# google-research/seed_rl

Measured on NVIDIA H100. Metric: env-frames/sec (learner, device-timed) on synthetic 84x84x4 T=20 unrolls @1/2/4/8 H100, higher is better.
Workload: dtype bf16x3 (fp32-faithful tensor-core contraction; activations stored as bf16 hi+lo pairs), f32 elsewhere

## Files before the change

include/seedrl_b200.h:

```cpp
#ifndef SEEDRL_B200_H_
#define SEEDRL_B200_H_

#include <stddef.h>
#include <stdint.h>

#ifdef __cplusplus
extern "C" {
#endif

#define SEEDRL_OK 0
#define SEEDRL_ERR_INVALID_ARGUMENT 3
#define SEEDRL_ERR_OUT_OF_RANGE 11
#define SEEDRL_ERR_INTERNAL 13
#define SEEDRL_ERR_CANCELLED 1
#define SEEDRL_ERR_UNAVAILABLE 14

typedef void* seedrl_stream_t;

const char* seedrl_last_error(void);
int seedrl_abi_version(void);
uint64_t seedrl_kernel_launch_count(void);

int seedrl_vtrace_from_importance_weights(
    int T, int B,
    const float* target_action_log_probs, const float* behaviour_action_log_probs,
    const float* discounts, const float* rewards, const float* values,
    const float* bootstrap_value,
    float clip_rho_threshold, float clip_pg_rho_threshold, float lambda_,
    float* vs, float* pg_advantages, seedrl_stream_t stream);

int seedrl_categorical_log_prob(int N, int A, const float* logits,
                                const int64_t* actions, float* log_prob,
                                seedrl_stream_t stream);
int seedrl_categorical_entropy(int N, int A, const float* logits, float* entropy,
                               seedrl_stream_t stream);
int seedrl_categorical_sample(int N, int A, const float* logits,
                              const float* gumbel_noise, uint64_t seed,
                              uint64_t offset, int64_t* actions,
                              seedrl_stream_t stream);
int seedrl_categorical_sample_counter(int N, int A, const float* logits, const float* gumbel_noise,
                                      uint64_t seed, uint64_t* counter_dev, int64_t* actions,
                                      seedrl_stream_t stream);

typedef struct seedrl_loss_config {
  float discounting;
  float lambda_;
  float baseline_cost;
  float kl_cost;
  float max_abs_reward;
  float clip_rho_threshold;
  float clip_pg_rho_threshold;
  float target_entropy;
  int32_t has_target_entropy;
  float entropy_cost_adjustment_speed;
// ... 171 lines not shown
                             const int64_t* replay_action, const float* reward, const uint8_t* done,
                             const float* importance_weights, float gamma, int n_steps, float eta,
                             float value_rescaling_eps, float* loss, float* priorities, float* dq,
                             void* scratch, seedrl_stream_t stream);
size_t seedrl_r2d2_retrace_loss_scratch_bytes(int T, int B);
int seedrl_r2d2_retrace_loss_fwd_bwd(int T, int B, int A, const float* q_train, const float* q_target,
                                     const int64_t* replay_action, const float* reward,
                                     const uint8_t* done, const float* importance_weights, float gamma,
                                     float lambda_, float eta, float value_rescaling_eps, float* loss,
                                     float* priorities, float* dq, void* scratch,
                                     seedrl_stream_t stream);
int seedrl_r2d2_epsilon_greedy(int N, int A, const int32_t* env_ids, const float* envs_epsilon,
                               uint64_t seed, uint64_t* counter_dev, int32_t* actions,
                               seedrl_stream_t stream);
int seedrl_replay_sample(int limit, const float* priorities, float priority_exp,
                         float importance_sampling_exp, int num_samples, const float* uniforms,
                         int64_t* indices, float* weights, float* probs_out, seedrl_stream_t stream);
size_t seedrl_clip_scratch_bytes(void);
int seedrl_clip_by_global_norm(size_t n, float* grads, float clip_norm, float* norm_out,
                               void* scratch, seedrl_stream_t stream);

int seedrl_debug_conv3x3(int cin, int cout, int in_mode, int N, int H, int W,
                         const void* in, const float* w, const float* bias,
                         const float* mask, const float* res, float* out,
                         seedrl_stream_t stream);
int seedrl_debug_conv3x3_flip(int cin, int cout, const float* w, float* wt,
                              seedrl_stream_t stream);
size_t seedrl_debug_wgrad_partial_bytes(void);
int seedrl_debug_conv_pixels(int N, int H, int W, int which, int start, int count, int* out);
int seedrl_debug_set_loss_stream(int enabled);
int seedrl_debug_set_wgrad_chunk(int kc);
int seedrl_debug_set_conv_tile(int mt);
int seedrl_debug_set_gemm_gather(int on);
int seedrl_debug_set_first_layer_dense(int on);
int seedrl_debug_conv0pool(int N, int H, int W, const uint8_t* frames, const float* w, const float* bias,
                           void* praw, void* prelu, uint8_t* idx, int* err, seedrl_stream_t stream);
int seedrl_debug_conv0pool_c(int N, int H, int W, int C, const uint8_t* frames, const float* w, const float* bias,
                             void* praw, void* prelu, uint8_t* idx, int* err, seedrl_stream_t stream);
int seedrl_debug_first_wgrad_pooled_c(int N, int H, int W, int C, const uint8_t* frames, const void* g_planes,
                                      const uint8_t* idx, float* dw, float* db, float* partial,
                                      size_t partial_bytes, seedrl_stream_t stream);
int seedrl_debug_conv3x3_wgrad(int cin, int cout, int in_mode, int N, int H, int W,
                               const void* x, const float* dy, float* dw, float* db,
                               float* partial, size_t partial_bytes,
                               seedrl_stream_t stream);
int seedrl_debug_conv3x3_tc(int cin, int cout, int in_mode, int split, int N, int H, int W,
                            const void* in, const float* w, const float* bias,
                            const float* mask, const float* res, float* out, int flip,
                            int variant, void* wq_scratch, int* error_flag,
                            seedrl_stream_t stream);
int seedrl_debug_conv3x3_wgrad_tc(int cin, int cout, int in_mode, int split, int N, int H, int W,
                                  const void* x, const float* dy, float* dw, float* db,
                                  float* partial, size_t partial_bytes, int* error_flag,
                                  seedrl_stream_t stream);
int seedrl_debug_maxpool(int backward, int N, int H, int W, int C, const float* x_or_dy,
                         float* y_or_dx, uint8_t* idx, seedrl_stream_t stream);
int seedrl_debug_gemm_tc(int ta, int tb, int split, int M, int N, int K, const float* A, int lda,
                         const float* B, int ldb, float* C, int ldc, const float* bias,
                         const float* mask, int ldm, int relu, int accumulate, int a_relu,
                         float* ws, size_t ws_bytes, int* error_flag, seedrl_stream_t stream);
int seedrl_debug_colsum(int M, int N, const float* X, int ld, float* out, float* ws, size_t ws_bytes,
                        seedrl_stream_t stream);
int seedrl_debug_sgemm(int ta, int tb, int M, int N, int K, const float* A, int lda,
                       const float* B, int ldb, float* C, int ldc, const float* bias,
                       const float* mask, int ldm, int relu, int accumulate, int a_relu,
                       seedrl_stream_t stream);
// ... 36 lines not shown
```

seed_rl_b200/_lib.py:

```python
import ctypes
import os

_HERE = os.path.dirname(os.path.abspath(__file__))
LIB_PATH = os.path.join(_HERE, 'libseedrl_b200.so')

c_void_p, c_int, c_float, c_size_t = ctypes.c_void_p, ctypes.c_int, ctypes.c_float, ctypes.c_size_t
c_i64, c_u64 = ctypes.c_int64, ctypes.c_uint64
P = c_void_p


class SeedrlError(RuntimeError):

  def __init__(self, code, msg):
    super().__init__('libseedrl_b200 error %d: %s' % (code, msg))
    self.code = code


class LossConfig(ctypes.Structure):
  _fields_ = [('discounting', c_float), ('lambda_', c_float), ('baseline_cost', c_float),
              ('kl_cost', c_float), ('max_abs_reward', c_float),
              ('clip_rho_threshold', c_float), ('clip_pg_rho_threshold', c_float),
              ('target_entropy', c_float), ('has_target_entropy', ctypes.c_int32),
              ('entropy_cost_adjustment_speed', c_float)]

# ... 5 lines not shown

ROW_GATHER, ROW_SCATTER, ROW_APPEND = 0, 1, 2


def rows_multi(jobs, env_ids_i32, index=None, id_limit=None):
  n = int(env_ids_i32.numel())
  arr = (RowJob * len(jobs))()
  for k, (table, rows, mode) in enumerate(jobs):
    rb = (table[0, 0] if mode == ROW_APPEND else table[0]).numel() * table.element_size()
    if rows.numel() * rows.element_size() != n * rb or rows.dtype != table.dtype or not rows.is_contiguous():
      raise ValueError('rows_multi: rows do not match the table (job %d)' % k)
    arr[k] = RowJob(table.data_ptr(), rows.data_ptr(), rb, mode, table.shape[1] if mode == ROW_APPEND else 0)
  if id_limit is None:
    check(lib().seedrl_rows_multi(arr, len(jobs), ptr(env_ids_i32), n, ptr(index), stream_ptr()))
  else:
    check(lib().seedrl_rows_multi_limit(arr, len(jobs), ptr(env_ids_i32), n, ptr(index), int(id_limit),
                                        stream_ptr()))


class NetConfig(ctypes.Structure):
  _fields_ = [('net', ctypes.c_int32), ('num_actions', ctypes.c_int32),
              ('obs_h', ctypes.c_int32), ('obs_w', ctypes.c_int32), ('obs_c', ctypes.c_int32)]


NET_DEEP, NET_SHALLOW = 0, 1
LOSS_TERMS = 16
LT = dict(total=0, policy=1, V=2, entropy=3, kl=4, entropy_adj=5, v_mean=6, v_l2_error=7,
          mean_entropy=8, entropy_cost=9, mean_kl=10, max_action_abs=11, popart_mean=12, popart_std=13)

SIGNATURES = {
    'seedrl_last_error': (ctypes.c_char_p, []),
    'seedrl_abi_version': (c_int, []),
    'seedrl_kernel_launch_count': (c_u64, []),
    'seedrl_vtrace_from_importance_weights':
        (c_int, [c_int, c_int, P, P, P, P, P, P, c_float, c_float, c_float, P, P, P]),
    'seedrl_categorical_log_prob': (c_int, [c_int, c_int, P, P, P, P]),
    'seedrl_categorical_entropy': (c_int, [c_int, c_int, P, P, P]),
    'seedrl_categorical_sample': (c_int, [c_int, c_int, P, P, c_u64, c_u64, P, P]),
    'seedrl_categorical_sample_counter': (c_int, [c_int, c_int, P, P, c_u64, P, P, P]),
    'seedrl_vtrace_loss_scratch_bytes': (c_size_t, [c_int, c_int, c_int]),
    'seedrl_vtrace_loss_fwd_bwd':
        (c_int, [c_int, c_int, c_int, P, P, P, P, P, P, ctypes.POINTER(LossConfig), P,
                 P, P, P, P, P, P, P, P]),
    'seedrl_vtrace_popart_loss_fwd':
        (c_int, [c_int, c_int, c_int, P, P, P, P, P, P, ctypes.POINTER(LossConfig), P, P, P,
                 P, P, P, P, P, P, P, P, P, P]),
    'seedrl_vtrace_popart_update':
        (c_int, [c_int, c_int, c_int, c_float, c_float, P, P, P, P, P, P, P, P, P, P]),
    'seedrl_adam_apply':
        (c_int, [c_size_t, P, P, P, P, c_float, c_float, c_float, c_float, c_float, c_i64,
                 c_float, c_float, P]),
    'seedrl_net_create': (c_int, [ctypes.POINTER(NetConfig), ctypes.POINTER(P)]),
    'seedrl_net_destroy': (None, [P]),
    'seedrl_net_num_param_tensors': (c_int, [P]),
    'seedrl_net_num_params': (c_size_t, [P]),
    'seedrl_net_arena_floats': (c_size_t, [P]),
    'seedrl_net_set_conv_mode': (c_int, [P, c_int]),
    'seedrl_net_set_lstm_mode': (c_int, [P, c_int]),
    'seedrl_net_param_info':
        (c_int, [P, c_int, ctypes.c_char_p, c_size_t, ctypes.POINTER(c_i64),
                 ctypes.POINTER(c_size_t)]),
    'seedrl_net_workspace_bytes': (c_size_t, [P, c_int, c_int]),
    'seedrl_net_forward':
        (c_int, [P, P, c_int, c_int, P, P, P, P, P, P, P, P, P, P, P, c_size_t, P]),
    'seedrl_net_backward':
        (c_int, [P, P, c_int, c_int, P, P, P, P, P, P, P, P, c_size_t, P]),
# ... 51 lines not shown
    'seedrl_clip_by_global_norm': (c_int, [c_size_t, P, c_float, P, P, P]),
    'seedrl_profile_num_categories': (c_int, []),
    'seedrl_profile_category_name': (ctypes.c_char_p, [c_int]),
    'seedrl_profile_begin': (c_int, [P]),
    'seedrl_profile_end': (c_int, [ctypes.POINTER(ctypes.c_double), ctypes.POINTER(c_u64)]),
    'seedrl_debug_planes_bytes': (c_size_t, [c_int, c_int, c_int, c_int]),
    'seedrl_debug_to_planes': (c_int, [c_int, c_int, c_int, c_int, c_int, P, P, P]),
    'seedrl_debug_from_planes': (c_int, [c_int, c_int, c_int, c_int, P, P, P]),
    'seedrl_debug_convp': (c_int, [c_int, c_int, c_int, c_int, c_int, P, P, P, P, P, c_int, P, P, P, P, P, P]),
    'seedrl_debug_wgradp': (c_int, [c_int, c_int, c_int, c_int, c_int, P, P, P, P, P, c_size_t, P, P]),
    'seedrl_debug_poolp': (c_int, [c_int, c_int, c_int, c_int, c_int, P, P, P, P, P, P]),
    'seedrl_debug_conv3x3': (c_int, [c_int, c_int, c_int, c_int, c_int, c_int, P, P, P, P, P, P, P]),
    'seedrl_debug_conv3x3_flip': (c_int, [c_int, c_int, P, P, P]),
    'seedrl_debug_conv3x3_tc':
        (c_int, [c_int, c_int, c_int, c_int, c_int, c_int, c_int, P, P, P, P, P, P, c_int, c_int, P, P, P]),
    'seedrl_debug_wgrad_partial_bytes': (c_size_t, []),
    'seedrl_debug_conv_pixels': (c_int, [c_int, c_int, c_int, c_int, c_int, c_int, P]),
    'seedrl_debug_set_loss_stream': (c_int, [c_int]),
    'seedrl_debug_set_wgrad_chunk': (c_int, [c_int]),
    'seedrl_debug_set_conv_tile': (c_int, [c_int]),
    'seedrl_debug_set_first_layer_dense': (c_int, [c_int]),
    'seedrl_debug_conv0pool': (c_int, [c_int, c_int, c_int, P, P, P, P, P, P, P, P]),
    'seedrl_debug_conv0pool_c': (c_int, [c_int, c_int, c_int, c_int, P, P, P, P, P, P, P, P]),
    'seedrl_debug_first_wgrad_pooled_c': (c_int, [c_int, c_int, c_int, c_int, P, P, P, P, P, P, c_size_t, P]),
    'seedrl_debug_conv3x3_wgrad_tc':
        (c_int, [c_int, c_int, c_int, c_int, c_int, c_int, c_int, P, P, P, P, P, c_size_t, P, P]),
    'seedrl_debug_conv3x3_wgrad':
        (c_int, [c_int, c_int, c_int, c_int, c_int, c_int, P, P, P, P, P, c_size_t, P]),
    'seedrl_debug_maxpool': (c_int, [c_int, c_int, c_int, c_int, c_int, P, P, P, P]),
    'seedrl_debug_gemm_tc':
        (c_int, [c_int, c_int, c_int, c_int, c_int, c_int, P, c_int, P, c_int, P, c_int, P, P, c_int, c_int, c_int,
                 c_int, P, c_size_t, P, P]),
    'seedrl_debug_set_gemm_gather': (c_int, [c_int]),
    'seedrl_debug_colsum': (c_int, [c_int, c_int, P, c_int, P, P, c_size_t, P]),
    'seedrl_debug_sgemm':
        (c_int, [c_int, c_int, c_int, c_int, c_int, P, c_int, P, c_int, P, c_int, P, P, c_int,
                 c_int, c_int, c_int, P]),
    'seedrl_debug_strided_conv':
        (c_int, [c_int, c_int, c_int, c_int, c_int, c_int, c_int, c_int, c_int, c_int, c_int, P, P, P, P, P, P,
                 c_int, P, P, c_size_t, P, c_size_t, P, ctypes.POINTER(c_int), P]),
    'seedrl_debug_lstm_workspace_bytes': (c_size_t, [c_int, c_int, c_int, c_int]),
    'seedrl_debug_lstm_forward':
        (c_int, [c_int, c_int, c_int, c_int, P, P, P, P, P, P, P, P, P, c_size_t, P, P]),
    'seedrl_debug_lstm_backward':
        (c_int, [c_int, c_int, c_int, c_int, P, P, P, P, P, P, P, P, c_size_t, P, P]),
    'seedrl_debug_r2d2_net_views':
        (c_int, [P, c_int, c_int, c_int, ctypes.POINTER(c_size_t), ctypes.POINTER(c_size_t)]),
    'seedrl_debug_net_views':
        (c_int, [P, c_int, c_int, c_int, ctypes.POINTER(c_size_t), ctypes.POINTER(c_size_t),
                 ctypes.POINTER(c_int)]),
}

_lib = None


def lib():
  global _lib
  if _lib is None:
    if not os.path.exists(LIB_PATH):
      raise ImportError(
          'seed_rl_b200: %s is missing -- build it with `python -c "import '
          '__graft_entry__ as g; g.build()"` (seed_rl_b200/csrc/build.sh). There is no '
          'CPU or PyTorch fallback.' % LIB_PATH)
    l = ctypes.CDLL(LIB_PATH)
    for name, (res, args) in SIGNATURES.items():
      fn = getattr(l, name)
      fn.restype = res
      fn.argtypes = args
    _lib = l
  return _lib


def check(rc):
  if rc != 0:
    raise SeedrlError(rc, (lib().seedrl_last_error() or b'').decode('utf-8', 'replace'))


def launch_count():
  return int(lib().seedrl_kernel_launch_count())


def ptr(t):
  return None if t is None else ctypes.c_void_p(t.data_ptr())


def stream_ptr():
  import torch
  return ctypes.c_void_p(torch.cuda.current_stream().cuda_stream)


def require_cuda(t, dtype, name):
  import torch
  if not isinstance(t, torch.Tensor):
    t = torch.as_tensor(t)
  if not torch.cuda.is_available():
    raise RuntimeError('seed_rl_b200 needs a CUDA device (H100); there is no CPU path '
                       '(argument %r).' % name)
  if t.device.type != 'cuda':
    t = t.cuda()
  if t.dtype != dtype:
    t = t.to(dtype)
  return t.contiguous()
```

seed_rl_b200/csrc/capi.cu:

```cuda
#include <vector>

#include "common.cuh"

namespace seedrl {
thread_local std::string g_last_error;
std::atomic<uint64_t> g_launch_count{0};
bool g_prof_on = false;
int g_conv_cat = PC_CONV_FWD;

struct ProfRec { int cat; cudaEvent_t e; };
static std::vector<ProfRec> g_prof;
static cudaEvent_t g_prof_start;

void prof_mark_(int cat, cudaStream_t st) {
  ProfRec r;
  r.cat = cat;
  cudaEventCreate(&r.e);
  cudaEventRecord(r.e, st);
  g_prof.push_back(r);
}
}

static const char* kProfNames[seedrl::PC_COUNT] = {
    "conv3x3_fwd", "conv3x3_dgrad", "conv3x3_wgrad", "maxpool", "sgemm", "lstm_pointwise",
    "vtrace_loss", "adam", "vtrace", "misc"};

extern "C" const char* seedrl_last_error(void) { return seedrl::g_last_error.c_str(); }
extern "C" int seedrl_abi_version(void) { return 1; }
extern "C" uint64_t seedrl_kernel_launch_count(void) {
  return seedrl::g_launch_count.load(std::memory_order_relaxed);
}

extern "C" int seedrl_profile_num_categories(void) { return seedrl::PC_COUNT; }
extern "C" const char* seedrl_profile_category_name(int i) {
  return (i >= 0 && i < seedrl::PC_COUNT) ? kProfNames[i] : "";
}
extern "C" int seedrl_profile_begin(seedrl_stream_t stream) {
  seedrl::g_prof.clear();
  cudaEventCreate(&seedrl::g_prof_start);
  cudaEventRecord(seedrl::g_prof_start, (cudaStream_t)stream);
  seedrl::g_prof_on = true;
  return SEEDRL_OK;
}
extern "C" int seedrl_profile_end(double* ms_per_category, uint64_t* launches_per_category) {
  seedrl::g_prof_on = false;
  if (!ms_per_category || !launches_per_category)
    return seedrl::set_error(SEEDRL_ERR_INVALID_ARGUMENT, "seedrl_profile_end: null pointer");
  if (cudaDeviceSynchronize() != cudaSuccess)
    return seedrl::set_error(SEEDRL_ERR_INTERNAL, "seedrl_profile_end: device sync failed");
  for (int i = 0; i < seedrl::PC_COUNT; ++i) {
    ms_per_category[i] = 0;
    launches_per_category[i] = 0;
  }
  cudaEvent_t prev = seedrl::g_prof_start;
  for (auto& r : seedrl::g_prof) {
    float ms = 0.f;
    if (cudaEventElapsedTime(&ms, prev, r.e) == cudaSuccess) {
      ms_per_category[r.cat] += ms;
      launches_per_category[r.cat] += 1;
    }
    cudaEventDestroy(prev);
    prev = r.e;
  }
// ... 5 lines not shown
```

seed_rl_b200/csrc/common.cuh:

```cuda
#pragma once
#include <cuda.h>
#include <cuda_runtime.h>
#include <stdint.h>
#include <stdio.h>

#include <atomic>
#include <string>

#include "../../include/seedrl_b200.h"

namespace seedrl {

extern thread_local std::string g_last_error;
extern std::atomic<uint64_t> g_launch_count;

inline int set_error(int code, const std::string& msg) {
  g_last_error = msg;
  return code;
}

#define SEEDRL_TRY(expr)                \
  do {                                  \
    const int rc__ = (expr);            \
    if (rc__ != SEEDRL_OK) return rc__; \
  } while (0)

#define SEEDRL_CHECK_ARG(cond, msg)                                         \
  do {                                                                      \
    if (!(cond))                                                            \
      return ::seedrl::set_error(SEEDRL_ERR_INVALID_ARGUMENT,               \
                                 std::string(__func__) + ": " + (msg));     \
  } while (0)

#define SEEDRL_CHECK_LAUNCH()                                               \
  do {                                                                      \
    cudaError_t e__ = cudaGetLastError();                                   \
    if (e__ != cudaSuccess)                                                 \
      return ::seedrl::set_error(                                           \
          SEEDRL_ERR_INTERNAL, std::string(__func__) + ": CUDA launch: " +  \
                                   cudaGetErrorString(e__));                \
  } while (0)

#define SEEDRL_CUDA(...)                                                    \
  do {                                                                      \
    cudaError_t e__ = (__VA_ARGS__);                                        \
    if (e__ != cudaSuccess)                                                 \
      return ::seedrl::set_error(                                           \
          SEEDRL_ERR_INTERNAL,                                              \
          std::string(__func__) + ": " #__VA_ARGS__ ": " + cudaGetErrorString(e__)); \
  } while (0)

enum ProfCat { PC_CONV_FWD = 0, PC_CONV_DGRAD, PC_CONV_WGRAD, PC_POOL, PC_GEMM, PC_LSTM_PW,
               PC_LOSS, PC_ADAM, PC_VTRACE, PC_MISC, PC_COUNT };
extern bool g_prof_on;
extern int g_conv_cat;
void prof_mark_(int cat, cudaStream_t st);

inline void count_launch(int cat = PC_MISC, cudaStream_t st = 0) {
  g_launch_count.fetch_add(1, std::memory_order_relaxed);
  if (g_prof_on) prof_mark_(cat, st);
}

constexpr int kNumSMs = 132;

template <auto K>
cudaError_t allow_smem(int bytes) {
  static const cudaError_t e = cudaFuncSetAttribute(K, cudaFuncAttributeMaxDynamicSharedMemorySize, bytes);
  return e;
}

typedef CUresult (*EncodeTiledFn)(CUtensorMap*, CUtensorMapDataType, cuuint32_t, void*, const cuuint64_t*,
                                  const cuuint64_t*, const cuuint32_t*, const cuuint32_t*, CUtensorMapInterleave,
                                  CUtensorMapSwizzle, CUtensorMapL2promotion, CUtensorMapFloatOOBfill);
inline EncodeTiledFn encode_tiled_fn() {
  static const EncodeTiledFn fn = [] {
    void* q = nullptr;
    cudaDriverEntryPointQueryResult qr;
    const bool found = cudaGetDriverEntryPoint("cuTensorMapEncodeTiled", &q, cudaEnableDefault, &qr) == cudaSuccess &&
                       qr == cudaDriverEntryPointSuccess;
    (void)cudaGetLastError();
    return found ? reinterpret_cast<EncodeTiledFn>(q) : nullptr;
  }();
  return fn;
}

__host__ __device__ inline int ceil_div(int a, int b) { return (a + b - 1) / b; }
__host__ __device__ inline size_t ceil_div_sz(size_t a, size_t b) { return (a + b - 1) / b; }

__device__ __forceinline__ float warp_sum(float v) {
#pragma unroll
  for (int o = 16; o > 0; o >>= 1) v += __shfl_xor_sync(0xffffffffu, v, o);
  return v;
}
__device__ __forceinline__ float warp_max(float v) {
#pragma unroll
// ... 21 lines not shown
```

seed_rl_b200/csrc/conv_first.cu:

```cuda
#include <cuda.h>

#include <cstring>

#include "kernels.h"
#include "tc_common.cuh"

namespace seedrl {

constexpr int kFwThreads = 256;
constexpr int kFwCo = 16;
constexpr int kFwLanes = kFwThreads / kFwCo;

static inline int first_layer_cp(int c) { return c <= 4 ? 4 : (c <= 8 ? 8 : 16); }
static inline int fw_rows_per_band(int cp) { return cp == 16 ? 4 : 6; }
static inline size_t fw_pixels_8b(int cp, int rb, int W) { return ((size_t)(2 * rb + 3) * (W + 2) * (cp / 4) + 1) & ~(size_t)1; }
static inline size_t fw_smem(int cp, int rb, int W) {
  const int wo = (W + 1) / 2;
  return fw_pixels_8b(cp, rb, W) * 8 + (size_t)rb * wo * kFwCo * 5;
}

struct FirstWgradArgs {
  int N, H, W, C, Ho, Wo, pt, pl;
  int Lpp, PWp, RHp;
  int rb;
  const uint8_t* frames;
  const uint4* g;
  const uint8_t* idx;
  float* partial;
};

__device__ __forceinline__ uint32_t load_u8x4(const uint8_t* px, int c0, int C) {
  uint32_t v = 0u;
#pragma unroll
  for (int j = 0; j < 4; ++j)
    if (c0 + j < C) v |= (uint32_t)__ldg(px + c0 + j) << (8 * j);
  return v;
}

template <int CP, bool kU32>
__global__ void __launch_bounds__(kFwThreads, kU32 ? 3 : 2) first_wgrad_pooled_kernel(const FirstWgradArgs a) {
  constexpr int G = CP / 4;
  constexpr int NL = kFwLanes / G;
  extern __shared__ __align__(128) uint8_t smem_raw[];
  const int tid = threadIdx.x;
  const int co = tid & (kFwCo - 1), grp = (tid >> 4) & (G - 1), ql = (tid >> 4) / G;
  const int SW = a.W + 2;
  const int RB = a.rb;
  const int SR = 2 * RB + 3;
  uint2* s_x = reinterpret_cast<uint2*>(smem_raw);
  float* s_g = reinterpret_cast<float*>(s_x + ((SR * SW * G + 1) & ~1));
  uint8_t* s_t = reinterpret_cast<uint8_t*>(s_g + RB * a.Wo * kFwCo);
  float acc[36];
#pragma unroll
  for (int i = 0; i < 36; ++i) acc[i] = 0.f;
  float accb = 0.f;
  const int bands = (a.Ho + RB - 1) / RB;
  const int units = a.N * bands;
  for (int u = blockIdx.x; u < units; u += gridDim.x) {
    const int n = u / bands, band = u - n * bands;
    const int r0 = band * RB, r1 = min(a.Ho, r0 + RB);
    const int nq = (r1 - r0) * a.Wo;
    const int f0 = 2 * r0 - a.pt - 1;
    for (int i = tid; i < SR * SW * G; i += kFwThreads) {
      const int px = i / G, gi = i - px * G;
      const int lr = px / SW, bc = px - lr * SW, fr = f0 + lr;
      uint32_t w32 = 0u;
      if (fr >= 0 && fr < a.H && bc >= 1 && bc <= a.W) {
        const size_t pix = ((size_t)n * a.H + fr) * a.W + bc - 1;
        if (kU32) w32 = __ldg(reinterpret_cast<const uint32_t*>(a.frames) + pix);
        else w32 = load_u8x4(a.frames + pix * a.C, 4 * gi, a.C);
      }
      const uint32_t f0_ = __float_as_uint(__uint_as_float(__byte_perm(w32, 0x4B000000u, 0x7540)) - 8388608.0f);
      const uint32_t f1_ = __float_as_uint(__uint_as_float(__byte_perm(w32, 0x4B000000u, 0x7541)) - 8388608.0f);
      const uint32_t f2_ = __float_as_uint(__uint_as_float(__byte_perm(w32, 0x4B000000u, 0x7542)) - 8388608.0f);
      const uint32_t f3_ = __float_as_uint(__uint_as_float(__byte_perm(w32, 0x4B000000u, 0x7543)) - 8388608.0f);
      s_x[i] = make_uint2(__byte_perm(f0_, f1_, 0x7632), __byte_perm(f2_, f3_, 0x7632));
    }
    for (int i = tid; i < nq * 2; i += kFwThreads) {
      const int gq = i & 1, qq = i >> 1;
      const int qr = qq / a.Wo, qw = qq - qr * a.Wo;
      const size_t sp = (size_t)(n * a.RHp + r0 + qr + 1) * a.PWp + qw + 1;
      const uint4 hh = __ldg(a.g + (size_t)gq * a.Lpp + sp), ll = __ldg(a.g + (size_t)(2 + gq) * a.Lpp + sp);
      float4* dst = reinterpret_cast<float4*>(s_g + (size_t)qq * kFwCo + gq * 8);
      dst[0] = make_float4(__uint_as_float(hh.x << 16) + __uint_as_float(ll.x << 16),
                           __uint_as_float(hh.x & 0xFFFF0000u) + __uint_as_float(ll.x & 0xFFFF0000u),
                           __uint_as_float(hh.y << 16) + __uint_as_float(ll.y << 16),
                           __uint_as_float(hh.y & 0xFFFF0000u) + __uint_as_float(ll.y & 0xFFFF0000u));
      dst[1] = make_float4(__uint_as_float(hh.z << 16) + __uint_as_float(ll.z << 16),
// ... 31 lines not shown
      while (qw >= a.Wo) { qw -= a.Wo; ++qh; }
    }
    __syncthreads();
  }
  float* s_red = reinterpret_cast<float*>(smem_raw);
  const int slot = ql * G + grp;
#pragma unroll
  for (int i = 0; i < 36; ++i) s_red[(slot * 37 + i) * kFwCo + co] = acc[i];
  s_red[(slot * 37 + 36) * kFwCo + co] = accb;
  __syncthreads();
  const int nw = 9 * a.C;
  float* dst = a.partial + (size_t)blockIdx.x * ((nw + 1) * kFwCo);
  for (int e = tid; e < (nw + 1) * kFwCo; e += kFwThreads) {
    const int i = e / kFwCo, c = e - i * kFwCo;
    const int tap = i / a.C, ci = i - tap * a.C;
    const int gi = i < nw ? ci >> 2 : 0, k = i < nw ? tap * 4 + (ci & 3) : 36;
    float s = 0.f;
#pragma unroll
    for (int l = 0; l < NL; ++l) s += s_red[((l * G + gi) * 37 + k) * kFwCo + c];
    if (i < nw) dst[i * kFwCo + c] = s * (1.0f / 255.0f);
    else dst[nw * kFwCo + c] = s;
  }
}

bool first_wgrad_pooled_supported(int cin, int cout, int H, int W) {
  if (cin < 1 || cin > 16 || cout != 16 || H < 3 || W < 3) return false;
  const int cp = first_layer_cp(cin);
  return fw_smem(cp, fw_rows_per_band(cp), W) <= 70 * 1024;
}

template <int CP, bool kU32>
static int launch_first_wgrad(const FirstWgradArgs& a, int grid, size_t smem, cudaStream_t st) {
  SEEDRL_CUDA(allow_smem<first_wgrad_pooled_kernel<CP, kU32>>(72 * 1024));
  first_wgrad_pooled_kernel<CP, kU32><<<grid, kFwThreads, smem, st>>>(a);
  return SEEDRL_OK;
}

int first_wgrad_pooled(int N, int H, int W, int C, const uint8_t* frames, const void* g_planes, const uint8_t* idx,
                       float* dw, float* db, WgradBatch* batch, cudaStream_t st) {
  if (!first_wgrad_pooled_supported(C, 16, H, W))
    return set_error(SEEDRL_ERR_INVALID_ARGUMENT, "first_wgrad_pooled: unsupported frame shape");
  int Ho, Wo, pt, pl;
  same_pad3s2(H, &Ho, &pt);
  same_pad3s2(W, &Wo, &pl);
  const int cp = first_layer_cp(C);
  FirstWgradArgs a;
  a.N = N; a.H = H; a.W = W; a.C = C; a.Ho = Ho; a.Wo = Wo; a.pt = pt; a.pl = pl;
  a.Lpp = (int)planes_positions(N, Ho, Wo); a.PWp = Wo + 2; a.RHp = Ho + 1;
  a.frames = frames; a.g = reinterpret_cast<const uint4*>(g_planes); a.idx = idx;
  a.rb = fw_rows_per_band(cp) < Ho ? fw_rows_per_band(cp) : Ho;
  size_t smem = fw_smem(cp, a.rb, W);
  const size_t red = (size_t)kFwLanes * 37 * kFwCo * 4;
  if (red > smem) smem = red;
  smem = (smem + 127) / 128 * 128;
  const int NW = 9 * C * kFwCo + kFwCo;
  const int units = N * ((Ho + a.rb - 1) / a.rb);
  int grid = (C == 4 ? 3 : 2) * kNumSMs;
  if (grid > units) grid = units;
  if (!batch || batch->n >= kMaxReduceJobs || batch->used + (size_t)grid * NW > batch->cap_floats)
    return set_error(SEEDRL_ERR_INVALID_ARGUMENT, "first_wgrad_pooled: partial buffer too small");
  a.partial = batch->buf + batch->used;
  batch->used += (size_t)grid * NW;
  const int rc = C == 4    ? launch_first_wgrad<4, true>(a, grid, smem, st)
                 : cp == 4 ? launch_first_wgrad<4, false>(a, grid, smem, st)
                 : cp == 8 ? launch_first_wgrad<8, false>(a, grid, smem, st)
                           : launch_first_wgrad<16, false>(a, grid, smem, st);
  if (rc != SEEDRL_OK) return rc;
  count_launch(PC_CONV_WGRAD, st);
  SEEDRL_CHECK_LAUNCH();
  batch->jobs[batch->n++] = ReduceJob{a.partial, dw, db, grid, 9 * C * kFwCo, kFwCo};
  return SEEDRL_OK;
}

constexpr int kCpThreadsF = 256;
constexpr int kCpRows = 3;
constexpr int kCpMaxBlocks = 6;
constexpr int kCpOutStride = 20;

struct Conv0PoolArgs {
  int N, H, W, Ho, Wo, pt, pl;
  int Lpp, PWp, RHp;
  int C;
  unsigned int sw_mul; int sw_sh;
  const uint8_t* frames;
  const float* w;
  const float* bias;
  uint4* praw; uint4* prelu;
  uint8_t* idx;
  int* err;
};

__device__ __forceinline__ uint2 u8x4_to_bf16x4(uint32_t w32) {
  const uint32_t f0 = __float_as_uint(__uint_as_float(__byte_perm(w32, 0x4B000000u, 0x7540)) - 8388608.0f);
  const uint32_t f1 = __float_as_uint(__uint_as_float(__byte_perm(w32, 0x4B000000u, 0x7541)) - 8388608.0f);
  const uint32_t f2 = __float_as_uint(__uint_as_float(__byte_perm(w32, 0x4B000000u, 0x7542)) - 8388608.0f);
  const uint32_t f3 = __float_as_uint(__uint_as_float(__byte_perm(w32, 0x4B000000u, 0x7543)) - 8388608.0f);
  return make_uint2(__byte_perm(f0, f1, 0x7632), __byte_perm(f2, f3, 0x7632));
}

template <int CP, bool kTma>
__global__ void __launch_bounds__(kCpThreadsF, 2) conv0pool_kernel(const __grid_constant__ CUtensorMap tm_frames,
// ... 9 lines not shown
  uint4* s_p = reinterpret_cast<uint4*>(smem_raw);
  float* s_out = reinterpret_cast<float*>(smem_raw + (size_t)kPlanes * npair * 16);
  uint8_t* s_bq = reinterpret_cast<uint8_t*>(s_out + (size_t)kCpMaxBlocks * 128 * kCpOutStride);
  s_bq = reinterpret_cast<uint8_t*>(((uintptr_t)s_bq + 127) & ~(uintptr_t)127);
  float* s_bias = reinterpret_cast<float*>(s_bq + KT * 32 * 2);
  uint64_t* s_full = reinterpret_cast<uint64_t*>(s_bias + 16);
  constexpr int kRawRows = 2 * kCpRows + 3;
  uint32_t* s_raw = reinterpret_cast<uint32_t*>(((uintptr_t)(s_full + 4) + 127) & ~(uintptr_t)127);
  const uint32_t raw_bytes = (uint32_t)(kRawRows * W) * 4u;
  const uint32_t raw_stride = (raw_bytes + 127u) & ~127u;

  for (int i = tid; i < KT * 32; i += kCpThreadsF) {
    const int k = i / 32, nn = i - k * 32;
    const int kh = k / KH, kw = (k - kh * KH) / CP, ci = k - kh * KH - kw * CP;
    float v = 0.f;
    if (kw < 3 && ci < a.C) {
      const float wv = __ldg(a.w + ((kh * 3 + kw) * a.C + ci) * 16 + (nn & 15));
      v = nn < 16 ? wv : bf16_resid(wv);
    }
    const uint32_t off = (uint32_t)(k >> 3) * 512u + (uint32_t)(nn >> 3) * 128u + (uint32_t)(nn & 7) * 16u +
                         (uint32_t)(k & 7) * 2u;
    *reinterpret_cast<__nv_bfloat16*>(s_bq + off) = __float2bfloat16_rn(v);
  }
  if (tid < 16) s_bias[tid] = __ldg(a.bias + tid);
  for (int i = tid; i < kPlanes * npair; i += kCpThreadsF) s_p[i] = make_uint4(0u, 0u, 0u, 0u);
  if (kTma && tid == 0) {
    mbar_init(s_full, 1);
    mbar_init(s_full + 1, 1);
    asm volatile("fence.mbarrier_init.release.cluster;" ::: "memory");
    asm volatile("prefetch.tensormap [%0];" ::"l"(reinterpret_cast<uint64_t>(&tm_frames)) : "memory");
  }
  asm volatile("fence.proxy.async.shared::cta;" ::: "memory");
  __syncthreads();
  const uint32_t a_base = smem_u32(s_p), b_base = smem_u32(s_bq);

  const int bands = (a.Ho + kCpRows - 1) / kCpRows;
  const int units = a.N * bands;
  bool timed_out = false;
  auto unit_geom = [&](int u, int* n, int* r0, int* r1, int* cr0, int* cr1) {
    *n = u / bands;
    const int band = u - *n * bands;
    *r0 = band * kCpRows; *r1 = min(a.Ho, *r0 + kCpRows);
    *cr0 = max(0, 2 * *r0 - a.pt); *cr1 = min(H - 1, 2 * (*r1 - 1) - a.pt + 2);
  };
  auto issue_tile = [&](int u, int st) {
    int n, r0, r1, cr0, cr1;
    unit_geom(u, &n, &r0, &r1, &cr0, &cr1);
    const uint32_t dst = smem_u32(s_raw) + (uint32_t)st * raw_stride, bar = smem_u32(s_full + st);
    asm volatile("mbarrier.arrive.expect_tx.shared::cta.b64 _, [%0], %1;" ::"r"(bar), "r"(raw_bytes) : "memory");
    asm volatile(
        "cp.async.bulk.tensor.3d.shared::cluster.global.tile.mbarrier::complete_tx::bytes [%0], [%1, {%2, %3, %4}], [%5];" ::
            "r"(dst), "l"(reinterpret_cast<uint64_t>(&tm_frames)), "r"(0), "r"(cr0 - 1), "r"(n), "r"(bar)
        : "memory");
  };
  if (kTma && tid == 0 && (int)blockIdx.x < units) issue_tile(blockIdx.x, 0);
  int it = 0;
  for (int u = blockIdx.x; u < units; u += gridDim.x, ++it) {
    int n, r0, r1, cr0, cr1;
    unit_geom(u, &n, &r0, &r1, &cr0, &cr1);
    const int band = u - n * bands;
    const int CR = cr1 - cr0 + 1, npos = CR * SW, nblk = (npos + 127) >> 7;
    const int st = it & 1;
    if constexpr (kTma) {
      if (tid == 0 && u + (int)gridDim.x < units) issue_tile(u + gridDim.x, st ^ 1);
      if (!mbar_wait_bounded(s_full + st, (uint32_t)((it >> 1) & 1))) timed_out = true;
      const uint32_t* raw = s_raw + (size_t)st * (raw_stride / 4);
// ... 123 lines not shown
        const size_t sp = (size_t)(n * a.RHp + r0 + rr + 1) * a.PWp + (side ? a.Wo + 1 : 0);
        a.praw[(size_t)pl_ * a.Lpp + sp] = z;
        a.prelu[(size_t)pl_ * a.Lpp + sp] = z;
      }
      if (band == 0) {
        for (int i = tid; i < a.PWp * 4; i += kCpThreadsF) {
          const int pl_ = i & 3, cc = i >> 2;
          const size_t sp = (size_t)(n * a.RHp) * a.PWp + cc;
          a.praw[(size_t)pl_ * a.Lpp + sp] = z;
          a.prelu[(size_t)pl_ * a.Lpp + sp] = z;
        }
      }
      if (u == units - 1) {
        const int t0 = a.N * a.RHp * a.PWp;
        for (int i = tid; i < (a.Lpp - t0) * 4; i += kCpThreadsF) {
          const int pl_ = i & 3, cc = i >> 2;
          a.praw[(size_t)pl_ * a.Lpp + t0 + cc] = z;
          a.prelu[(size_t)pl_ * a.Lpp + t0 + cc] = z;
        }
      }
    }
    __syncthreads();
  }
  if (timed_out && a.err) atomicExch(a.err, 1);
}

bool conv0pool_supported(int cin, int cout, int H, int W) {
  if (cout != 16 || H < 3 || W < 3 || 7 * (W + 2) > 6 * 128) return false;
  if (cin == 4) return W % 4 == 0 && W <= 256;
  return cin >= 1 && cin <= 16;
}

template <int CP, bool TMA>
static int launch_conv0pool(Conv0PoolArgs a, const uint8_t* frames, cudaStream_t st) {
  constexpr int KT = 3 * (CP == 16 ? 48 : 4 * CP);
  const int N = a.N, H = a.H, W = a.W;
  const size_t raw_stride = TMA ? (((size_t)(2 * kCpRows + 3) * W * 4) + 127) / 128 * 128 : 0;
  const size_t smem = (size_t)(CP == 16 ? 2 : 1) * (kCpMaxBlocks * 128 + 2 * (W + 2) + 8) * 16 +
                      (size_t)kCpMaxBlocks * 128 * kCpOutStride * 4 + 128 + KT * 32 * 2 + 16 * 4 + 64 + 128 +
                      2 * raw_stride;
  SEEDRL_CUDA(allow_smem<conv0pool_kernel<CP, TMA>>(112 * 1024));
  if (smem > 112 * 1024) return set_error(SEEDRL_ERR_INVALID_ARGUMENT, "conv0pool: image too wide");
  CUtensorMap tm;
  memset(&tm, 0, sizeof(tm));
  if (TMA) {
    const EncodeTiledFn enc = encode_tiled_fn();
    if (!enc) return set_error(SEEDRL_ERR_INTERNAL, "cuTensorMapEncodeTiled is not available");
    const cuuint64_t gdim[3] = {(cuuint64_t)W, (cuuint64_t)H, (cuuint64_t)N};
    const cuuint64_t gstr[2] = {(cuuint64_t)W * 4, (cuuint64_t)H * W * 4};
    const cuuint32_t box[3] = {(cuuint32_t)W, (cuuint32_t)(2 * kCpRows + 3), 1};
    const cuuint32_t estr[3] = {1, 1, 1};
    if (enc(&tm, CU_TENSOR_MAP_DATA_TYPE_UINT32, 3, const_cast<uint8_t*>(frames), gdim, gstr, box, estr,
            CU_TENSOR_MAP_INTERLEAVE_NONE, CU_TENSOR_MAP_SWIZZLE_NONE, CU_TENSOR_MAP_L2_PROMOTION_L2_128B,
            CU_TENSOR_MAP_FLOAT_OOB_FILL_NONE) != CUDA_SUCCESS)
      return set_error(SEEDRL_ERR_INTERNAL, "conv0pool: cuTensorMapEncodeTiled failed");
  }
  const int units = N * ((a.Ho + kCpRows - 1) / kCpRows);
  const int grid = units < 2 * kNumSMs ? units : 2 * kNumSMs;
  conv0pool_kernel<CP, TMA><<<grid, kCpThreadsF, smem, st>>>(tm, a);
  count_launch(PC_CONV_FWD, st);
  SEEDRL_CHECK_LAUNCH();
  return SEEDRL_OK;
}

int conv0pool_forward(int N, int H, int W, int C, const uint8_t* frames, const float* w, const float* bias,
                      void* praw, void* prelu, uint8_t* idx, int* err, cudaStream_t st) {
  if (!conv0pool_supported(C, 16, H, W))
    return set_error(SEEDRL_ERR_INVALID_ARGUMENT, "conv0pool: unsupported frame shape");
  Conv0PoolArgs a;
  a.N = N; a.H = H; a.W = W; a.C = C;
  same_pad3s2(H, &a.Ho, &a.pt);
  same_pad3s2(W, &a.Wo, &a.pl);
  a.Lpp = (int)planes_positions(N, a.Ho, a.Wo); a.PWp = a.Wo + 2; a.RHp = a.Ho + 1;
  fast_div_setup((unsigned int)(W + 2), &a.sw_mul, &a.sw_sh);
  a.frames = frames; a.w = w; a.bias = bias;
  a.praw = reinterpret_cast<uint4*>(praw); a.prelu = reinterpret_cast<uint4*>(prelu); a.idx = idx; a.err = err;
  if (C == 4) return launch_conv0pool<4, true>(a, frames, st);
  const int cp = first_layer_cp(C);
  return cp == 4 ? launch_conv0pool<4, false>(a, frames, st)
                 : (cp == 8 ? launch_conv0pool<8, false>(a, frames, st) : launch_conv0pool<16, false>(a, frames, st));
}

}
```

seed_rl_b200/csrc/conv_planes.cu:

```cuda
#include <cuda.h>
#include <cuda_bf16.h>

#include <cstdio>

#include "kernels.h"
#include "tc_common.cuh"

namespace seedrl {

long long planes_positions(int N, int H, int W) {
  const long long Q = (long long)N * (H + 1) * (W + 2);
  return ((Q + 2 * (W + 2) + 2 + 256 + 127) / 128) * 128;
}
size_t planes_bytes(int N, int H, int W, int C) {
  return (size_t)planes_positions(N, H, W) * 16 * 2 * (C / 8);
}

constexpr int kPlanesChunk = 128;

static int make_plane_map(CUtensorMap* tm, const void* base, long long Lp, int planes, int shift,
                          int CH, int box_chunks, int box_planes) {
  EncodeTiledFn enc = encode_tiled_fn();
  if (!enc) return set_error(SEEDRL_ERR_INTERNAL, "cuTensorMapEncodeTiled is not available");
  if (box_chunks < 1 || box_chunks > 256 || box_planes < 1 || box_planes > planes)
// ... 65 lines not shown
    }
  }
}

template <int CIN, int COUT, int NSUB>
__global__ void __launch_bounds__(kCpThreads, 1)
convp_kernel(const __grid_constant__ CUtensorMap tm_in, const ConvpArgs a) {
  constexpr int G = CIN / 8, GO = COUT / 8, NS = CIN / 16;
  constexpr int MT = NSUB * kCpM;
  constexpr int NBLK = 2 * NSUB;
  extern __shared__ __align__(128) uint8_t smem_raw[];
  const int PW = a.g.PW, nb = a.nb;
  const uint32_t P = (uint32_t)(a.nch * a.chunk) * 16u;
  const uint32_t stage_bytes = 2u * G * P;
  uint8_t* s_stage = smem_raw;
  uint4* s_b = reinterpret_cast<uint4*>(smem_raw + (size_t)nb * stage_bytes);
  float* s_bias = reinterpret_cast<float*>(s_b + 2 * 9 * CIN * COUT / 8);
  uint64_t* s_full = reinterpret_cast<uint64_t*>(s_bias + COUT);
  uint64_t* s_empty = s_full + kCpMaxStages;
  const int tid = threadIdx.x, warp = tid >> 5, lane = tid & 31;

  for (int i = tid; i < 2 * 9 * CIN * COUT / 8; i += kCpThreads) s_b[i] = __ldg(a.wq + i);
  if (tid < COUT) s_bias[tid] = a.bias ? __ldg(a.bias + tid) : 0.f;
  if (tid == 0) {
    for (int i = 0; i < nb; ++i) {
      mbar_init(s_full + i, 1);
      mbar_init(s_empty + i, 4 * kCpWarpgroups);
    }
    asm volatile("fence.mbarrier_init.release.cluster;" ::: "memory");
    asm volatile("prefetch.tensormap [%0];" ::"l"(reinterpret_cast<uint64_t>(&tm_in)) : "memory");
  }
  asm volatile("fence.proxy.async.shared::cta;" ::: "memory");
  __syncthreads();

  const int my_tiles = ((int)blockIdx.x < a.ntiles) ? (a.ntiles - 1 - (int)blockIdx.x) / (int)gridDim.x + 1 : 0;
  bool timed_out = false;

  if (warp == 4 * kCpWarpgroups) {
    if (elect_one()) {
      for (int it = 0; it < my_tiles; ++it) {
        const int s = it % nb;
        if (it >= nb && !mbar_wait_bounded(s_empty + s, (uint32_t)(((it / nb) - 1) & 1))) { timed_out = true; break; }
        const int tile = (int)blockIdx.x + it * (int)gridDim.x;
        mbar_expect_tx(s_full + s, stage_bytes);
        tma_load_3d(s_stage + (size_t)s * stage_bytes, &tm_in, 0, tile * MT / a.chunk, 0, s_full + s);
      }
    }
    __syncwarp();
  } else {
    const int cw = warp >> 2;
    const size_t plane_u = (size_t)a.Lp;
    if (blockIdx.x == 0) {
      const uint4 z = make_uint4(0u, 0u, 0u, 0u);
      for (int i = tid; i < (PW + 1) * 2 * GO; i += 128 * kCpWarpgroups) {
        const int pl = i / (PW + 1), s = i - pl * (PW + 1);
        if (a.out_raw) a.out_raw[(size_t)pl * plane_u + s] = z;
        if (a.out_relu) a.out_relu[(size_t)pl * plane_u + s] = z;
      }
    }
    const int q = lane & 3;
    const int row = 16 * (warp & 3) + (lane >> 2) + 8 * (q & 1);
    const uint32_t b_base = smem_u32(s_b);
    const uint64_t db0 = gmma_desc(b_base, (uint32_t)(2 * GO) * 128u, 128u);
    for (int it = 0; it < my_tiles; ++it) {
      const int s = it % nb;
      const int tile = (int)blockIdx.x + it * (int)gridDim.x;
// ... 98 lines not shown
      }
    }
  }
  if (timed_out && a.err) atomicExch(a.err, 1);
}

template <int CIN, int COUT, int NSUB>
static int launch_convp(const PlaneConv& c, cudaStream_t st) {
  const ConvGeom g = make_geom(c.N, c.H, c.W);
  constexpr int MT = NSUB * kCpM;
  const long long Lp = planes_positions(c.N, c.H, c.W);
  if (Lp + MT + 4 * g.PW >= (1LL << 31))
    return set_error(SEEDRL_ERR_INVALID_ARGUMENT, "convp: batch too large for 32-bit positions");
  const int L = MT + 2 * g.PW + 2;
  const int CH = kPlanesChunk;
  const int nch = (L + CH - 1) / CH;
  const size_t stage = (size_t)2 * (CIN / 8) * nch * CH * 16;
  const size_t fixed = (size_t)2 * 9 * CIN * COUT * 2 + COUT * 4 + 2 * kCpMaxStages * 8;
  int nb = kCpMaxStages;
  while (nb > 1 && nb * stage + fixed > 227 * 1024) --nb;
  if (nb < 2) return kPlanesTryNext;
  const size_t smem = nb * stage + fixed;
  CUtensorMap tm;
  SEEDRL_TRY(make_plane_map(&tm, c.in, Lp, 2 * (CIN / 8), 0, CH, nch, 2 * (CIN / 8)));
  SEEDRL_CUDA(allow_smem<convp_kernel<CIN, COUT, NSUB>>(227 * 1024));
  ConvpArgs a;
  a.g = g; a.Lp = (int)Lp; a.nch = nch; a.chunk = CH; a.nb = nb;
  a.ntiles = (int)((Lp - g.PW - 1 + MT - 1) / MT);
  a.wq = reinterpret_cast<const uint4*>(c.wq); a.bias = c.bias;
  a.mask = reinterpret_cast<const uint4*>(c.mask); a.res = reinterpret_cast<const uint4*>(c.res);
  a.out_raw = reinterpret_cast<uint4*>(c.out_raw); a.out_relu = reinterpret_cast<uint4*>(c.out_relu);
  a.out_nhwc = c.out_nhwc; a.err = c.err;
  const int grid = a.ntiles < kNumSMs ? a.ntiles : kNumSMs;
  convp_kernel<CIN, COUT, NSUB><<<grid, kCpThreads, smem, st>>>(tm, a);
  count_launch(g_conv_cat, st);
  SEEDRL_CHECK_LAUNCH();
  return SEEDRL_OK;
}

bool convp_supported(int cin, int cout) {
  return (cin == 16 || cin == 32) && (cout == 16 || cout == 32);
}

int convp_forward(int cin, int cout, const PlaneConv& c, cudaStream_t st) {
  const long long Lp = planes_positions(c.N, c.H, c.W);
  const bool small = Lp / 512 < 2 * kNumSMs;
#define SEEDRL_CP_CASE(CI, CO_)                                                   \
  if (cin == CI && cout == CO_) {                                                 \
    int rc = kPlanesTryNext;                                                      \
    if (!small) rc = launch_convp<CI, CO_, 4>(c, st);                             \
    if (rc == kPlanesTryNext) rc = launch_convp<CI, CO_, 2>(c, st);               \
    if (rc == kPlanesTryNext) rc = launch_convp<CI, CO_, 1>(c, st);               \
    if (rc == kPlanesTryNext) return set_error(SEEDRL_ERR_INVALID_ARGUMENT, "convp: image too wide"); \
    return rc;                                                                    \
  }
  SEEDRL_CP_CASE(16, 16)
  SEEDRL_CP_CASE(16, 32)
  SEEDRL_CP_CASE(32, 16)
  SEEDRL_CP_CASE(32, 32)
#undef SEEDRL_CP_CASE
  return set_error(SEEDRL_ERR_INVALID_ARGUMENT, "convp: unsupported (cin,cout)");
}

struct WgradpArgs {
  int PW, T, nchunks, nb;
  int chunk;
  float* partial;
  int* err;
};

constexpr int kWpMaxStages = 6;
constexpr int kWpHaloRow = 8;
__host__ __device__ constexpr int wgradp_mtiles(int CP) { return 3 * CP + 1 <= 64 ? 1 : 2; }
__host__ __device__ constexpr int wgradp_khsplit(int CP) { return CP == 16 ? 3 : 1; }
__host__ __device__ constexpr int wgradp_threads(int CP) { return 128 * wgradp_mtiles(CP) * wgradp_khsplit(CP) + 32; }

struct WgradMaps { CUtensorMap x, x_halo, dy, dy_halo; };

template <int CP, int COUT, int KC>
__global__ void __launch_bounds__(wgradp_threads(CP), 1)
wgradp_kernel(const __grid_constant__ WgradMaps tm, const WgradpArgs a) {
  constexpr int G = CP / 8, GO = COUT / 8;
  constexpr int MT = wgradp_mtiles(CP), KSPL = wgradp_khsplit(CP), NCW = MT * KSPL;
  constexpr int NKH = 3 / KSPL;
  constexpr int NW = 9 * CP * COUT + COUT;
  constexpr uint32_t Px = (KC + kWpHaloRow) * 16;
  extern __shared__ __align__(128) uint8_t smem_raw[];
  const int nb = a.nb, PW = a.PW;
  const uint32_t Pd = (uint32_t)(KC + a.T) * 16u;
  const uint32_t x_bytes = 2u * G * Px;
  const uint32_t stage_bytes = x_bytes + 2u * GO * Pd;
  uint64_t* s_full = reinterpret_cast<uint64_t*>(smem_raw);
  uint64_t* s_empty = s_full + kWpMaxStages;
  uint8_t* s_stage = smem_raw + 128;
  const int tid = threadIdx.x, warp = tid >> 5, lane = tid & 31;

  if (tid == 0) {
    for (int i = 0; i < kWpMaxStages; ++i) { mbar_init(s_full + i, 1); mbar_init(s_empty + i, 4 * NCW); }
    asm volatile("fence.mbarrier_init.release.cluster;" ::: "memory");
  }
  __syncthreads();

  const int my_chunks = ((int)blockIdx.x < a.nchunks) ? (a.nchunks - 1 - (int)blockIdx.x) / (int)gridDim.x + 1 : 0;
  bool timed_out = false;

  if (warp == 4 * NCW) {
    if (elect_one()) {
      for (int it = 0; it < my_chunks; ++it) {
        const int s = it % nb;
        if (it >= nb && !mbar_wait_bounded(s_empty + s, (uint32_t)(((it / nb) - 1) & 1))) { timed_out = true; break; }
        const int j0 = ((int)blockIdx.x + it * (int)gridDim.x) * KC;
        uint8_t* xs = s_stage + (size_t)s * stage_bytes;
        uint8_t* ds = xs + x_bytes;
        mbar_expect_tx(s_full + s, stage_bytes);
        for (int p = 0; p < 2 * G; ++p) {
          tma_load_3d(xs + p * Px, &tm.x, 0, j0 / a.chunk, p, s_full + s);
          tma_load_3d(xs + p * Px + KC * 16, &tm.x_halo, 0, (j0 + KC) / kWpHaloRow, p, s_full + s);
        }
        for (int p = 0; p < 2 * GO; ++p) {
          tma_load_3d(ds + p * Pd, &tm.dy, 0, j0 / a.chunk, p, s_full + s);
          tma_load_3d(ds + p * Pd + KC * 16, &tm.dy_halo, 0, (j0 + KC) / kWpHaloRow, p, s_full + s);
        }
      }
    }
    __syncwarp();
  } else {
    const int cw = warp >> 2, mt = cw % MT, kh0 = (cw / MT) * NKH;
    const int mg0 = 8 * mt + 2 * (warp & 3);
    const int mg = mg0 + ((lane >> 3) & 1);
    const uint32_t a_off = (mg < 3 * G ? (uint32_t)(mg % G) * Px + (uint32_t)(mg / G) * 16u : 0u) +
                           (uint32_t)((lane >> 4) * 8 + (lane & 7)) * 16u;
    const bool data0 = mg0 < 3 * G, data1 = mg0 + 1 < 3 * G;
    const uint32_t one = (lane >> 2) == 0 ? 0x3F803F80u : 0u;
    const uint32_t c0 = mg0 == 3 * G ? one : 0u, c1 = mg0 + 1 == 3 * G ? one : 0u;
// ... 55 lines not shown
  }
  if (timed_out && a.err) atomicExch(a.err, 1);
}

template <int CP, int COUT, int KC>
static int launch_wgradp(int N, int H, int W, const void* x, const void* dy, float* dw, float* db, int* err,
                         WgradBatch* batch, cudaStream_t st) {
  const ConvGeom g = make_geom(N, H, W);
  const long long Lp = planes_positions(N, H, W);
  constexpr int G = CP / 8, GO = COUT / 8;
  const int CH = kPlanesChunk < KC ? kPlanesChunk : KC;
  if (KC % CH) return kPlanesTryNext;
  const int T = (2 * g.PW + kWpHaloRow - 1) / kWpHaloRow * kWpHaloRow;
  const size_t stage = (size_t)2 * G * (KC + kWpHaloRow) * 16 + (size_t)2 * GO * (KC + T) * 16;
  int nb = kWpMaxStages;
  while (nb > 1 && 128 + nb * stage > 227 * 1024) --nb;
  if (nb < 2) return kPlanesTryNext;
  const size_t smem = 128 + nb * stage;
  WgradMaps tm;
  SEEDRL_TRY(make_plane_map(&tm.x, x, Lp, 2 * G, g.PW, CH, KC / CH, 1));
  SEEDRL_TRY(make_plane_map(&tm.x_halo, x, Lp, 2 * G, g.PW, kWpHaloRow, 1, 1));
  SEEDRL_TRY(make_plane_map(&tm.dy, dy, Lp, 2 * GO, 1, CH, KC / CH, 1));
  SEEDRL_TRY(make_plane_map(&tm.dy_halo, dy, Lp, 2 * GO, 1, kWpHaloRow, T / kWpHaloRow, 1));
  SEEDRL_CUDA(allow_smem<wgradp_kernel<CP, COUT, KC>>(227 * 1024));
  constexpr int NW = 9 * CP * COUT + COUT;
  WgradpArgs a;
  a.PW = g.PW; a.T = T; a.nb = nb; a.err = err; a.chunk = CH;
  a.nchunks = (int)((g.Q + g.PW + KC - 1) / KC);
  const int grid = a.nchunks < kNumSMs ? a.nchunks : kNumSMs;
  if (!batch || batch->n >= kMaxReduceJobs || batch->used + (size_t)grid * NW > batch->cap_floats)
    return set_error(SEEDRL_ERR_INVALID_ARGUMENT, "wgradp: partial buffer too small");
  a.partial = batch->buf + batch->used;
  batch->used += (size_t)grid * NW;
  wgradp_kernel<CP, COUT, KC><<<grid, wgradp_threads(CP), smem, st>>>(tm, a);
  count_launch(PC_CONV_WGRAD, st);
  SEEDRL_CHECK_LAUNCH();
  batch->jobs[batch->n++] = ReduceJob{a.partial, dw, db, grid, 9 * CP * COUT, COUT};
  return SEEDRL_OK;
}

int wgradp(int cin, int cout, int N, int H, int W, const void* x, const void* dy, float* dw, float* db,
           int* err, WgradBatch* batch, cudaStream_t st) {
#define SEEDRL_WP_CASE(CI, CO_, KC0)                                                                        \
  if (cin == CI && cout == CO_) {                                                                           \
    int rc = kPlanesTryNext;                                                                                \
    if constexpr (KC0 >= 256) rc = launch_wgradp<CI, CO_, 256>(N, H, W, x, dy, dw, db, err, batch, st);     \
    if (rc == kPlanesTryNext) rc = launch_wgradp<CI, CO_, 128>(N, H, W, x, dy, dw, db, err, batch, st);     \
    if (rc == kPlanesTryNext) rc = launch_wgradp<CI, CO_, 64>(N, H, W, x, dy, dw, db, err, batch, st);      \
    if (rc == kPlanesTryNext) return set_error(SEEDRL_ERR_INVALID_ARGUMENT, "wgradp: does not fit");        \
    return rc;                                                                                              \
  }
  SEEDRL_WP_CASE(16, 16, 256)
  SEEDRL_WP_CASE(16, 32, 128)
  SEEDRL_WP_CASE(32, 32, 128)
#undef SEEDRL_WP_CASE
  return set_error(SEEDRL_ERR_INVALID_ARGUMENT, "wgradp: unsupported (cin,cout)");
}

__global__ void to_planes_kernel(ConvGeom g, int Lp, int G, int relu, const float* __restrict__ x,
                                 uint4* __restrict__ out) {
  const long long i = (long long)blockIdx.x * blockDim.x + threadIdx.x;
  if (i >= (long long)Lp * G) return;
  const int s = (int)(i / G), go = (int)(i - (long long)s * G);
  const int pix = in_pixel(g, s);
  float4 a = make_float4(0.f, 0.f, 0.f, 0.f), b = a;
  if (pix >= 0) {
    const float4* src = reinterpret_cast<const float4*>(x + (size_t)pix * (G * 8) + go * 8);
    a = __ldg(src); b = __ldg(src + 1);
    if (relu) {
      a.x = fmaxf(a.x, 0.f); a.y = fmaxf(a.y, 0.f); a.z = fmaxf(a.z, 0.f); a.w = fmaxf(a.w, 0.f);
      b.x = fmaxf(b.x, 0.f); b.y = fmaxf(b.y, 0.f); b.z = fmaxf(b.z, 0.f); b.w = fmaxf(b.w, 0.f);
    }
  }
  out[(size_t)go * Lp + s] = pack8_bf16(a, b);
  out[(size_t)(G + go) * Lp + s] = pack8_bf16(bf16_resid4(a), bf16_resid4(b));
}

__global__ void from_planes_kernel(ConvGeom g, int Lp, int G, const uint4* __restrict__ in, float* __restrict__ y) {
  const long long i = (long long)blockIdx.x * blockDim.x + threadIdx.x;
  if (i >= (long long)Lp * G) return;
  const int s = (int)(i / G), go = (int)(i - (long long)s * G);
  const int pix = in_pixel(g, s);
  if (pix < 0) return;
  const uint4 h = __ldg(in + (size_t)go * Lp + s), l = __ldg(in + (size_t)(G + go) * Lp + s);
  float4* dst = reinterpret_cast<float4*>(y + (size_t)pix * (G * 8) + go * 8);
  dst[0] = make_float4(bf16lo(h.x) + bf16lo(l.x), bf16hi(h.x) + bf16hi(l.x), bf16lo(h.y) + bf16lo(l.y),
                       bf16hi(h.y) + bf16hi(l.y));
  dst[1] = make_float4(bf16lo(h.z) + bf16lo(l.z), bf16hi(h.z) + bf16hi(l.z), bf16lo(h.w) + bf16lo(l.w),
                       bf16hi(h.w) + bf16hi(l.w));
}

int to_planes(int N, int H, int W, int C, int relu, const float* x, void* out, cudaStream_t st) {
  const ConvGeom g = make_geom(N, H, W);
  const long long Lp = planes_positions(N, H, W);
  const long long n = Lp * (C / 8);
  to_planes_kernel<<<(unsigned)((n + 255) / 256), 256, 0, st>>>(g, (int)Lp, C / 8, relu, x,
                                                                reinterpret_cast<uint4*>(out));
  count_launch(PC_MISC, st);
  SEEDRL_CHECK_LAUNCH();
  return SEEDRL_OK;
}
int from_planes(int N, int H, int W, int C, const void* in, float* y, cudaStream_t st) {
  const ConvGeom g = make_geom(N, H, W);
  const long long Lp = planes_positions(N, H, W);
  const long long n = Lp * (C / 8);
  from_planes_kernel<<<(unsigned)((n + 255) / 256), 256, 0, st>>>(g, (int)Lp, C / 8,
                                                                  reinterpret_cast<const uint4*>(in), y);
  count_launch(PC_MISC, st);
  SEEDRL_CHECK_LAUNCH();
  return SEEDRL_OK;
}

__global__ void poolp_fwd_kernel(ConvGeom go_, int Lp, int G, int H, int W, int pt, int pl,
                                 const float* __restrict__ x, uint4* __restrict__ out_raw,
                                 uint4* __restrict__ out_relu, uint8_t* __restrict__ idx) {
  const long long i = (long long)blockIdx.x * blockDim.x + threadIdx.x;
  if (i >= (long long)Lp * G) return;
  const int s = (int)(i / G), gq = (int)(i - (long long)s * G);
  const int pix = in_pixel(go_, s);
  float best[8];
  unsigned char arg[8];
#pragma unroll
  for (int e = 0; e < 8; ++e) { best[e] = 0.f; arg[e] = 0; }
  if (pix >= 0) {
    const int Wo = go_.W, Ho = go_.H, C = G * 8;
    const int n = pix / (Ho * Wo), r = pix - n * (Ho * Wo), ho = r / Wo, wo = r - ho * Wo;
#pragma unroll
    for (int e = 0; e < 8; ++e) best[e] = -INFINITY;
#pragma unroll
    for (int kh = 0; kh < 3; ++kh) {
      const int h = ho * 2 - pt + kh;
      if (h < 0 || h >= H) continue;
#pragma unroll
      for (int kw = 0; kw < 3; ++kw) {
        const int w = wo * 2 - pl + kw;
        if (w < 0 || w >= W) continue;
        const float4* src = reinterpret_cast<const float4*>(x + ((size_t)(n * H + h) * W + w) * C + gq * 8);
        const float4 a = __ldg(src), b = __ldg(src + 1);
        const float v[8] = {a.x, a.y, a.z, a.w, b.x, b.y, b.z, b.w};
        const unsigned char t = (unsigned char)(kh * 3 + kw);
#pragma unroll
        for (int e = 0; e < 8; ++e)
          if (v[e] > best[e]) { best[e] = v[e]; arg[e] = t; }
      }
    }
    uint2 packed;
    packed.x = arg[0] | (arg[1] << 8) | (arg[2] << 16) | ((uint32_t)arg[3] << 24);
    packed.y = arg[4] | (arg[5] << 8) | (arg[6] << 16) | ((uint32_t)arg[7] << 24);
    *reinterpret_cast<uint2*>(idx + (size_t)pix * C + gq * 8) = packed;
  }
  const float4 a = make_float4(best[0], best[1], best[2], best[3]), b = make_float4(best[4], best[5], best[6], best[7]);
  out_raw[(size_t)gq * Lp + s] = pack8_bf16(a, b);
  out_raw[(size_t)(G + gq) * Lp + s] = pack8_bf16(bf16_resid4(a), bf16_resid4(b));
  const float4 ra = make_float4(fmaxf(a.x, 0.f), fmaxf(a.y, 0.f), fmaxf(a.z, 0.f), fmaxf(a.w, 0.f));
  const float4 rb = make_float4(fmaxf(b.x, 0.f), fmaxf(b.y, 0.f), fmaxf(b.z, 0.f), fmaxf(b.w, 0.f));
  out_relu[(size_t)gq * Lp + s] = pack8_bf16(ra, rb);
  out_relu[(size_t)(G + gq) * Lp + s] = pack8_bf16(bf16_resid4(ra), bf16_resid4(rb));
}

template <bool OUT_PLANES>
__global__ void poolp_bwd_kernel(ConvGeom gf, int Lpf, ConvGeom gp, int Lpp, int G, int pt, int pl,
                                 const uint4* __restrict__ dy, const uint8_t* __restrict__ idx,
                                 uint4* __restrict__ dx_planes, float* __restrict__ dx_nhwc) {
  const long long i = (long long)blockIdx.x * blockDim.x + threadIdx.x;
  const int H = gf.H, W = gf.W, Ho = gp.H, Wo = gp.W, C = G * 8;
  int gq, s = 0, pix;
  if (OUT_PLANES) {
    if (i >= (long long)Lpf * G) return;
    s = (int)(i / G); gq = (int)(i - (long long)s * G);
    pix = in_pixel(gf, s);
  } else {
    if (i >= (long long)gf.N * H * W * G) return;
    pix = (int)(i / G); gq = (int)(i - (long long)pix * G);
  }
  float acc[8];
#pragma unroll
  for (int e = 0; e < 8; ++e) acc[e] = 0.f;
  if (pix >= 0) {
    const int n = pix / (H * W), r = pix - n * (H * W), h = r / W, w = r - h * W;
    const int hp = h + pt, wp = w + pl;
#pragma unroll
    for (int dh = 0; dh < 2; ++dh) {
      const int ho = (hp >> 1) - dh;
      const int kh = hp - 2 * ho;
      if (ho < 0 || ho >= Ho || kh > 2) continue;
#pragma unroll
      for (int dw = 0; dw < 2; ++dw) {
        const int wo = (wp >> 1) - dw;
        const int kw = wp - 2 * wo;
        if (wo < 0 || wo >= Wo || kw > 2) continue;
        const unsigned tap = (unsigned)(kh * 3 + kw);
        const size_t o = ((size_t)(n * Ho + ho) * Wo + wo) * C + gq * 8;
        const uint2 t = __ldg(reinterpret_cast<const uint2*>(idx + o));
        const int sp = (n * gp.RH + ho + 1) * gp.PW + wo + 1;
        const uint4 hh = __ldg(dy + (size_t)gq * Lpp + sp), ll = __ldg(dy + (size_t)(G + gq) * Lpp + sp);
        const float gv[8] = {bf16lo(hh.x) + bf16lo(ll.x), bf16hi(hh.x) + bf16hi(ll.x), bf16lo(hh.y) + bf16lo(ll.y),
                             bf16hi(hh.y) + bf16hi(ll.y), bf16lo(hh.z) + bf16lo(ll.z), bf16hi(hh.z) + bf16hi(ll.z),
                             bf16lo(hh.w) + bf16lo(ll.w), bf16hi(hh.w) + bf16hi(ll.w)};
#pragma unroll
        for (int e = 0; e < 8; ++e) {
          const unsigned te = ((e < 4 ? t.x : t.y) >> (8 * (e & 3))) & 0xFFu;
          if (te == tap) acc[e] += gv[e];
        }
      }
    }
  }
  const float4 a = make_float4(acc[0], acc[1], acc[2], acc[3]), b = make_float4(acc[4], acc[5], acc[6], acc[7]);
  if (OUT_PLANES) {
    dx_planes[(size_t)gq * Lpf + s] = pack8_bf16(a, b);
    dx_planes[(size_t)(G + gq) * Lpf + s] = pack8_bf16(bf16_resid4(a), bf16_resid4(b));
  } else {
    float4* dst = reinterpret_cast<float4*>(dx_nhwc + (size_t)pix * C + gq * 8);
    dst[0] = a; dst[1] = b;
  }
}

int poolp_forward(int N, int H, int W, int C, const float* x, void* out_raw, void* out_relu, uint8_t* idx,
                  cudaStream_t st) {
  int Ho, Wo, pt, pl;
  same_pad3s2(H, &Ho, &pt);
  same_pad3s2(W, &Wo, &pl);
  const ConvGeom g = make_geom(N, Ho, Wo);
  const long long Lp = planes_positions(N, Ho, Wo);
  const long long n = Lp * (C / 8);
  poolp_fwd_kernel<<<(unsigned)((n + 255) / 256), 256, 0, st>>>(g, (int)Lp, C / 8, H, W, pt, pl, x,
                                                                reinterpret_cast<uint4*>(out_raw),
                                                                reinterpret_cast<uint4*>(out_relu), idx);
  count_launch(PC_POOL, st);
  SEEDRL_CHECK_LAUNCH();
  return SEEDRL_OK;
}

int poolp_backward(int N, int H, int W, int C, const void* dy, const uint8_t* idx, void* dx_planes,
                   float* dx_nhwc, cudaStream_t st) {
  int Ho, Wo, pt, pl;
  same_pad3s2(H, &Ho, &pt);
  same_pad3s2(W, &Wo, &pl);
  const ConvGeom gf = make_geom(N, H, W), gp = make_geom(N, Ho, Wo);
  const long long Lpf = planes_positions(N, H, W), Lpp = planes_positions(N, Ho, Wo);
  if (dx_planes) {
    const long long n = Lpf * (C / 8);
    poolp_bwd_kernel<true><<<(unsigned)((n + 255) / 256), 256, 0, st>>>(
        gf, (int)Lpf, gp, (int)Lpp, C / 8, pt, pl, reinterpret_cast<const uint4*>(dy), idx,
        reinterpret_cast<uint4*>(dx_planes), nullptr);
  } else {
    const long long n = (long long)N * H * W * (C / 8);
    poolp_bwd_kernel<false><<<(unsigned)((n + 255) / 256), 256, 0, st>>>(
        gf, (int)Lpf, gp, (int)Lpp, C / 8, pt, pl, reinterpret_cast<const uint4*>(dy), idx, nullptr, dx_nhwc);
  }
  count_launch(PC_POOL, st);
  SEEDRL_CHECK_LAUNCH();
  return SEEDRL_OK;
}

}
```

seed_rl_b200/csrc/conv_tc_kernels.cu:

```cuda
#include <cuda_bf16.h>

#include "kernels.h"
#include "tc_common.cuh"

namespace seedrl {

__global__ void pack_w_tc_kernel(int CIN, int COUT, int cin_src, int flip, int split, const float* __restrict__ w,
                                 __nv_bfloat16* __restrict__ wq) {
  const int i = blockIdx.x * blockDim.x + threadIdx.x;
  if (i >= 9 * CIN * COUT) return;
  const int e = i & 7;
  const int r = (i >> 3) & 7;
  int rest = i >> 6;
  const int cog = rest % (COUT / 8); rest /= (COUT / 8);
  const int kc = rest & 1; rest >>= 1;
  const int NS = CIN / 16;
  const int slab = rest % NS;
  const int tap = rest / NS;
  const int ci = slab * 16 + kc * 8 + e, co = cog * 8 + r;
  const float v = ci >= cin_src ? 0.f
                  : (flip ? w[((size_t)(8 - tap) * COUT + co) * CIN + ci] : w[((size_t)tap * cin_src + ci) * COUT + co]);
  const __nv_bfloat16 hi = __float2bfloat16_rn(v);
  if (split == 2) {
    const int GOc = COUT / 8;
    const size_t j = ((((size_t)(tap * NS + slab) * 2 + kc) * (2 * GOc) + cog) * 8 + r) * 8 + e;
    wq[j] = hi;
    wq[j + (size_t)GOc * 64] = __float2bfloat16_rn(v - __bfloat162float(hi));
    return;
  }
  wq[i] = hi;
  if (split) wq[9 * CIN * COUT + i] = __float2bfloat16_rn(v - __bfloat162float(hi));
}

__global__ void pack_w_tc_batch_kernel(const __grid_constant__ PackTable t, int split) {
  const PackJob j = t.jobs[blockIdx.y];
  const int CIN = j.ck, COUT = j.cout;
  const int i = blockIdx.x * blockDim.x + threadIdx.x;
  if (i >= 9 * CIN * COUT) return;
  const int e = i & 7;
  const int r = (i >> 3) & 7;
  int rest = i >> 6;
  const int cog = rest % (COUT / 8); rest /= (COUT / 8);
  const int kc = rest & 1; rest >>= 1;
  const int NS = CIN / 16;
  const int slab = rest % NS;
  const int tap = rest / NS;
  const int ci = slab * 16 + kc * 8 + e, co = cog * 8 + r;
  const float v = ci >= j.cin_src ? 0.f
                  : (j.flip ? j.w[((size_t)(8 - tap) * COUT + co) * CIN + ci]
                            : j.w[((size_t)tap * j.cin_src + ci) * COUT + co]);
  __nv_bfloat16* wq = reinterpret_cast<__nv_bfloat16*>(j.wq);
  const __nv_bfloat16 hi = __float2bfloat16_rn(v);
  if (split == 2 && !j.legacy) {
    const int GOc = COUT / 8;
    const size_t q = ((((size_t)(tap * NS + slab) * 2 + kc) * (2 * GOc) + cog) * 8 + r) * 8 + e;
    wq[q] = hi;
    wq[q + (size_t)GOc * 64] = __float2bfloat16_rn(v - __bfloat162float(hi));
    return;
  }
  wq[i] = hi;
  if (split) wq[9 * CIN * COUT + i] = __float2bfloat16_rn(v - __bfloat162float(hi));
}

int conv3x3_tc_pack_weights_batch(const PackTable& t, int split, cudaStream_t st) {
  if (t.n == 0) return SEEDRL_OK;
  pack_w_tc_batch_kernel<<<dim3(ceil_div(9 * 32 * 32, 256), t.n), 256, 0, st>>>(t, split);
  count_launch(PC_MISC, st);
  SEEDRL_CHECK_LAUNCH();
  return SEEDRL_OK;
}

constexpr int kTcThreads = 256;
constexpr int kTcM = 128;
#ifndef SEEDRL_TC_ITEMS_U8
#define SEEDRL_TC_ITEMS_U8 4
#endif
#ifndef SEEDRL_TC_ITEMS_G2
#define SEEDRL_TC_ITEMS_G2 4
#endif
#ifndef SEEDRL_TC_MIN_BLOCKS
#define SEEDRL_TC_MIN_BLOCKS 4
#endif
constexpr int kTcMinBlocks = SEEDRL_TC_MIN_BLOCKS;

template <int CIN, int COUT, int IN_MODE, bool SPLIT, int MT>
__global__ void __launch_bounds__(kTcThreads, CIN >= 32 ? kTcMinBlocks - 1 : kTcMinBlocks)
conv3x3_tc_kernel(ConvGeom g, const void* __restrict__ in_, const uint4* __restrict__ wq,
                  const float* __restrict__ bias, const float* __restrict__ mask,
                  const float* __restrict__ res, float* __restrict__ out) {
  constexpr int CK = CIN < 16 ? 16 : CIN;
  constexpr int G = CIN < 8 ? 1 : CIN / 8;
  constexpr int NS = CK / 16;
  constexpr bool ASPLIT = SPLIT && IN_MODE != IN_U8;
  constexpr int SA = ASPLIT ? 2 : 1, SB = SPLIT ? 2 : 1;
  constexpr int NBLK = MT / 64;
  constexpr int IT = IN_MODE == IN_U8 ? SEEDRL_TC_ITEMS_U8 : (G == 2 ? SEEDRL_TC_ITEMS_G2 : 4);
  extern __shared__ __align__(128) uint8_t smem_raw[];
  const int PW = g.PW;
  const int L = MT + 2 * PW + 2;
  const int LPl = L | 1;
// ... 422 lines not shown
  if (grid > nchunks) grid = (int)nchunks;
  const bool defer = batch && batch->n < kMaxReduceJobs &&
                     batch->used + (size_t)grid * NW <= batch->cap_floats;
  if (defer) {
    partial = batch->buf + batch->used;
    batch->used += (size_t)grid * NW;
  } else if ((size_t)grid * NW * sizeof(float) > partial_bytes) {
    return set_error(SEEDRL_ERR_INVALID_ARGUMENT, "wgrad_tc: partial buffer too small");
  }
  conv3x3_wgrad_tc_kernel<CIN, COUT, IN_MODE, SPLIT, KC><<<grid, kWgThreads, smem, st>>>(g, x, dy, partial, nb, err);
  count_launch(PC_CONV_WGRAD, st);
  SEEDRL_CHECK_LAUNCH();
  if (defer) {
    batch->jobs[batch->n++] = ReduceJob{partial, dw, db, grid, 9 * CIN * COUT, COUT};
    return SEEDRL_OK;
  }
  return wgrad_reduce(grid, 9 * CIN * COUT, COUT, partial, dw, db, st);
}

template <int CIN, int COUT, int IN_MODE, int KC>
static int try_wgrad_tc(int split, int N, int H, int W, const void* x, const float* dy, float* dw, float* db,
                        float* partial, size_t partial_bytes, int* err, WgradBatch* batch, cudaStream_t st) {
  if constexpr (KC > wg_max_chunk(CIN < 8 ? 8 : CIN)) {
    return kWgTryNext;
  } else {
    return split ? launch_wgrad_tc<CIN, COUT, IN_MODE, true, KC>(N, H, W, x, dy, dw, db, partial, partial_bytes,
                                                                 err, batch, st)
                 : launch_wgrad_tc<CIN, COUT, IN_MODE, false, KC>(N, H, W, x, dy, dw, db, partial, partial_bytes,
                                                                  err, batch, st);
  }
}

__global__ void wgrad_reduce_batch_kernel(const __grid_constant__ ReduceTable t) {
  const ReduceJob j = t.jobs[blockIdx.y];
  const int i = blockIdx.x * blockDim.x + threadIdx.x;
  if (i >= j.nw + j.nb) return;
  float s = 0.f;
  const size_t stride = (size_t)(j.nw + j.nb);
  const float* src = j.partial + i;
  int k = 0;
  for (; k + 8 <= j.nparts; k += 8) {
    float v[8];
#pragma unroll
    for (int q = 0; q < 8; ++q) v[q] = __ldcs(src + (size_t)(k + q) * stride);
#pragma unroll
    for (int q = 0; q < 8; ++q) s += v[q];
  }
  for (; k < j.nparts; ++k) s += __ldcs(src + (size_t)k * stride);
  if (i < j.nw) j.dw[i] = s; else j.db[i - j.nw] = s;
}

int wgrad_reduce_batch(WgradBatch* b, cudaStream_t st) {
  if (!b || b->n == 0) return SEEDRL_OK;
  ReduceTable t;
  int maxn = 0;
  for (int i = 0; i < b->n; ++i) {
    t.jobs[i] = b->jobs[i];
    if (b->jobs[i].nw + b->jobs[i].nb > maxn) maxn = b->jobs[i].nw + b->jobs[i].nb;
  }
  wgrad_reduce_batch_kernel<<<dim3(ceil_div(maxn, 256), b->n), 256, 0, st>>>(t);
  count_launch(PC_CONV_WGRAD, st);
  SEEDRL_CHECK_LAUNCH();
  b->n = 0;
  b->used = 0;
  return SEEDRL_OK;
}

int conv3x3_wgrad_tc(int cin, int cout, int in_mode, int split, int N, int H, int W, const void* x,
                     const float* dy, float* dw, float* db, float* partial, size_t partial_bytes,
                     int* err, WgradBatch* batch, cudaStream_t st) {
#define SEEDRL_WGTC_ARGS N, H, W, x, dy, dw, db, partial, partial_bytes, err, batch, st
#define SEEDRL_WGTC_CASE(CI, CO_, MODE)                                                          \
  if (cin == CI && cout == CO_ && in_mode == MODE) {                                             \
    int rc = kWgTryNext;                                                                         \
    if (g_wgrad_kc >= 512) rc = try_wgrad_tc<CI, CO_, MODE, 512>(split, SEEDRL_WGTC_ARGS);         \
    if (rc == kWgTryNext && g_wgrad_kc >= 256)                                                   \
      rc = try_wgrad_tc<CI, CO_, MODE, 256>(split, SEEDRL_WGTC_ARGS);                            \
    if (rc == kWgTryNext) rc = try_wgrad_tc<CI, CO_, MODE, 128>(split, SEEDRL_WGTC_ARGS);          \
    if (rc == kWgTryNext) return set_error(SEEDRL_ERR_INVALID_ARGUMENT, "wgrad_tc: image too wide"); \
    return rc;                                                                                   \
  }
  SEEDRL_WGTC_CASE(4, 16, IN_U8)
  SEEDRL_WGTC_CASE(16, 16, IN_RELU)
  SEEDRL_WGTC_CASE(16, 32, IN_F32)
  SEEDRL_WGTC_CASE(32, 32, IN_F32)
  SEEDRL_WGTC_CASE(32, 32, IN_RELU)
#undef SEEDRL_WGTC_CASE
#undef SEEDRL_WGTC_ARGS
  return set_error(SEEDRL_ERR_INVALID_ARGUMENT, "wgrad_tc: unsupported (cin,cout,mode)");
}

bool conv3x3_wgrad_tc_supported(int cin, int cout, int in_mode) {
  return (cin == 4 && cout == 16 && in_mode == IN_U8) || (cin == 16 && cout == 16 && in_mode == IN_RELU) ||
         (cin == 16 && cout == 32 && in_mode == IN_F32) ||
// ... 49 lines not shown
```

seed_rl_b200/csrc/gemm_kernels.cu:

```cuda
#include "kernels.h"

namespace seedrl {

template <bool TA, bool TB>
__global__ void __launch_bounds__(256)
sgemm_kernel(int M, int N, int K, const float* __restrict__ A, int lda,
             const float* __restrict__ B, int ldb, float* __restrict__ C, int ldc, GemmEpi e) {
  constexpr int BM = 64, BN = 64, BK = 16;
  __shared__ float As[BK][BM + 4];
  __shared__ float Bs[BK][BN + 4];
  const int tid = threadIdx.x;
  const int m0 = blockIdx.y * BM, n0 = blockIdx.x * BN;
  const int tx = tid & 15, ty = tid >> 4;
  float acc[4][4];
#pragma unroll
  for (int i = 0; i < 4; ++i)
#pragma unroll
    for (int j = 0; j < 4; ++j) acc[i][j] = 0.f;

  for (int k0 = 0; k0 < K; k0 += BK) {
#pragma unroll
    for (int r = 0; r < 4; ++r) {
      const int idx = tid + r * 256;
      int m, k;
// ... 24 lines not shown
      const float av[4] = {a.x, a.y, a.z, a.w};
      const float bv[4] = {b.x, b.y, b.z, b.w};
#pragma unroll
      for (int i = 0; i < 4; ++i)
#pragma unroll
        for (int j = 0; j < 4; ++j) acc[i][j] = fmaf(av[i], bv[j], acc[i][j]);
    }
    __syncthreads();
  }
#pragma unroll
  for (int i = 0; i < 4; ++i) {
    const int gm = m0 + ty * 4 + i;
    if (gm >= M) continue;
#pragma unroll
    for (int j = 0; j < 4; ++j) {
      const int gn = n0 + tx * 4 + j;
      if (gn >= N) continue;
      float v = acc[i][j];
      if (e.bias) v += e.bias[gn];
      if (e.relu) v = fmaxf(v, 0.f);
      if (e.mask) v = e.mask[(size_t)gm * e.ldm + gn] > 0.f ? v : 0.f;
      float* c = C + (size_t)gm * ldc + gn;
      *c = e.accumulate ? *c + v : v;
    }
  }
}

__global__ void colsum_kernel(int M, int N, const float* __restrict__ X, int ld, const float* __restrict__ w,
                              int ldw, float* __restrict__ out);

__global__ void __launch_bounds__(256) rowdot_kernel(int M, int K, const float* __restrict__ A, int lda,
                                                      const float* __restrict__ b, const float* __restrict__ bias,
                                                      float* __restrict__ C) {
  const int row = blockIdx.x * (blockDim.x >> 5) + (threadIdx.x >> 5), lane = threadIdx.x & 31;
  if (row >= M) return;
  const float* a = A + (size_t)row * lda;
  float s = 0.f;
  for (int k = lane; k < K; k += 32) s = fmaf(a[k], __ldg(b + k), s);
  s = warp_sum(s);
  if (lane == 0) C[row] = s + (bias ? __ldg(bias) : 0.f);
}

int sgemm(bool ta, bool tb, int M, int N, int K, const float* A, int lda, const float* B, int ldb,
          float* C, int ldc, const GemmEpi& e, cudaStream_t st) {
  if (M <= 0 || N <= 0) return SEEDRL_OK;
  if (!ta && !tb && N == 1 && ldb == 1 && ldc == 1 && !e.mask && !e.relu && !e.accumulate && !e.a_relu) {
    rowdot_kernel<<<ceil_div(M, 8), 256, 0, st>>>(M, K, A, lda, B, e.bias, C);
    count_launch(PC_GEMM, st);
    SEEDRL_CHECK_LAUNCH();
    return SEEDRL_OK;
  }
  if (ta && N == 1 && ldc == 1 && !e.bias && !e.mask && !e.relu && !e.accumulate && !e.a_relu) {
    colsum_kernel<<<ceil_div(M, 32), 1024, 0, st>>>(K, M, A, lda, B, ldb, C);
    count_launch(PC_GEMM, st);
    SEEDRL_CHECK_LAUNCH();
    return SEEDRL_OK;
  }
  constexpr int kRowsPerLaunch = 65535 * 64;
  for (int r0 = 0; r0 < M; r0 += kRowsPerLaunch) {
    const int m = M - r0 < kRowsPerLaunch ? M - r0 : kRowsPerLaunch;
    const float* Ar = ta ? A + r0 : A + (size_t)r0 * lda;
    float* Cr = C + (size_t)r0 * ldc;
    GemmEpi er = e;
    if (e.mask) er.mask = e.mask + (size_t)r0 * e.ldm;
    dim3 grid(ceil_div(N, 64), ceil_div(m, 64));
    if (!ta && !tb) sgemm_kernel<false, false><<<grid, 256, 0, st>>>(m, N, K, Ar, lda, B, ldb, Cr, ldc, er);
    else if (ta && !tb) sgemm_kernel<true, false><<<grid, 256, 0, st>>>(m, N, K, Ar, lda, B, ldb, Cr, ldc, er);
    else if (!ta && tb) sgemm_kernel<false, true><<<grid, 256, 0, st>>>(m, N, K, Ar, lda, B, ldb, Cr, ldc, er);
    else sgemm_kernel<true, true><<<grid, 256, 0, st>>>(m, N, K, Ar, lda, B, ldb, Cr, ldc, er);
    count_launch(PC_GEMM, st);
    SEEDRL_CHECK_LAUNCH();
  }
  return SEEDRL_OK;
}

__global__ void __launch_bounds__(1024)
colsum_kernel(int M, int N, const float* __restrict__ X, int ld, const float* __restrict__ w, int ldw,
              float* __restrict__ out) {
  __shared__ float red[32][33];
  const int lane = threadIdx.x & 31, wid = threadIdx.x >> 5;
  const int n = blockIdx.x * 32 + lane;
  float s0 = 0.f, s1 = 0.f, s2 = 0.f, s3 = 0.f;
  if (n < N) {
    int m = wid;
    for (; m + 96 < M; m += 128) {
      const float x0 = X[(size_t)m * ld + n], x1 = X[(size_t)(m + 32) * ld + n];
      const float x2 = X[(size_t)(m + 64) * ld + n], x3 = X[(size_t)(m + 96) * ld + n];
      if (w) {
        s0 = fmaf(x0, w[(size_t)m * ldw], s0); s1 = fmaf(x1, w[(size_t)(m + 32) * ldw], s1);
        s2 = fmaf(x2, w[(size_t)(m + 64) * ldw], s2); s3 = fmaf(x3, w[(size_t)(m + 96) * ldw], s3);
      } else {
        s0 += x0; s1 += x1; s2 += x2; s3 += x3;
      }
    }
    for (; m < M; m += 32) s0 += X[(size_t)m * ld + n] * (w ? w[(size_t)m * ldw] : 1.f);
  }
  red[wid][lane] = (s0 + s1) + (s2 + s3);
  __syncthreads();
  if (wid == 0 && n < N) {
    float t = 0.f;
#pragma unroll
    for (int k = 0; k < 32; ++k) t += red[k][lane];
    out[n] = t;
  }
}

__global__ void __launch_bounds__(512)
colsum_slab_kernel(int M, int N, int rps, const float* __restrict__ X, float* __restrict__ part) {
  __shared__ float4 red[512];
  const int t = threadIdx.x;
  const size_t r0 = (size_t)blockIdx.x * rps;
  const size_t r1 = r0 + rps < (size_t)M ? r0 + rps : (size_t)M;
  const float4* x4 = reinterpret_cast<const float4*>(X);
  const size_t e4 = r1 * N / 4;
  size_t j = r0 * N / 4 + t;
  float4 a0 = make_float4(0.f, 0.f, 0.f, 0.f), a1 = a0, a2 = a0, a3 = a0;
  for (; j + 3 * 512 < e4; j += 4 * 512) {
    const float4 v0 = __ldcs(x4 + j), v1 = __ldcs(x4 + j + 512), v2 = __ldcs(x4 + j + 1024), v3 = __ldcs(x4 + j + 1536);
    a0.x += v0.x; a0.y += v0.y; a0.z += v0.z; a0.w += v0.w;
    a1.x += v1.x; a1.y += v1.y; a1.z += v1.z; a1.w += v1.w;
    a2.x += v2.x; a2.y += v2.y; a2.z += v2.z; a2.w += v2.w;
    a3.x += v3.x; a3.y += v3.y; a3.z += v3.z; a3.w += v3.w;
  }
  for (; j < e4; j += 512) {
    const float4 v0 = __ldcs(x4 + j);
    a0.x += v0.x; a0.y += v0.y; a0.z += v0.z; a0.w += v0.w;
  }
  red[t] = make_float4((a0.x + a1.x) + (a2.x + a3.x), (a0.y + a1.y) + (a2.y + a3.y),
                       (a0.z + a1.z) + (a2.z + a3.z), (a0.w + a1.w) + (a2.w + a3.w));
  __syncthreads();
  const int G = N >> 2;
  if (t < G) {
    float4 s = red[t];
    for (int k = t + G; k < 512; k += G) {
      const float4 v = red[k];
      s.x += v.x; s.y += v.y; s.z += v.z; s.w += v.w;
    }
    reinterpret_cast<float4*>(part + (size_t)blockIdx.x * N)[t] = s;
  }
}

int colsum(int M, int N, const float* X, int ld, float* out, cudaStream_t st, float* ws, size_t ws_bytes) {
  const bool pow2 = N >= 4 && N <= 2048 && (N & (N - 1)) == 0;
  if (ws && pow2 && ld == N && (size_t)M * N >= ((size_t)1 << 20) && (reinterpret_cast<uintptr_t>(X) & 15) == 0) {
    const int sweep = 2048 / N;
    int rps = ceil_div(ceil_div(M, 4 * kNumSMs), sweep) * sweep;
    if (rps < 8 * sweep) rps = 8 * sweep;
    const int S = ceil_div(M, rps);
    if ((size_t)S * N * sizeof(float) <= ws_bytes && S > 1) {
      colsum_slab_kernel<<<S, 512, 0, st>>>(M, N, rps, X, ws);
      count_launch(PC_GEMM, st);
      SEEDRL_CHECK_LAUNCH();
      colsum_kernel<<<ceil_div(N, 32), 1024, 0, st>>>(S, N, ws, N, nullptr, 0, out);
      count_launch(PC_GEMM, st);
      SEEDRL_CHECK_LAUNCH();
      return SEEDRL_OK;
    }
  }
  colsum_kernel<<<ceil_div(N, 32), 1024, 0, st>>>(M, N, X, ld, nullptr, 0, out);
  count_launch(PC_GEMM, st);
  SEEDRL_CHECK_LAUNCH();
  return SEEDRL_OK;
}

__global__ void fill_kernel(size_t n, float* p, float v) {
  const size_t i = (size_t)blockIdx.x * blockDim.x + threadIdx.x;
  if (i < n) p[i] = v;
}
int fill(size_t n, float* p, float v, cudaStream_t st) {
  if (n == 0) return SEEDRL_OK;
  fill_kernel<<<(unsigned)ceil_div_sz(n, 256), 256, 0, st>>>(n, p, v);
  count_launch(PC_MISC, st);
  SEEDRL_CHECK_LAUNCH();
  return SEEDRL_OK;
}

__global__ void copy_col_kernel(int n, const float* __restrict__ src, int ld, int col,
                                float* __restrict__ dst) {
  const int i = blockIdx.x * blockDim.x + threadIdx.x;
  if (i < n) dst[i] = src[(size_t)i * ld + col];
}

}
```

seed_rl_b200/csrc/gemm_tc_kernels.cu:

```cuda
#include "kernels.h"
#include "tc_common.cuh"

namespace seedrl {

constexpr int kGtThreads = 256;
constexpr int kGtBM = 128;
constexpr int kGtMaxBN = 128;
constexpr int kGtBK = 32;

struct GemmTcParams {
  int M, N, K;
  const float* A; int lda;
  const float* B; int ldb;
  float* C; int ldc;
  float* ws;
  int BN;
  int kblocks_per_split;
  int vecA, vecB;
  GemmEpi e;
  int* error_flag;
  ConvGather cg;
};

struct RawUnit { float4 a, b; };
// ... 62 lines not shown
    case 48: Wgmma<48>::mma<TA, TB>(acc, a, b, 1u); break;
    case 64: Wgmma<64>::mma<TA, TB>(acc, a, b, 1u); break;
    case 80: Wgmma<80>::mma<TA, TB>(acc, a, b, 1u); break;
    case 96: Wgmma<96>::mma<TA, TB>(acc, a, b, 1u); break;
    case 112: Wgmma<112>::mma<TA, TB>(acc, a, b, 1u); break;
    default: Wgmma<128>::mma<TA, TB>(acc, a, b, 1u); break;
  }
}

template <bool TA, bool TB, bool SPLIT, bool GATHER>
__global__ void __launch_bounds__(kGtThreads)
gemm_tc_kernel(const GemmTcParams p) {
  constexpr int S = SPLIT ? 2 : 1;
  constexpr int KG = kGtBK / 8;
  extern __shared__ __align__(128) uint8_t smem_raw[];
  const int BN = p.BN;
  constexpr uint32_t a_ps = TA ? (kGtBK + 1) : (kGtBM + 1);
  constexpr uint32_t a_units = TA ? (kGtBM / 8) * a_ps : (kGtBK / 8) * a_ps;
  const uint32_t b_ps = TB ? (uint32_t)BN + 1 : (uint32_t)kGtBK + 1;
  const uint32_t b_units = TB ? (kGtBK / 8) * b_ps : (uint32_t)(BN / 8) * b_ps;
  const int b_items = BN * kGtBK / 8;
  const uint32_t stage_units = S * (a_units + b_units);
  uint4* s_buf = reinterpret_cast<uint4*>(smem_raw);
  const int tid = threadIdx.x, wg = tid >> 7;
  const int m0 = blockIdx.y * kGtBM, n0 = blockIdx.x * BN;
  const int kb0 = blockIdx.z * p.kblocks_per_split;
  const int nkb_total = (p.K + kGtBK - 1) / kGtBK;
  const int nkb = min(p.kblocks_per_split, nkb_total - kb0);
  const uint32_t a_wg = TA ? (uint32_t)wg * 8u * a_ps * 16u : (uint32_t)wg * 64u * 16u;
  float acc[kGtMaxBN / 2];
#pragma unroll
  for (int i = 0; i < kGtMaxBN / 2; ++i) acc[i] = 0.f;
  wgmma_fence_acc<kGtMaxBN / 2>(acc);

  for (int kb = 0; kb < nkb; ++kb) {
    const int st = kb & 1;
    const int k0 = (kb0 + kb) * kGtBK;
    uint4* sA = s_buf + (size_t)st * stage_units;
    uint4* sB = sA + (size_t)S * a_units;
    constexpr int AI = (kGtBM * kGtBK / 8) / kGtThreads;
    constexpr int BI = (kGtMaxBN * kGtBK / 8) / kGtThreads;
    RawUnit ra[AI], rb[BI];
#pragma unroll
    for (int r = 0; r < AI; ++r) {
      const int u = tid + r * kGtThreads;
      if (GATHER) {
        if (!TA) ra[r] = load_gather(p.cg, m0 + u / KG, k0 + (u % KG) * 8, p.M, p.K);
        else     ra[r] = load_gather(p.cg, k0 + (u >> 4), m0 + (u & 15) * 8, p.K, p.M);
      } else {
        if (!TA) ra[r] = load_raw(p.A, p.lda, m0 + u / KG, k0 + (u % KG) * 8, p.M, p.K, p.vecA != 0);
        else     ra[r] = load_raw(p.A, p.lda, k0 + (u >> 4), m0 + (u & 15) * 8, p.K, p.M, p.vecA != 0);
      }
    }
    const int bng = BN >> 3;
#pragma unroll
    for (int r = 0; r < BI; ++r) {
      const int u = tid + r * kGtThreads;
      if (u < b_items) {
        if (TB) rb[r] = load_raw(p.B, p.ldb, n0 + u / KG, k0 + (u % KG) * 8, p.N, p.K, p.vecB != 0);
        else    rb[r] = load_raw(p.B, p.ldb, k0 + u / bng, n0 + (u % bng) * 8, p.K, p.N, p.vecB != 0);
      }
    }
    if (kb >= 2) wgmma_wait<1>();
    __syncthreads();
#pragma unroll
    for (int r = 0; r < AI; ++r) {
// ... 40 lines not shown
    for (int j = 0; j < kGtMaxBN / 8; ++j) {
      if (8 * j < BN) {
#pragma unroll
        for (int h = 0; h < 2; ++h)
          *reinterpret_cast<float2*>(tile + (size_t)(r0 + 8 * h) * ld + 8 * j + c0) =
              make_float2(acc[4 * j + 2 * h], acc[4 * j + 2 * h + 1]);
      }
    }
    __syncthreads();
    const bool partial = p.ws != nullptr;
    for (int i = tid; i < kGtBM * BN; i += kGtThreads) {
      const int r = i / BN, c = i - r * BN;
      const int gm = m0 + r, gn = n0 + c;
      if (gm < p.M && gn < p.N) {
        float x = tile[(size_t)r * ld + c];
        if (partial) {
          p.ws[((size_t)blockIdx.z * p.M + gm) * p.N + gn] = x;
        } else {
          if (p.e.bias) x += __ldg(p.e.bias + gn);
          if (p.e.relu) x = fmaxf(x, 0.f);
          if (p.e.mask) x = __ldg(p.e.mask + (size_t)gm * p.e.ldm + gn) > 0.f ? x : 0.f;
          float* cp = p.C + (size_t)gm * p.ldc + gn;
          *cp = p.e.accumulate ? *cp + x : x;
        }
      }
    }
  }
}

template <bool VEC>
__global__ void gemm_tc_reduce_kernel(int M, int N, int splits, const float* __restrict__ ws,
                                      float* __restrict__ C, int ldc, GemmEpi e) {
  constexpr int W = VEC ? 4 : 1;
  const int i = (blockIdx.x * blockDim.x + threadIdx.x) * W;
  if (i >= M * N) return;
  const int m = i / N, n = i - m * N;
  float x[W];
#pragma unroll
  for (int j = 0; j < W; ++j) x[j] = 0.f;
  const size_t plane = (size_t)M * N;
#pragma unroll 4
  for (int z = 0; z < splits; ++z) {
    if (VEC) {
      const float4 v = __ldcs(reinterpret_cast<const float4*>(ws + (size_t)z * plane + i));
      x[0] += v.x; x[W > 1 ? 1 : 0] += v.y; x[W > 2 ? 2 : 0] += v.z; x[W > 3 ? 3 : 0] += v.w;
    } else {
      x[0] += __ldcs(ws + (size_t)z * plane + i);
    }
  }
#pragma unroll
  for (int j = 0; j < W; ++j) {
    float v = x[j];
    if (e.bias) v += __ldg(e.bias + n + j);
    if (e.relu) v = fmaxf(v, 0.f);
    if (e.mask) v = __ldg(e.mask + (size_t)m * e.ldm + n + j) > 0.f ? v : 0.f;
    float* c = C + (size_t)m * ldc + n + j;
    *c = e.accumulate ? *c + v : v;
  }
}

__global__ void __launch_bounds__(256)
gemm_tc_reduce_wide_kernel(int M, int N, int splits, const float* __restrict__ ws, float* __restrict__ C, int ldc,
                           GemmEpi e) {
  __shared__ float4 part[8][32];
  const int o = threadIdx.x & 31, zl = threadIdx.x >> 5;
  const int i = (blockIdx.x * 32 + o) * 4;
  const bool in = i < M * N;
  const size_t plane = (size_t)M * N;
  float4 a = make_float4(0.f, 0.f, 0.f, 0.f), b = a;
  if (in) {
    int z = zl;
    for (; z + 8 < splits; z += 16) {
      const float4 v = __ldcs(reinterpret_cast<const float4*>(ws + (size_t)z * plane + i));
      const float4 w = __ldcs(reinterpret_cast<const float4*>(ws + (size_t)(z + 8) * plane + i));
      a.x += v.x; a.y += v.y; a.z += v.z; a.w += v.w;
      b.x += w.x; b.y += w.y; b.z += w.z; b.w += w.w;
    }
    if (z < splits) {
      const float4 v = __ldcs(reinterpret_cast<const float4*>(ws + (size_t)z * plane + i));
      a.x += v.x; a.y += v.y; a.z += v.z; a.w += v.w;
    }
  }
  part[zl][o] = make_float4(a.x + b.x, a.y + b.y, a.z + b.z, a.w + b.w);
  __syncthreads();
  if (zl != 0 || !in) return;
  float x[4] = {0.f, 0.f, 0.f, 0.f};
#pragma unroll
  for (int k = 0; k < 8; ++k) {
    const float4 v = part[k][o];
    x[0] += v.x; x[1] += v.y; x[2] += v.z; x[3] += v.w;
  }
  const int m = i / N, n = i - m * N;
#pragma unroll
  for (int j = 0; j < 4; ++j) {
    float v = x[j];
    if (e.bias) v += __ldg(e.bias + n + j);
    if (e.relu) v = fmaxf(v, 0.f);
// ... 34 lines not shown
  if (cg) p.cg = *cg; else p.cg = ConvGather{};
  p.M = M; p.N = N; p.K = K; p.A = A; p.lda = lda; p.B = B; p.ldb = ldb; p.C = C; p.ldc = ldc;
  p.e = e; p.error_flag = err;
  const int n16 = ((N + 15) / 16) * 16;
  int bn = kGtMaxBN;
  if (bn > n16) bn = n16;
  const int nkb_all = ceil_div(K, kGtBK);
  const int kb256 = 256 / kGtBK;
  while (bn > 64 && ceil_div(M, kGtBM) * ceil_div(N, bn) * (nkb_all >= kb256 ? nkb_all / (kb256 / 2) : 1) < kNumSMs)
    bn >>= 1;
  p.BN = ((bn + 15) / 16) * 16;
  auto al16 = [](const void* q) { return (reinterpret_cast<uintptr_t>(q) & 15) == 0; };
  p.vecA = al16(A) && (lda & 3) == 0;
  p.vecB = al16(B) && (ldb & 3) == 0;
  const int tiles = ceil_div(M, kGtBM) * ceil_div(N, p.BN);
  const int nkb = ceil_div(K, kGtBK);
  int splits = 1;
  while (tiles * splits < kNumSMs && nkb / (splits * 2) >= 128 / kGtBK &&
         (size_t)(splits * 2) * M * N * sizeof(float) <= ws_bytes && ws)
    splits *= 2;
  p.kblocks_per_split = ceil_div(nkb, splits);
  splits = ceil_div(nkb, p.kblocks_per_split);
  p.ws = splits > 1 ? ws : nullptr;
  const int S = split ? 2 : 1;
  const size_t a_un = ta ? (size_t)(kGtBM / 8) * (kGtBK + 1) : (size_t)(kGtBK / 8) * (kGtBM + 1);
  const size_t b_un = tb ? (size_t)(kGtBK / 8) * (p.BN + 1) : (size_t)(p.BN / 8) * (kGtBK + 1);
  size_t smem = (size_t)2 * S * (a_un + b_un) * 16;
  const size_t epi = (size_t)kGtBM * (p.BN + 4) * 4;
  if (smem < epi) smem = epi;
  dim3 grid(ceil_div(N, p.BN), ceil_div(M, kGtBM), splits);
#define SEEDRL_GT_LAUNCH2(TA_, TB_, SP_, G_)                                                    \
  do {                                                                                          \
    SEEDRL_CUDA(allow_smem<gemm_tc_kernel<TA_, TB_, SP_, G_>>(200 * 1024));                     \
    gemm_tc_kernel<TA_, TB_, SP_, G_><<<grid, kGtThreads, smem, st>>>(p);                       \
  } while (0)
#define SEEDRL_GT_LAUNCH(TA_, TB_, SP_)                                                         \
  do {                                                                                          \
    if (cg && !(TB_)) SEEDRL_GT_LAUNCH2(TA_, false, SP_, true);                                 \
    else SEEDRL_GT_LAUNCH2(TA_, TB_, SP_, false);                                               \
  } while (0)
  if (split) {
    if (!ta && !tb) SEEDRL_GT_LAUNCH(false, false, true);
    else if (ta && !tb) SEEDRL_GT_LAUNCH(true, false, true);
    else if (!ta && tb) SEEDRL_GT_LAUNCH(false, true, true);
    else SEEDRL_GT_LAUNCH(true, true, true);
  } else {
    if (!ta && !tb) SEEDRL_GT_LAUNCH(false, false, false);
    else if (ta && !tb) SEEDRL_GT_LAUNCH(true, false, false);
    else if (!ta && tb) SEEDRL_GT_LAUNCH(false, true, false);
    else SEEDRL_GT_LAUNCH(true, true, false);
  }
#undef SEEDRL_GT_LAUNCH
#undef SEEDRL_GT_LAUNCH2
  count_launch(PC_GEMM, st);
  SEEDRL_CHECK_LAUNCH();
  if (splits > 1) {
    if ((N & 3) == 0 && splits >= 16)
      gemm_tc_reduce_wide_kernel<<<ceil_div(M * N / 4, 32), 256, 0, st>>>(M, N, splits, ws, C, ldc, e);
    else if ((N & 3) == 0)
      gemm_tc_reduce_kernel<true><<<ceil_div(M * N / 4, 256), 256, 0, st>>>(M, N, splits, ws, C, ldc, e);
    else
      gemm_tc_reduce_kernel<false><<<ceil_div(M * N, 256), 256, 0, st>>>(M, N, splits, ws, C, ldc, e);
    count_launch(PC_GEMM, st);
    SEEDRL_CHECK_LAUNCH();
  }
  return SEEDRL_OK;
}

}
```

seed_rl_b200/csrc/kernels.h:

```cpp
#pragma once
#include "common.cuh"

namespace seedrl {

enum { IN_F32 = 0, IN_RELU = 1, IN_U8 = 2 };

struct ConvGeom {
  int N, H, W;
  int PW;
  int RH;
  long long Q;
  unsigned int pw_mul, rh_mul;
  int pw_sh, rh_sh;
};

__host__ __device__ inline void fast_div_setup(unsigned int d, unsigned int* mul, int* sh) {
  int l = 1;
  while ((1u << l) < d) ++l;
  *mul = (unsigned int)(((1ULL << (31 + l)) + d - 1) / d);
  *sh = l - 1;
}
__host__ __device__ __forceinline__ unsigned int fast_div(unsigned int n, unsigned int mul, int sh) {
#ifdef __CUDA_ARCH__
  return __umulhi(n, mul) >> sh;
// ... 34 lines not shown
struct ReduceJob { const float* partial; float* dw; float* db; int nparts, nw, nb; };
struct ReduceTable { ReduceJob jobs[kMaxReduceJobs]; };
struct WgradBatch { float* buf; size_t cap_floats, used; int n; ReduceJob jobs[kMaxReduceJobs]; };

bool conv3x3_tc_supported(int cin, int cout, int in_mode);
int conv3x3_tc_pack_weights(int cin, int cout, int flip, int split, const float* w, void* wq,
                            cudaStream_t st);
bool conv3x3_wgrad_tc_supported(int cin, int cout, int in_mode);
void conv3x3_wgrad_tc_set_chunk(int kc);
int conv3x3_wgrad_tc(int cin, int cout, int in_mode, int split, int N, int H, int W, const void* x,
                     const float* dy, float* dw, float* db, float* partial, size_t partial_bytes,
                     int* err, WgradBatch* batch, cudaStream_t st);
int wgrad_reduce_batch(WgradBatch* b, cudaStream_t st);
int conv3x3_tc_pack_weights_batch(const PackTable& t, int split, cudaStream_t st);
void conv3x3_tc_set_tile(int mt);
int conv3x3_tc_forward(int cin, int cout, int in_mode, int split, int N, int H, int W, const void* in,
                       const void* wq, const float* bias, const float* mask, const float* res,
                       float* out, int* err, cudaStream_t st);

constexpr int kPlanesTryNext = -12347;
long long planes_positions(int N, int H, int W);
size_t planes_bytes(int N, int H, int W, int C);
struct PlaneConv {
  int N, H, W;
  const void* in;
  const void* wq;
  const float* bias;
  const void* mask;
  const void* res;
  void* out_raw;
  void* out_relu;
  float* out_nhwc;
  int* err;
};
bool convp_supported(int cin, int cout);
int convp_forward(int cin, int cout, const PlaneConv& c, cudaStream_t st);
int wgradp(int cin, int cout, int N, int H, int W, const void* x, const void* dy, float* dw, float* db,
           int* err, WgradBatch* batch, cudaStream_t st);
int to_planes(int N, int H, int W, int C, int relu, const float* x, void* out, cudaStream_t st);
int from_planes(int N, int H, int W, int C, const void* in, float* y, cudaStream_t st);
int poolp_forward(int N, int H, int W, int C, const float* x, void* out_raw, void* out_relu, uint8_t* idx,
                  cudaStream_t st);
int poolp_backward(int N, int H, int W, int C, const void* dy, const uint8_t* idx, void* dx_planes,
                   float* dx_nhwc, cudaStream_t st);

bool first_wgrad_pooled_supported(int cin, int cout, int H, int W);
int first_wgrad_pooled(int N, int H, int W, int C, const uint8_t* frames, const void* g_planes, const uint8_t* idx,
                       float* dw, float* db, WgradBatch* batch, cudaStream_t st);
bool conv0pool_supported(int cin, int cout, int H, int W);
int conv0pool_forward(int N, int H, int W, int C, const uint8_t* frames, const float* w, const float* bias,
                      void* praw, void* prelu, uint8_t* idx, int* err, cudaStream_t st);

int conv3x3_forward(int cin, int cout, int in_mode, int N, int H, int W, const void* in,
                    const float* w, const float* bias, const float* mask, const float* res,
                    float* out, cudaStream_t st);
int conv3x3_u8_forward(int C, int N, int H, int W, const uint8_t* frames, const float* w, const float* bias,
                       float* out, cudaStream_t st);
int conv3x3_u8_wgrad(int C, int N, int H, int W, const uint8_t* frames, const float* dy, float* dw, float* db,
                     float* partial, size_t partial_bytes, cudaStream_t st);
int conv3x3_flip_weights(int cin, int cout, const float* w, float* wt, cudaStream_t st);
size_t conv3x3_wgrad_partial_bytes();
int wgrad_reduce(int nparts, int nw, int nb, const float* partial, float* dw, float* db,
                 cudaStream_t st);
int conv3x3_wgrad(int cin, int cout, int in_mode, int N, int H, int W, const void* x,
                  const float* dy, float* dw, float* db, float* partial, size_t partial_bytes,
                  cudaStream_t st);
inline void same_pad3s2(int in, int* out, int* before) {
  *out = (in + 1) / 2;
  const int total = (*out - 1) * 2 + 3 - in;
  *before = total > 0 ? total / 2 : 0;
}
int maxpool3s2_forward(int N, int H, int W, int C, const float* x, float* y, uint8_t* idx,
                       cudaStream_t st);
int maxpool3s2_backward(int N, int H, int W, int C, const float* dy, const uint8_t* idx, float* dx,
                        cudaStream_t st);

int convgen_forward(int N, int H, int W, int cin, int cout, int k, int stride, int in_u8,
                    const void* in, const float* w, const float* bias, int relu, float* out,
                    cudaStream_t st);
int convgen_dgrad(int N, int H, int W, int cin, int cout, int k, int stride, const float* dy,
                  const float* w, const float* mask, float* dx, cudaStream_t st);
int convgen_wgrad(int N, int H, int W, int cin, int cout, int k, int stride, int in_u8,
                  const void* x, const float* dy, float* dw, float* db, float* partial,
                  size_t partial_bytes, cudaStream_t st);
// ... 49 lines not shown
```

seed_rl_b200/csrc/lstm.cu:

```cuda
#include "schedule.h"

namespace seedrl {

int lstm_recurrence_forward(int mode, int H, int T1, int B, const float* U, const uint8_t* done, float* z,
                            const float* h0, const float* c0, float* hs, float* cs, float* hp, unsigned int* counter,
                            int* err, cudaStream_t st) {
  if (mode == 2) return lstm_forward_tiled(H, T1, B, U, done, z, h0, c0, hs, cs, hp, counter, err, st);
  if (mode == 3) return lstm_forward_tc(H, T1, B, U, done, z, h0, c0, hs, cs, hp, counter, err, st);
  return set_error(SEEDRL_ERR_INVALID_ARGUMENT, "lstm mode must be 2 (tiled) or 3 (tc3)");
}

int lstm_recurrence_backward(int mode, int H, int T1, int B, const float* U, const uint8_t* done, const float* gates,
                             const float* cs, const float* c0, const float* dhs, float* dz, unsigned int* counter,
                             int* err, cudaStream_t st) {
  if (mode == 2) return lstm_backward_tiled(H, T1, B, U, done, gates, cs, c0, dhs, dz, counter, err, st);
  if (mode == 3) return lstm_backward_tc(H, T1, B, U, done, gates, cs, c0, dhs, dz, counter, err, st);
  return set_error(SEEDRL_ERR_INVALID_ARGUMENT, "lstm mode must be 2 (tiled) or 3 (tc3)");
}

Core core_create(ParamTable& t, const std::string& dense, int H, int flat, int A, bool clip_reward, bool flat_relu) {
  Core k;
  k.H = H; k.flat = flat; k.A = A; k.core_in = H + 1 + A;
  k.clip_reward = clip_reward; k.flat_relu = flat_relu;
  k.dense_w = t.add(dense + "/kernel", {flat, H});
  k.dense_b = t.add(dense + "/bias", {H});
  k.w = t.add("core/kernel", {k.core_in, 4 * H});
  k.u = t.add("core/recurrent_kernel", {H, 4 * H});
  k.b = t.add("core/bias", {4 * H});
  return k;
}

CorePlan core_plan(const Core& k, Bump& b, int T1, int B) {
  CorePlan p;
  p.T1 = T1; p.B = B; p.N = T1 * B;
  const size_t N = (size_t)p.N, H = (size_t)k.H;
  p.xc = b.take(N * k.core_in * 4);
  p.z = b.take(N * 4 * H * 4);
  p.hp = b.take(N * H * 4);
  p.cs = b.take(N * H * 4);
  p.hs = b.take(N * H * 4);
  p.c0buf = b.take((size_t)B * H * 4);
  p.dhs = b.take(N * H * 4);
  p.dz = b.take(N * 4 * H * 4);
  p.dd = b.take(N * H * 4);
  p.counter = b.take(256);
  return p;
}

__global__ void core_input_tail_kernel(int Nrows, int D, int A, bool clip, const float* __restrict__ reward,
                                       const int64_t* __restrict__ prev_action, float* __restrict__ core_in) {
  const int i = blockIdx.x * blockDim.x + threadIdx.x;
  const int Wd = 1 + A;
  if (i >= Nrows * Wd) return;
  const int n = i / Wd, j = i - n * Wd;
  float v;
  if (j == 0) v = clip ? fminf(fmaxf(reward[n], -1.f), 1.f) : reward[n];
  else v = prev_action[n] == (int64_t)(j - 1) ? 1.f : 0.f;
  core_in[(size_t)n * (D + Wd) + D + j] = v;
}

int core_forward(const Core& k, const ParamTable& t, const CorePlan& p, const GemmExec& ex, void* ws, const float* prm,
                 const float* flat, const float* reward, const int64_t* prev_actions, const uint8_t* done,
                 const float* h0, const float* c0) {
  cudaStream_t st = ex.st;
  const int N = p.N, H = k.H, CI = k.core_in;
  float* xc = W<float>(ws, p.xc);
  float* z = W<float>(ws, p.z);
  float* c0buf = W<float>(ws, p.c0buf);
  GemmEpi e = epi_none();
  e.bias = prm + t.offset(k.dense_b); e.relu = 1; e.a_relu = k.flat_relu;
  SEEDRL_TRY(ex.gemm(false, false, N, H, k.flat, flat, k.flat, prm + t.offset(k.dense_w), H, xc, CI, e));
  core_input_tail_kernel<<<ceil_div(N * (1 + k.A), 256), 256, 0, st>>>(N, H, k.A, k.clip_reward, reward,
                                                                       prev_actions, xc);
  count_launch(PC_MISC, st);
  SEEDRL_CHECK_LAUNCH();
  e = epi_none();
  e.bias = prm + t.offset(k.b);
  SEEDRL_TRY(ex.gemm(false, false, N, 4 * H, CI, xc, CI, prm + t.offset(k.w), 4 * H, z, 4 * H, e));
  SEEDRL_CUDA(cudaMemcpyAsync(c0buf, c0, (size_t)p.B * H * 4, cudaMemcpyDeviceToDevice, st));
  return lstm_recurrence_forward(k.lstm_mode, H, p.T1, p.B, prm + t.offset(k.u), done, z, h0, c0buf,
                                 W<float>(ws, p.hs), W<float>(ws, p.cs), W<float>(ws, p.hp),
                                 W<unsigned int>(ws, p.counter), ex.err, st);
}

int core_final_state(const Core& k, const CorePlan& p, cudaStream_t st, void* ws, float* h_out, float* c_out) {
  const size_t last = (size_t)(p.T1 - 1) * p.B * k.H, bytes = (size_t)p.B * k.H * 4;
  if (h_out)
    SEEDRL_CUDA(cudaMemcpyAsync(h_out, W<float>(ws, p.hs) + last, bytes, cudaMemcpyDeviceToDevice, st));
  if (c_out)
    SEEDRL_CUDA(cudaMemcpyAsync(c_out, W<float>(ws, p.cs) + last, bytes, cudaMemcpyDeviceToDevice, st));
  return SEEDRL_OK;
}

int core_backward(const Core& k, const ParamTable& t, const CorePlan& p, const GemmExec& ex, void* ws,
                  const float* prm, float* grd, const uint8_t* done, const float* flat, float* dflat,
                  cudaEvent_t head_ready) {
  const int N = p.N, H = k.H, CI = k.core_in;
  const float* xc = W<float>(ws, p.xc);
  float* dz = W<float>(ws, p.dz);
  float* dd = W<float>(ws, p.dd);
  const GemmEpi e = epi_none();
  SEEDRL_TRY(lstm_recurrence_backward(k.lstm_mode, H, p.T1, p.B, prm + t.offset(k.u), done, W<float>(ws, p.z),
                                      W<float>(ws, p.cs), W<float>(ws, p.c0buf), W<float>(ws, p.dhs), dz,
                                      W<unsigned int>(ws, p.counter), ex.err, ex.st));
  SEEDRL_TRY(ex.gemm(true, false, H, 4 * H, N, W<float>(ws, p.hp), H, dz, 4 * H, grd + t.offset(k.u), 4 * H, e));
  SEEDRL_TRY(ex.gemm(true, false, CI, 4 * H, N, xc, CI, dz, 4 * H, grd + t.offset(k.w), 4 * H, e));
  SEEDRL_TRY(ex.colsum(N, 4 * H, dz, 4 * H, grd + t.offset(k.b)));
// ... 48 lines not shown
```

seed_rl_b200/csrc/net.cu:

```cuda
#include "schedule.h"

namespace seedrl {

constexpr int kHidden = 256;

struct ConvLayer {
  int cin, cout;
  int w, b;
};
struct Stack {
  int hin, win, cin, c, hout, wout;
  ConvLayer conv, r00, r01, r10, r11;
};

}

struct seedrl_net {
  seedrl_net_config cfg;
  seedrl::ParamTable params;
  size_t logical_params;
  int p_base_w, p_base_b, p_pol_w, p_pol_b;
  seedrl::Core core;
  std::vector<seedrl::Stack> stacks;
  seedrl::StridedConv sh[2];
// ... 185 lines not shown
  wp[i] = ci < 3 ? w[(tap * 3 + ci) * cout + co] : 0.f;
}
__global__ void unpad_dw0_kernel(int cout, const float* __restrict__ dwp, float* __restrict__ dw) {
  const int i = blockIdx.x * blockDim.x + threadIdx.x;
  if (i >= 9 * 3 * cout) return;
  const int co = i % cout, ci = (i / cout) % 3, tap = i / (3 * cout);
  dw[i] = dwp[(tap * 4 + ci) * cout + co];
}

static int pack_all_weights(Call& c, int flip) {
  const seedrl_net* n = c.n;
  c.packed.n = 0;
  if (n->conv_mode < 1 || n->cfg.net != SEEDRL_NET_DEEP) return SEEDRL_OK;
  char* base = W<char>(c.ws, c.pl.wq_all);
  for (size_t s = 0; s < n->stacks.size(); ++s) {
    const Stack& k = n->stacks[s];
    const ConvLayer* ls[5] = {&k.conv, &k.r00, &k.r01, &k.r10, &k.r11};
    for (int i = 0; i < 5; ++i) {
      const ConvLayer& l = *ls[i];
      const bool first = s == 0 && i == 0;
      if (first && (flip || c.first != kFirstStaged)) continue;
      const int cin = flip ? l.cout : l.cin, cout = flip ? l.cin : l.cout;
      if (c.packed.n >= kMaxPackJobs) return SEEDRL_OK;
      PackJob j;
      j.w = c.P(l.w);
      j.wq = base + (size_t)c.packed.n * kPackSlotBytes;
      j.ck = cin < 16 ? 16 : cin; j.cout = cout; j.cin_src = cin; j.flip = flip;
      j.legacy = first;
      c.packed.jobs[c.packed.n++] = j;
    }
  }
  return conv3x3_tc_pack_weights_batch(c.packed, n->conv_mode == 3 ? 2 : (n->conv_mode >= 2 ? 1 : 0), c.ex.st);
}
static int packed_weights(const Call& c, int cin, int cout, const float* w, int flip, int split, const void** wq) {
  for (int i = 0; i < c.packed.n; ++i)
    if (c.packed.jobs[i].w == w && c.packed.jobs[i].flip == flip) {
      *wq = c.packed.jobs[i].wq;
      return SEEDRL_OK;
    }
  void* scratch = W<void>(c.ws, c.pl.wq);
  SEEDRL_TRY(conv3x3_tc_pack_weights(cin, cout, flip, split, w, scratch, c.ex.st));
  *wq = scratch;
  return SEEDRL_OK;
}

static int run_conv(const Call& c, const ConvLayer& l, int H, int Wd, int in_mode, const Act& in, const Act* res,
                    const Act& out, int flip = 0, const Act* mask = nullptr) {
  cudaStream_t st = c.ex.st;
  const int N = c.pl.N, cin = flip ? l.cout : l.cin, cout = flip ? l.cin : l.cout;
  const float* w = c.P(l.w);
  const float* bias = flip ? nullptr : c.P(l.b);
  const void* x = c.at(in_mode == IN_RELU ? in.relu : in.raw);
  const float* m = mask ? c.at<float>(mask->relu) : nullptr;
  const float* r = res ? c.at<float>(res->raw) : nullptr;
  const void* wq;
  if (in.planes) {
    SEEDRL_TRY(packed_weights(c, cin, cout, w, flip, 2, &wq));
    PlaneConv pc;
    pc.N = N; pc.H = H; pc.W = Wd; pc.in = x; pc.wq = wq; pc.bias = bias; pc.mask = m; pc.res = r;
    pc.out_raw = out.planes ? c.at(out.raw) : nullptr; pc.out_relu = out.planes ? c.at(out.relu) : nullptr;
    pc.out_nhwc = out.planes ? nullptr : c.at<float>(out.raw); pc.err = c.ex.err;
    return convp_forward(cin, cout, pc, st);
  }
  if (c.n->conv_mode >= 1 && conv3x3_tc_supported(cin, cout, in_mode)) {
    const int split = c.n->conv_mode >= 2;
    SEEDRL_TRY(packed_weights(c, cin, cout, w, flip, split, &wq));
    return conv3x3_tc_forward(cin, cout, in_mode, split, N, H, Wd, x, wq, bias, m, r, c.at<float>(out.raw),
                              c.ex.err, st);
  }
  if (flip) {
    float* wt = W<float>(c.ws, c.pl.wt);
    SEEDRL_TRY(conv3x3_flip_weights(cout, cin, w, wt, st));
    w = wt;
  }
  return conv3x3_forward(cin, cout, in_mode, N, H, Wd, x, w, bias, m, r, c.at<float>(out.raw), st);
}

static int conv_bwd(Call& c, const ConvLayer& l, int H, int Wd, int x_mode, const Act& x, const Act& dy,
                    const Act* dres, const Act& dx) {
  const seedrl_net* n = c.n; const Plan& pl = c.pl; cudaStream_t st = c.ex.st;
  const void* xin = c.at(x_mode == IN_RELU ? x.relu : x.raw);
  if (x.planes) {
    SEEDRL_TRY(wgradp(l.cin, l.cout, pl.N, H, Wd, xin, c.at(dy.raw), c.G(l.w), c.G(l.b), c.ex.err, &c.wb, st));
  } else if (n->conv_mode >= 1 && conv3x3_wgrad_tc_supported(l.cin, l.cout, x_mode)) {
    SEEDRL_TRY(conv3x3_wgrad_tc(l.cin, l.cout, x_mode, n->conv_mode >= 2, pl.N, H, Wd, xin, c.at<float>(dy.raw),
                                c.G(l.w), c.G(l.b), W<float>(c.ws, pl.partial), conv3x3_wgrad_partial_bytes(),
                                c.ex.err, &c.wb, st));
  } else {
    SEEDRL_TRY(conv3x3_wgrad(l.cin, l.cout, x_mode, pl.N, H, Wd, xin, c.at<float>(dy.raw), c.G(l.w), c.G(l.b),
                             W<float>(c.ws, pl.partial), conv3x3_wgrad_partial_bytes(), st));
  }
  g_conv_cat = PC_CONV_DGRAD;
  const int rc = run_conv(c, l, H, Wd, IN_F32, dy, dres, dx, 1, x_mode == IN_RELU ? &x : nullptr);
  g_conv_cat = PC_CONV_FWD;
// ... 18 lines not shown
  const Act& g = c.pl.g[0];
  if (!g.planes) return SEEDRL_OK;
  const Stack& k = c.n->stacks.back();
  return to_planes(c.pl.N, k.hout, k.wout, k.c, 0, W<float>(c.ws, c.pl.gA), c.at(g.raw), c.ex.st);
}

static int pad_first_layer(Call& c, const uint8_t** obs) {
  const seedrl_net* n = c.n;
  if (n->cfg.net != SEEDRL_NET_DEEP || n->cfg.obs_c != 3) return SEEDRL_OK;
  const Plan& pl = c.pl;
  cudaStream_t st = c.ex.st;
  const size_t npix = (size_t)pl.N * n->cfg.obs_h * n->cfg.obs_w;
  pad_frames3_kernel<<<(unsigned)((npix + 255) / 256), 256, 0, st>>>(npix, *obs, W<uchar4>(c.ws, pl.obs4));
  count_launch(PC_MISC, st);
  const int wi = n->stacks[0].conv.w;
  pad_w0_kernel<<<ceil_div(9 * 4 * 16, 128), 128, 0, st>>>(16, c.prm + n->params.offset(wi), W<float>(c.ws, pl.w0pad));
  count_launch(PC_MISC, st);
  if (cudaGetLastError() != cudaSuccess) return set_error(SEEDRL_ERR_INTERNAL, "3-channel padding launch failed");
  *obs = W<uint8_t>(c.ws, pl.obs4);
  c.w0_index = wi; c.w0_pad = W<float>(c.ws, pl.w0pad); c.dw0_pad = W<float>(c.ws, pl.dw0pad);
  return SEEDRL_OK;
}

static int first_forward(const Call& c, const uint8_t* obs) {
  const seedrl_net* n = c.n; cudaStream_t st = c.ex.st;
  const Stack& k = n->stacks[0];
  const StackBufs& b = c.pl.st[0];
  const int N = c.pl.N, split = n->conv_mode >= 2;
  const float *w = c.P(k.conv.w), *bias = c.P(k.conv.b);
  float* a0 = c.at<float>(b.a0.raw);
  const void* wq;
  if (c.first == kFirstFused)
    return conv0pool_forward(N, k.hin, k.win, first_c(n), obs, w, bias, c.at(b.p.raw), c.at(b.p.relu),
                             c.at<uint8_t>(b.idx), c.ex.err, st);
  if (c.first == kFirstStaged) {
    SEEDRL_TRY(packed_weights(c, k.cin, k.c, w, 0, split, &wq));
    SEEDRL_TRY(conv3x3_tc_forward(k.cin, k.c, IN_U8, split, N, k.hin, k.win, obs, wq, bias, nullptr, nullptr, a0,
                                  c.ex.err, st));
  } else {
    SEEDRL_TRY(conv3x3_u8_forward(first_c(n), N, k.hin, k.win, obs, w, bias, a0, st));
  }
  return pool_forward(c, k, b);
}

static int first_backward(Call& c, const uint8_t* obs) {
  const seedrl_net* n = c.n; const Plan& pl = c.pl; cudaStream_t st = c.ex.st;
  const Stack& k = n->stacks[0];
  const int N = pl.N;
  float *dw = c.G(k.conv.w), *db = c.G(k.conv.b);
  if (c.first == kFirstFused)
    return first_wgrad_pooled(N, k.hin, k.win, first_c(n), obs, c.at(pl.g[0].raw), c.at<uint8_t>(pl.st[0].idx), dw,
                              db, &c.wb, st);
  SEEDRL_TRY(pool_backward(c, k, pl.st[0].idx, pl.g[0], f32_act(pl.gFull)));
  const float* gF = W<float>(c.ws, pl.gFull);
  float* partial = W<float>(c.ws, pl.partial);
  const size_t pbytes = conv3x3_wgrad_partial_bytes();
  if (c.first == kFirstStaged)
    return conv3x3_wgrad_tc(k.cin, k.c, IN_U8, n->conv_mode >= 2, N, k.hin, k.win, obs, gF, dw, db, partial, pbytes,
                            c.ex.err, &c.wb, st);
  return conv3x3_u8_wgrad(first_c(n), N, k.hin, k.win, obs, gF, dw, db, partial, pbytes, st);
}

}

using namespace seedrl;

extern "C" int seedrl_net_create(const seedrl_net_config* cfg, seedrl_net** out) {
// ... 475 lines not shown
```

seed_rl_b200/csrc/optim_kernels.cu:

```cuda
#include "common.cuh"

namespace seedrl {

__global__ void __launch_bounds__(256)
adam_kernel(size_t n, float* __restrict__ p, const float* __restrict__ g, float* __restrict__ m,
            float* __restrict__ v, float lr_t, float b1, float b2, float eps, float gscale,
            long long clamp_index, float clamp_lo, float clamp_hi) {
  const size_t n4 = n >> 2;
  const size_t stride = (size_t)gridDim.x * blockDim.x;
  const size_t tid = (size_t)blockIdx.x * blockDim.x + threadIdx.x;
  const float ob1 = 1.0f - b1, ob2 = 1.0f - b2;
  float4* p4 = reinterpret_cast<float4*>(p);
  const float4* g4 = reinterpret_cast<const float4*>(g);
  float4* m4 = reinterpret_cast<float4*>(m);
  float4* v4 = reinterpret_cast<float4*>(v);
  for (size_t i = tid; i < n4; i += stride) {
    float4 pp = p4[i], gg = g4[i], mm = m4[i], vv = v4[i];
#define SEEDRL_ADAM1(c)                                   \
    {                                                     \
      const float gs = gg.c * gscale;                     \
      mm.c += (gs - mm.c) * ob1;                          \
      vv.c += (gs * gs - vv.c) * ob2;                     \
      pp.c -= (mm.c * lr_t) / (sqrtf(vv.c) + eps);        \
    }
    SEEDRL_ADAM1(x) SEEDRL_ADAM1(y) SEEDRL_ADAM1(z) SEEDRL_ADAM1(w)
#undef SEEDRL_ADAM1
    p4[i] = pp; m4[i] = mm; v4[i] = vv;
  }
  for (size_t i = (n4 << 2) + tid; i < n; i += stride) {
    const float gs = g[i] * gscale;
    const float mm = m[i] + (gs - m[i]) * ob1;
    const float vv = v[i] + (gs * gs - v[i]) * ob2;
    m[i] = mm; v[i] = vv;
    p[i] -= (mm * lr_t) / (sqrtf(vv) + eps);
  }
  (void)clamp_index; (void)clamp_lo; (void)clamp_hi;
}

__global__ void clamp_one_kernel(float* p, long long idx, float lo, float hi) {
  p[idx] = fminf(fmaxf(p[idx], lo), hi);
}

}

using namespace seedrl;

extern "C" int seedrl_adam_apply(size_t n, float* params, const float* grads, float* m, float* v,
                                 float lr_t, float beta1, float beta2, float eps,
                                 float grad_scale, int64_t clamp_index, float clamp_lo,
                                 float clamp_hi, seedrl_stream_t stream) {
  if (n == 0) return SEEDRL_OK;
  SEEDRL_CHECK_ARG(params && grads && m && v, "null pointer");
  SEEDRL_CHECK_ARG(((uintptr_t)params % 16 == 0) && ((uintptr_t)grads % 16 == 0) &&
                       ((uintptr_t)m % 16 == 0) && ((uintptr_t)v % 16 == 0),
                   "arena pointers must be 16-byte aligned");
  SEEDRL_CHECK_ARG(clamp_index < (int64_t)n, "clamp_index out of range");
  const size_t n4 = n >> 2;
  int blocks = (int)ceil_div_sz(n4 > 0 ? n4 : 1, 256);
  const int max_blocks = kNumSMs * 8;
  if (blocks > max_blocks) blocks = max_blocks;
  adam_kernel<<<blocks, 256, 0, (cudaStream_t)stream>>>(n, params, grads, m, v, lr_t, beta1,
                                                         beta2, eps, grad_scale,
                                                         (long long)clamp_index, clamp_lo,
                                                         clamp_hi);
  count_launch(PC_ADAM, (cudaStream_t)stream);
  SEEDRL_CHECK_LAUNCH();
  if (clamp_index >= 0) {
    clamp_one_kernel<<<1, 1, 0, (cudaStream_t)stream>>>(params, (long long)clamp_index, clamp_lo,
                                                         clamp_hi);
    count_launch(PC_ADAM, (cudaStream_t)stream);
    SEEDRL_CHECK_LAUNCH();
  }
  return SEEDRL_OK;
}
```

seed_rl_b200/csrc/vtrace_kernels.cu:

```cuda
#include <cuda.h>
#include <math.h>

#include <algorithm>
#include <type_traits>

#include "common.cuh"

namespace seedrl {

template <int CH>
__global__ void __launch_bounds__(128)
vtrace_kernel(int T, int B, const float* __restrict__ tlp, const float* __restrict__ blp,
              const float* __restrict__ disc, const float* __restrict__ rew,
              const float* __restrict__ val, const float* __restrict__ boot,
              float clip_rho, float clip_pg, float lambda_, int has_clip_rho,
              int has_clip_pg, float* __restrict__ vs, float* __restrict__ pg) {
  const int b = blockIdx.x * blockDim.x + threadIdx.x;
  if (b >= B) return;
  float acc = 0.f;
  const float bootv = boot[b];
  float vs_next = bootv, v_next = bootv;
  int t_hi = T;
  while (t_hi > 0) {
    const int t_lo = t_hi - CH > 0 ? t_hi - CH : 0;
// ... 576 lines not shown
  }
  __syncthreads();
  tile_copy<false>(s_logits, p.dlogits + (size_t)b0 * A, T, B, A, BB, nb, tid);
  {
    float* dst = p.dlogits + ((size_t)T * B + b0) * A;
    for (int e = tid; e < nb * A; e += kLossThreads) dst[e] = 0.f;
  }
  for (int i = tid; i < (T + 1) * BB; i += kLossThreads) {
    const int t = i / BB, c = i - t * BB;
    if (c < nb) {
      if (POPART && t < T) {
        p.pop_td[(size_t)t * B + b0 + c] = s_blp[i];
      } else {
        p.dbaseline[(size_t)t * B + b0 + c] = t < T ? -p.cfg.baseline_cost * s_blp[i] * invN : 0.f;
      }
    }
  }

  double r;
  double* part = p.partials + (size_t)blockIdx.x * kLossPartials;
  r = block_reduce_sum_d(sum_tp);  if (tid == 0) part[0] = r;
  r = block_reduce_sum_d(sum_ve2); if (tid == 0) part[1] = r;
  r = block_reduce_sum_d(sum_h);   if (tid == 0) part[2] = r;
  r = block_reduce_sum_d(sum_kl);  if (tid == 0) part[3] = r;
  r = block_reduce_sum_d(sum_v);   if (tid == 0) part[4] = r;
  r = block_reduce_max(max_a, s_red);   if (tid == 0) part[5] = r;
  if (POPART) {
    r = block_reduce_sum_d(sum_vs);  if (tid == 0) part[6] = r;
    r = block_reduce_sum_d(sum_vs2); if (tid == 0) part[7] = r;
  }
  loss_finalize<POPART>(p, s_red, ec);
}

__global__ void __launch_bounds__(kLossThreads) vtrace_loss_kernel(const LossParams p) { loss_small_body<false>(p); }
__global__ void __launch_bounds__(kLossThreads) vtrace_popart_loss_kernel(const LossParams p) {
  loss_small_body<true>(p);
}


constexpr int kStreamThreadsMax = 1024;
constexpr size_t kStreamSmemMax = 227 * 1024 - 2048;
constexpr int kStreamRounds = 4;

__device__ __forceinline__ uint32_t sm_u32(const void* p) {
  return (uint32_t)__cvta_generic_to_shared(p);
}
__device__ __forceinline__ void mbar_wait_or_trap(uint64_t* bar, uint32_t parity) {
  uint32_t done = 0;
  int spins = 0;
  while (!done) {
    asm volatile(
        "{\n\t.reg .pred p;\n\t"
        "mbarrier.try_wait.parity.shared::cta.b64 p, [%1], %2;\n\t"
        "selp.u32 %0, 1, 0, p;\n\t}\n"
        : "=r"(done)
        : "r"(sm_u32(bar)), "r"(parity)
        : "memory");
    if (!done && ++spins > (1 << 24)) __trap();
  }
}

struct SmallRegs {
  float rew[kStreamRounds], val[kStreamRounds];
  int act[kStreamRounds];
  uint8_t done[kStreamRounds];
};

template <int AS, bool POPART>
// ... 232 lines not shown
                   : "memory");
      asm volatile("cp.async.bulk.commit_group;" ::: "memory");
    }
    {
      float* dz = p.dlogits + ((size_t)T * B + (size_t)tile * BB) * A;
      for (int e = tid; e < BB * A; e += nthreads) dz[e] = 0.f;
      if (tid < BB) p.dbaseline[(size_t)T * B + (size_t)tile * BB + tid] = 0.f;
    }
    if (has_next) store_small(sm);
    __syncthreads();
  }
  if (tid == 0) asm volatile("cp.async.bulk.wait_group.read 0;" ::: "memory");

  double r;
  double* part = p.partials + (size_t)blockIdx.x * kLossPartials;
  r = block_reduce_sum_d(sum_tp);  if (tid == 0) part[0] = r;
  r = block_reduce_sum_d(sum_ve2); if (tid == 0) part[1] = r;
  r = block_reduce_sum_d(sum_h);   if (tid == 0) part[2] = r;
  r = block_reduce_sum_d(sum_kl);  if (tid == 0) part[3] = r;
  r = block_reduce_sum_d(sum_v);   if (tid == 0) part[4] = r;
  r = block_reduce_max(max_a, s_red);   if (tid == 0) part[5] = r;
  if (POPART) {
    r = block_reduce_sum_d(sum_vs);  if (tid == 0) part[6] = r;
    r = block_reduce_sum_d(sum_vs2); if (tid == 0) part[7] = r;
  }
  loss_finalize<POPART>(p, s_red, ec);
}

template <int AS>
__global__ void __launch_bounds__(kStreamThreadsMax)
vtrace_loss_stream_kernel(const LossParams p, const int ntiles, const int tile_stride_f,
                          const __grid_constant__ CUtensorMap tm_bl, const __grid_constant__ CUtensorMap tm_ll,
                          const __grid_constant__ CUtensorMap tm_dl) {
  loss_stream_body<AS, false>(p, ntiles, tile_stride_f, tm_bl, tm_ll, tm_dl);
}
template <int AS>
__global__ void __launch_bounds__(kStreamThreadsMax)
vtrace_popart_loss_stream_kernel(const LossParams p, const int ntiles, const int tile_stride_f,
                                 const __grid_constant__ CUtensorMap tm_bl, const __grid_constant__ CUtensorMap tm_ll,
                                 const __grid_constant__ CUtensorMap tm_dl) {
  loss_stream_body<AS, true>(p, ntiles, tile_stride_f, tm_bl, tm_ll, tm_dl);
}

constexpr int kPopThreads = 512;
constexpr int kPopPartials = 4;

struct PopArtUpdateParams {
  int T, B;
  float baseline_cost, beta;
  double count;
  const float* lb;
  const float* td;
  const float* sums;
  float* mom;
  float* comp;
  float* dbaseline;
  float* dcomp;
  float* loss_terms;
  double* partials;
  unsigned int* ticket;
};

__global__ void __launch_bounds__(kPopThreads)
vtrace_popart_update_kernel(const PopArtUpdateParams p) {
  __shared__ bool s_last;
  const int tid = threadIdx.x;
  const float mu1 = p.mom[0], mu2 = p.mom[1], sigma = p.comp[0], mu = p.comp[1];
  const float bm1 = (float)((double)p.sums[0] / p.count), bm2 = (float)((double)p.sums[1] / p.count);
  const float mu1n = __fadd_rn(mu1, __fmul_rn(p.beta, __fsub_rn(bm1, mu1)));
  const float mu2n = __fadd_rn(mu2, __fmul_rn(p.beta, __fsub_rn(bm2, mu2)));
  const float s = popart_std(mu1, mu2), sn = popart_std(mu1n, mu2n);
  const float sigma_n = __fmul_rn(__fdiv_rn(s, sn), sigma);
  const float mu_n = __fdiv_rn(__fadd_rn(__fsub_rn(mu1, mu1n), __fmul_rn(s, mu)), sn);

  const size_t n = (size_t)p.T * p.B;
  const float invN = 1.0f / ((float)p.T * (float)p.B);
  double se2 = 0.0, sev = 0.0, se = 0.0;
  for (size_t i = (size_t)blockIdx.x * kPopThreads + tid; i < n; i += (size_t)gridDim.x * kPopThreads) {
    const float V = __ldg(p.lb + i);
    const float e = __ldg(p.td + i) + (fmaf(sigma, V, mu) - fmaf(sigma_n, V, mu_n));
    p.dbaseline[i] = (-p.baseline_cost * e * invN) * sigma_n;
    se2 += (double)e * e;
    sev += (double)e * V;
    se += e;
  }
  double r;
  double* part = p.partials + (size_t)blockIdx.x * kPopPartials;
  r = block_reduce_sum_d(se2); if (tid == 0) part[0] = r;
  r = block_reduce_sum_d(sev); if (tid == 0) part[1] = r;
  r = block_reduce_sum_d(se);  if (tid == 0) part[2] = r;
  if (tid == 0) {
    __threadfence();
    s_last = atomicAdd(p.ticket, 1u) == gridDim.x - 1;
  }
  __syncthreads();
  if (!s_last) return;
  __threadfence();
  double a[3] = {0.0, 0.0, 0.0};
// ... 77 lines not shown
  for (int pass = 0; pass < 2; ++pass)
  for (int BB = 16; BB >= 2; BB >>= 1) {
    if (forced_bb > 1 && BB != forced_bb) continue;
    if (B % BB != 0 || ((BB * A) & 3) != 0 || BB * A > 256) continue;
    if (B / BB < num_sms()) continue;
    const size_t bytes = stream_smem_bytes(T, A, BB);
    if (bytes > kStreamSmemMax) continue;
    if (pass == 0 && forced_bb <= 1 && 2 * (bytes + 2048 + 1024) > (size_t)228 * 1024) continue;
    const int rows = T * BB;
    const int rounds = ceil_div(rows, kStreamThreadsMax);
    int th = ceil_div(ceil_div(rows, rounds), 32) * 32;
    if (th < 128) th = 128;
    if ((T + 1) * BB > kStreamRounds * th) continue;
    *threads = th;
    *smem_bytes = bytes;
    return BB;
  }
  return 0;
}

template <int AS, bool POPART>
static cudaError_t launch_stream(const LossParams& p, int ntiles, int threads, size_t smem, cudaStream_t stream,
                                 const CUtensorMap& tm_bl, const CUtensorMap& tm_ll, const CUtensorMap& tm_dl) {
  auto kernel = POPART ? vtrace_popart_loss_stream_kernel<AS> : vtrace_loss_stream_kernel<AS>;
  const cudaError_t e = POPART ? allow_smem<vtrace_popart_loss_stream_kernel<AS>>((int)kStreamSmemMax)
                               : allow_smem<vtrace_loss_stream_kernel<AS>>((int)kStreamSmemMax);
  if (e != cudaSuccess) return e;
  int per_sm = (int)((size_t)(228 * 1024) / (smem + 2048 + 1024));
  if (per_sm > 2048 / threads) per_sm = 2048 / threads;
  if (per_sm > 6) per_sm = 6;
  if (per_sm < 1) per_sm = 1;
  int grid = num_sms() * per_sm;
  if (grid > ntiles) grid = ntiles;
  kernel<<<grid, threads, smem, stream>>>(
      p, ntiles, stream_tile_stride_f(p.T, p.A, p.BB), tm_bl, tm_ll, tm_dl);
  return cudaSuccess;
}

}

using namespace seedrl;

static int g_loss_stream_enabled = 1;

extern "C" int seedrl_debug_set_loss_stream(int enabled) {
  g_loss_stream_enabled = enabled < 0 ? 0 : enabled;
  return SEEDRL_OK;
}

extern "C" int seedrl_vtrace_from_importance_weights(
    int T, int B, const float* tlp, const float* blp, const float* disc, const float* rew,
    const float* val, const float* boot, float clip_rho, float clip_pg, float lambda_,
    float* vs, float* pg, seedrl_stream_t stream) {
  SEEDRL_CHECK_ARG(T >= 0 && B >= 0, "T and B must be non-negative");
  if (T == 0 || B == 0) return SEEDRL_OK;
  SEEDRL_CHECK_ARG(tlp && blp && disc && rew && val && boot && vs && pg, "null pointer");
  const int threads = 128;
  vtrace_kernel<5><<<ceil_div(B, threads), threads, 0, (cudaStream_t)stream>>>(
      T, B, tlp, blp, disc, rew, val, boot, clip_rho, clip_pg, lambda_, !isnan(clip_rho),
      !isnan(clip_pg), vs, pg);
  count_launch(PC_VTRACE, (cudaStream_t)stream);
  SEEDRL_CHECK_LAUNCH();
  return SEEDRL_OK;
}

extern "C" int seedrl_categorical_log_prob(int N, int A, const float* logits,
                                           const int64_t* actions, float* log_prob,
                                           seedrl_stream_t stream) {
  SEEDRL_CHECK_ARG(N >= 0 && A > 0, "bad N/A");
// ... 48 lines not shown
  SEEDRL_CHECK_LAUNCH();
  return SEEDRL_OK;
}

extern "C" size_t seedrl_vtrace_loss_scratch_bytes(int T1, int B, int A) {
  (void)T1; (void)A;
  return 256 + (size_t)(B > kNumSMs ? B : kNumSMs) * kLossPartials * sizeof(double);
}

template <bool POPART>
static int launch_loss(LossParams p, cudaStream_t st) {
  const int T1 = p.T + 1, B = p.B, A = p.A;
  size_t smem = 0;
  auto small_kernel = POPART ? vtrace_popart_loss_kernel : vtrace_loss_kernel;
  SEEDRL_CUDA(POPART ? allow_smem<vtrace_popart_loss_kernel>(200 * 1024) : allow_smem<vtrace_loss_kernel>(200 * 1024));
  int threads = 0;
  p.BB = g_loss_stream_enabled ? pick_stream(p, g_loss_stream_enabled, &threads, &smem) : 0;
  alignas(64) CUtensorMap tm_bl, tm_ll, tm_dl;
  if (p.BB > 0 && !(make_tile_map(&tm_bl, p.bl, T1, p.T, B, A, p.BB) &&
                    make_tile_map(&tm_ll, p.ll, T1, p.T, B, A, p.BB) &&
                    make_tile_map(&tm_dl, p.dlogits, T1, p.T, B, A, p.BB)))
    p.BB = 0;
  if (p.BB > 0) {
    const int ntiles = B / p.BB;
    switch (A) {
      case 9:  SEEDRL_CUDA((launch_stream<9, POPART>(p, ntiles, threads, smem, st, tm_bl, tm_ll, tm_dl))); break;
      case 18: SEEDRL_CUDA((launch_stream<18, POPART>(p, ntiles, threads, smem, st, tm_bl, tm_ll, tm_dl))); break;
      case 19: SEEDRL_CUDA((launch_stream<19, POPART>(p, ntiles, threads, smem, st, tm_bl, tm_ll, tm_dl))); break;
      default: SEEDRL_CUDA((launch_stream<0, POPART>(p, ntiles, threads, smem, st, tm_bl, tm_ll, tm_dl))); break;
    }
  } else {
    p.BB = pick_bb(p.T, B, A, &smem);
    SEEDRL_CHECK_ARG(p.BB > 0, "unroll_length * num_actions too large for shared memory");
    small_kernel<<<ceil_div(B, p.BB), kLossThreads, smem, st>>>(p);
  }
  count_launch(PC_LOSS, st);
  SEEDRL_CHECK_LAUNCH();
  return SEEDRL_OK;
}

static LossParams loss_params(int T1, int B, int A, const float* learner_logits, const float* learner_baseline,
                              const float* behaviour_logits, const int64_t* actions, const float* rewards,
                              const uint8_t* done, const seedrl_loss_config* cfg, const float* entropy_cost_param,
                              float* loss_terms, float* dlogits, float* dbaseline, float* d_entropy_cost_param,
                              float* vs_out, float* pg_advantages_out, void* scratch) {
  LossParams p = {};
  p.T = T1 - 1; p.B = B; p.A = A;
  p.AP = A | 1;
  p.ll = learner_logits; p.lb = learner_baseline; p.bl = behaviour_logits;
  p.act = actions; p.rew = rewards; p.done = done; p.cfg = *cfg; p.ecp = entropy_cost_param;
  p.loss_terms = loss_terms; p.dlogits = dlogits; p.dbaseline = dbaseline;
  p.d_ecp = d_entropy_cost_param; p.vs_out = vs_out; p.pg_out = pg_advantages_out;
  p.ticket = reinterpret_cast<unsigned int*>(scratch);
  p.partials = reinterpret_cast<double*>(reinterpret_cast<char*>(scratch) + 256);
  return p;
}

extern "C" int seedrl_vtrace_loss_fwd_bwd(
    int T1, int B, int A, const float* learner_logits, const float* learner_baseline,
    const float* behaviour_logits, const int64_t* actions, const float* rewards,
    const uint8_t* done, const seedrl_loss_config* cfg, const float* entropy_cost_param,
    float* loss_terms, float* dlogits, float* dbaseline, float* d_entropy_cost_param,
    float* vs_out, float* pg_advantages_out, void* scratch, seedrl_stream_t stream) {
  SEEDRL_CHECK_ARG(T1 >= 2 && B >= 1 && A >= 1, "need T1>=2, B>=1, A>=1");
  SEEDRL_CHECK_ARG(learner_logits && learner_baseline && behaviour_logits && actions &&
                       rewards && done && cfg && entropy_cost_param && loss_terms &&
                       dlogits && dbaseline && d_entropy_cost_param && scratch,
                   "null pointer");
  return launch_loss<false>(
// ... 16 lines not shown
                       rewards && done && cfg && entropy_cost_param && popart_moments &&
                       popart_compensation && loss_terms && dlogits && dbaseline &&
                       d_entropy_cost_param && td_out && moment_sums && scratch,
                   "null pointer");
  LossParams p = loss_params(T1, B, A, learner_logits, learner_baseline, behaviour_logits, actions, rewards, done,
                             cfg, entropy_cost_param, loss_terms, dlogits, dbaseline, d_entropy_cost_param,
                             vs_out, pg_advantages_out, scratch);
  p.pop_mom = popart_moments; p.pop_comp = popart_compensation;
  p.pop_td = td_out; p.pop_sums = moment_sums;
  return launch_loss<true>(p, (cudaStream_t)stream);
}

extern "C" int seedrl_vtrace_popart_update(
    int T1, int B, int world, float beta, float baseline_cost, const float* learner_baseline,
    const float* td, const float* moment_sums, float* popart_moments, float* popart_compensation,
    float* dbaseline, float* d_popart_compensation, float* loss_terms, void* scratch,
    seedrl_stream_t stream) {
  SEEDRL_CHECK_ARG(T1 >= 2 && B >= 1 && world >= 1, "need T1>=2, B>=1, world>=1");
  SEEDRL_CHECK_ARG(beta >= 0.f && beta <= 1.f, "beta must be in [0, 1]");
  SEEDRL_CHECK_ARG(learner_baseline && td && moment_sums && popart_moments && popart_compensation &&
                       dbaseline && d_popart_compensation && loss_terms && scratch,
                   "null pointer");
  PopArtUpdateParams p;
  p.T = T1 - 1; p.B = B;
  p.baseline_cost = baseline_cost; p.beta = beta;
  p.count = (double)world * (double)p.T * (double)B;
  p.lb = learner_baseline; p.td = td; p.sums = moment_sums;
  p.mom = popart_moments; p.comp = popart_compensation;
  p.dbaseline = dbaseline; p.dcomp = d_popart_compensation; p.loss_terms = loss_terms;
  p.ticket = reinterpret_cast<unsigned int*>(scratch);
  p.partials = reinterpret_cast<double*>(reinterpret_cast<char*>(scratch) + 256);
  const size_t n = (size_t)p.T * B;
  const int grid = (int)std::min<size_t>(ceil_div_sz(n, (size_t)kPopThreads * 4), (size_t)kNumSMs);
  vtrace_popart_update_kernel<<<grid, kPopThreads, 0, (cudaStream_t)stream>>>(p);
  count_launch(PC_LOSS, (cudaStream_t)stream);
  SEEDRL_CHECK_LAUNCH();
  return SEEDRL_OK;
}
```

Baseline: 197,200.

## Enable programmatic dependent launch across learner kernels to overlap launch latency

Adds a launch_kernel helper that launches through cudaLaunchKernelEx with the programmatic stream serialization attribute, and inserts griddepcontrol.wait/launch_dependents into most learner kernels (convs, pooling, plane conversion, GEMM helpers, loss, Adam). Each kernel's prologue (smem setup, barrier init, TMA descriptor prefetch) can then overlap with the tail of the previous kernel, hiding launch gaps in a pipeline of many small kernels. Risks include extra residency pressure from early-launched grids, and correctness hinges on every kernel waiting before it reads its predecessor's output. A runtime toggle and a PDL launch counter are added for debugging.

Result: faster. 200,500 (median of 6 runs) (+1.7%).

```diff
diff --git a/include/seedrl_b200.h b/include/seedrl_b200.h
--- a/include/seedrl_b200.h
+++ b/include/seedrl_b200.h
@@ -20,6 +20,7 @@
 const char* seedrl_last_error(void);
 int seedrl_abi_version(void);
 uint64_t seedrl_kernel_launch_count(void);
+uint64_t seedrl_pdl_launch_count(void);
 
 int seedrl_vtrace_from_importance_weights(
     int T, int B,
@@ -257,6 +258,7 @@
 int seedrl_debug_set_wgrad_chunk(int kc);
 int seedrl_debug_set_conv_tile(int mt);
 int seedrl_debug_set_gemm_gather(int on);
+int seedrl_debug_set_pdl(int on);
 int seedrl_debug_set_first_layer_dense(int on);
 int seedrl_debug_conv0pool(int N, int H, int W, const uint8_t* frames, const float* w, const float* bias,
                            void* praw, void* prelu, uint8_t* idx, int* err, seedrl_stream_t stream);
diff --git a/seed_rl_b200/_lib.py b/seed_rl_b200/_lib.py
--- a/seed_rl_b200/_lib.py
+++ b/seed_rl_b200/_lib.py
@@ -61,6 +61,7 @@
     'seedrl_last_error': (ctypes.c_char_p, []),
     'seedrl_abi_version': (c_int, []),
     'seedrl_kernel_launch_count': (c_u64, []),
+    'seedrl_pdl_launch_count': (c_u64, []),
     'seedrl_vtrace_from_importance_weights':
         (c_int, [c_int, c_int, P, P, P, P, P, P, c_float, c_float, c_float, P, P, P]),
     'seedrl_categorical_log_prob': (c_int, [c_int, c_int, P, P, P, P]),
@@ -178,6 +179,7 @@
         (c_int, [c_int, c_int, c_int, c_int, c_int, c_int, P, c_int, P, c_int, P, c_int, P, P, c_int, c_int, c_int,
                  c_int, P, c_size_t, P, P]),
     'seedrl_debug_set_gemm_gather': (c_int, [c_int]),
+    'seedrl_debug_set_pdl': (c_int, [c_int]),
     'seedrl_debug_colsum': (c_int, [c_int, c_int, P, c_int, P, P, c_size_t, P]),
     'seedrl_debug_sgemm':
         (c_int, [c_int, c_int, c_int, c_int, c_int, P, c_int, P, c_int, P, c_int, P, P, c_int,
@@ -226,6 +228,10 @@
   return int(lib().seedrl_kernel_launch_count())
 
 
+def pdl_launch_count():
+  return int(lib().seedrl_pdl_launch_count())
+
+
 def ptr(t):
   return None if t is None else ctypes.c_void_p(t.data_ptr())
 
diff --git a/seed_rl_b200/csrc/capi.cu b/seed_rl_b200/csrc/capi.cu
--- a/seed_rl_b200/csrc/capi.cu
+++ b/seed_rl_b200/csrc/capi.cu
@@ -5,6 +5,8 @@
 namespace seedrl {
 thread_local std::string g_last_error;
 std::atomic<uint64_t> g_launch_count{0};
+std::atomic<int> g_pdl_on{1};
+std::atomic<uint64_t> g_pdl_launch_count{0};
 bool g_prof_on = false;
 int g_conv_cat = PC_CONV_FWD;
 
@@ -29,6 +31,14 @@
 extern "C" int seedrl_abi_version(void) { return 1; }
 extern "C" uint64_t seedrl_kernel_launch_count(void) {
   return seedrl::g_launch_count.load(std::memory_order_relaxed);
+}
+
+extern "C" uint64_t seedrl_pdl_launch_count(void) {
+  return seedrl::g_pdl_launch_count.load(std::memory_order_relaxed);
+}
+extern "C" int seedrl_debug_set_pdl(int on) {
+  seedrl::g_pdl_on.store(on ? 1 : 0, std::memory_order_relaxed);
+  return SEEDRL_OK;
 }
 
 extern "C" int seedrl_profile_num_categories(void) { return seedrl::PC_COUNT; }
diff --git a/seed_rl_b200/csrc/common.cuh b/seed_rl_b200/csrc/common.cuh
--- a/seed_rl_b200/csrc/common.cuh
+++ b/seed_rl_b200/csrc/common.cuh
@@ -6,6 +6,7 @@
 
 #include <atomic>
 #include <string>
+#include <utility>
 
 #include "../../include/seedrl_b200.h"
 
@@ -61,6 +62,28 @@
   if (g_prof_on) prof_mark_(cat, st);
 }
 
+extern std::atomic<int> g_pdl_on;
+extern std::atomic<uint64_t> g_pdl_launch_count;
+
+__device__ __forceinline__ void pdl_wait() { asm volatile("griddepcontrol.wait;" ::: "memory"); }
+__device__ __forceinline__ void pdl_trigger() { asm volatile("griddepcontrol.launch_dependents;" ::: "memory"); }
+
+template <typename... P, typename... A>
+cudaError_t launch_kernel(bool pdl, int cat, void (*k)(P...), dim3 grid, dim3 block, size_t smem, cudaStream_t st,
+                          A&&... args) {
+  cudaLaunchAttribute attr[1];
+  attr[0].id = cudaLaunchAttributeProgrammaticStreamSerialization;
+  attr[0].val.programmaticStreamSerializationAllowed = 1;
+  cudaLaunchConfig_t cfg = {};
+  cfg.gridDim = grid; cfg.blockDim = block; cfg.dynamicSmemBytes = smem; cfg.stream = st;
+  cfg.attrs = attr;
+  cfg.numAttrs = pdl && g_pdl_on.load(std::memory_order_relaxed) ? 1 : 0;
+  const cudaError_t e = cudaLaunchKernelEx(&cfg, k, std::forward<A>(args)...);
+  if (e == cudaSuccess && cfg.numAttrs) g_pdl_launch_count.fetch_add(1, std::memory_order_relaxed);
+  count_launch(cat, st);
+  return e;
+}
+
 constexpr int kNumSMs = 132;
 
 template <auto K>
diff --git a/seed_rl_b200/csrc/conv_first.cu b/seed_rl_b200/csrc/conv_first.cu
--- a/seed_rl_b200/csrc/conv_first.cu
+++ b/seed_rl_b200/csrc/conv_first.cu
@@ -54,6 +54,8 @@
 #pragma unroll
   for (int i = 0; i < 36; ++i) acc[i] = 0.f;
   float accb = 0.f;
+  pdl_wait();
+  pdl_trigger();
   const int bands = (a.Ho + RB - 1) / RB;
   const int units = a.N * bands;
   for (int u = blockIdx.x; u < units; u += gridDim.x) {
@@ -151,7 +153,7 @@
 template <int CP, bool kU32>
 static int launch_first_wgrad(const FirstWgradArgs& a, int grid, size_t smem, cudaStream_t st) {
   SEEDRL_CUDA(allow_smem<first_wgrad_pooled_kernel<CP, kU32>>(72 * 1024));
-  first_wgrad_pooled_kernel<CP, kU32><<<grid, kFwThreads, smem, st>>>(a);
+  launch_kernel(true, PC_CONV_WGRAD, first_wgrad_pooled_kernel<CP, kU32>, grid, kFwThreads, smem, st, a);
   return SEEDRL_OK;
 }
 
@@ -185,7 +187,6 @@
                  : cp == 8 ? launch_first_wgrad<8, false>(a, grid, smem, st)
                            : launch_first_wgrad<16, false>(a, grid, smem, st);
   if (rc != SEEDRL_OK) return rc;
-  count_launch(PC_CONV_WGRAD, st);
   SEEDRL_CHECK_LAUNCH();
   batch->jobs[batch->n++] = ReduceJob{a.partial, dw, db, grid, 9 * C * kFwCo, kFwCo};
   return SEEDRL_OK;
@@ -261,6 +262,8 @@
   }
   asm volatile("fence.proxy.async.shared::cta;" ::: "memory");
   __syncthreads();
+  pdl_wait();
+  pdl_trigger();
   const uint32_t a_base = smem_u32(s_p), b_base = smem_u32(s_bq);
 
   const int bands = (a.Ho + kCpRows - 1) / kCpRows;
@@ -450,7 +453,7 @@
 }
 
 template <int CP, bool TMA>
-static int launch_conv0pool(Conv0PoolArgs a, const uint8_t* frames, cudaStream_t st) {
+static int launch_conv0pool(Conv0PoolArgs a, const uint8_t* frames, cudaStream_t st, bool pdl) {
   constexpr int KT = 3 * (CP == 16 ? 48 : 4 * CP);
   const int N = a.N, H = a.H, W = a.W;
   const size_t raw_stride = TMA ? (((size_t)(2 * kCpRows + 3) * W * 4) + 127) / 128 * 128 : 0;
@@ -475,14 +478,13 @@
   }
   const int units = N * ((a.Ho + kCpRows - 1) / kCpRows);
   const int grid = units < 2 * kNumSMs ? units : 2 * kNumSMs;
-  conv0pool_kernel<CP, TMA><<<grid, kCpThreadsF, smem, st>>>(tm, a);
-  count_launch(PC_CONV_FWD, st);
+  launch_kernel(pdl, PC_CONV_FWD, conv0pool_kernel<CP, TMA>, grid, kCpThreadsF, smem, st, tm, a);
   SEEDRL_CHECK_LAUNCH();
   return SEEDRL_OK;
 }
 
 int conv0pool_forward(int N, int H, int W, int C, const uint8_t* frames, const float* w, const float* bias,
-                      void* praw, void* prelu, uint8_t* idx, int* err, cudaStream_t st) {
+                      void* praw, void* prelu, uint8_t* idx, int* err, cudaStream_t st, bool pdl) {
   if (!conv0pool_supported(C, 16, H, W))
     return set_error(SEEDRL_ERR_INVALID_ARGUMENT, "conv0pool: unsupported frame shape");
   Conv0PoolArgs a;
@@ -493,10 +495,11 @@
   fast_div_setup((unsigned int)(W + 2), &a.sw_mul, &a.sw_sh);
   a.frames = frames; a.w = w; a.bias = bias;
   a.praw = reinterpret_cast<uint4*>(praw); a.prelu = reinterpret_cast<uint4*>(prelu); a.idx = idx; a.err = err;
-  if (C == 4) return launch_conv0pool<4, true>(a, frames, st);
+  if (C == 4) return launch_conv0pool<4, true>(a, frames, st, pdl);
   const int cp = first_layer_cp(C);
-  return cp == 4 ? launch_conv0pool<4, false>(a, frames, st)
-                 : (cp == 8 ? launch_conv0pool<8, false>(a, frames, st) : launch_conv0pool<16, false>(a, frames, st));
-}
-
-}
+  return cp == 4 ? launch_conv0pool<4, false>(a, frames, st, pdl)
+                 : (cp == 8 ? launch_conv0pool<8, false>(a, frames, st, pdl)
+                            : launch_conv0pool<16, false>(a, frames, st, pdl));
+}
+
+}
diff --git a/seed_rl_b200/csrc/conv_planes.cu b/seed_rl_b200/csrc/conv_planes.cu
--- a/seed_rl_b200/csrc/conv_planes.cu
+++ b/seed_rl_b200/csrc/conv_planes.cu
@@ -121,6 +121,8 @@
   }
   asm volatile("fence.proxy.async.shared::cta;" ::: "memory");
   __syncthreads();
+  pdl_wait();
+  pdl_trigger();
 
   const int my_tiles = ((int)blockIdx.x < a.ntiles) ? (a.ntiles - 1 - (int)blockIdx.x) / (int)gridDim.x + 1 : 0;
   bool timed_out = false;
@@ -285,8 +287,7 @@
   a.out_raw = reinterpret_cast<uint4*>(c.out_raw); a.out_relu = reinterpret_cast<uint4*>(c.out_relu);
   a.out_nhwc = c.out_nhwc; a.err = c.err;
   const int grid = a.ntiles < kNumSMs ? a.ntiles : kNumSMs;
-  convp_kernel<CIN, COUT, NSUB><<<grid, kCpThreads, smem, st>>>(tm, a);
-  count_launch(g_conv_cat, st);
+  launch_kernel(c.pdl, g_conv_cat, convp_kernel<CIN, COUT, NSUB>, grid, kCpThreads, smem, st, tm, a);
   SEEDRL_CHECK_LAUNCH();
   return SEEDRL_OK;
 }
@@ -353,6 +354,8 @@
     asm volatile("fence.mbarrier_init.release.cluster;" ::: "memory");
   }
   __syncthreads();
+  pdl_wait();
+  pdl_trigger();
 
   const int my_chunks = ((int)blockIdx.x < a.nchunks) ? (a.nchunks - 1 - (int)blockIdx.x) / (int)gridDim.x + 1 : 0;
   bool timed_out = false;
@@ -474,8 +477,7 @@
     return set_error(SEEDRL_ERR_INVALID_ARGUMENT, "wgradp: partial buffer too small");
   a.partial = batch->buf + batch->used;
   batch->used += (size_t)grid * NW;
-  wgradp_kernel<CP, COUT, KC><<<grid, wgradp_threads(CP), smem, st>>>(tm, a);
-  count_launch(PC_CONV_WGRAD, st);
+  launch_kernel(true, PC_CONV_WGRAD, wgradp_kernel<CP, COUT, KC>, grid, wgradp_threads(CP), smem, st, tm, a);
   SEEDRL_CHECK_LAUNCH();
   batch->jobs[batch->n++] = ReduceJob{a.partial, dw, db, grid, 9 * CP * COUT, COUT};
   return SEEDRL_OK;
@@ -501,6 +503,8 @@
 
 __global__ void to_planes_kernel(ConvGeom g, int Lp, int G, int relu, const float* __restrict__ x,
                                  uint4* __restrict__ out) {
+  pdl_wait();
+  pdl_trigger();
   const long long i = (long long)blockIdx.x * blockDim.x + threadIdx.x;
   if (i >= (long long)Lp * G) return;
   const int s = (int)(i / G), go = (int)(i - (long long)s * G);
@@ -519,6 +523,8 @@
 }
 
 __global__ void from_planes_kernel(ConvGeom g, int Lp, int G, const uint4* __restrict__ in, float* __restrict__ y) {
+  pdl_wait();
+  pdl_trigger();
   const long long i = (long long)blockIdx.x * blockDim.x + threadIdx.x;
   if (i >= (long long)Lp * G) return;
   const int s = (int)(i / G), go = (int)(i - (long long)s * G);
@@ -536,9 +542,8 @@
   const ConvGeom g = make_geom(N, H, W);
   const long long Lp = planes_positions(N, H, W);
   const long long n = Lp * (C / 8);
-  to_planes_kernel<<<(unsigned)((n + 255) / 256), 256, 0, st>>>(g, (int)Lp, C / 8, relu, x,
-                                                                reinterpret_cast<uint4*>(out));
-  count_launch(PC_MISC, st);
+  launch_kernel(true, PC_MISC, to_planes_kernel, (unsigned)((n + 255) / 256), 256, 0, st, g, (int)Lp, C / 8, relu, x,
+                reinterpret_cast<uint4*>(out));
   SEEDRL_CHECK_LAUNCH();
   return SEEDRL_OK;
 }
@@ -546,9 +551,8 @@
   const ConvGeom g = make_geom(N, H, W);
   const long long Lp = planes_positions(N, H, W);
   const long long n = Lp * (C / 8);
-  from_planes_kernel<<<(unsigned)((n + 255) / 256), 256, 0, st>>>(g, (int)Lp, C / 8,
-                                                                  reinterpret_cast<const uint4*>(in), y);
-  count_launch(PC_MISC, st);
+  launch_kernel(true, PC_MISC, from_planes_kernel, (unsigned)((n + 255) / 256), 256, 0, st, g, (int)Lp, C / 8,
+                reinterpret_cast<const uint4*>(in), y);
   SEEDRL_CHECK_LAUNCH();
   return SEEDRL_OK;
 }
@@ -556,6 +560,8 @@
 __global__ void poolp_fwd_kernel(ConvGeom go_, int Lp, int G, int H, int W, int pt, int pl,
                                  const float* __restrict__ x, uint4* __restrict__ out_raw,
                                  uint4* __restrict__ out_relu, uint8_t* __restrict__ idx) {
+  pdl_wait();
+  pdl_trigger();
   const long long i = (long long)blockIdx.x * blockDim.x + threadIdx.x;
   if (i >= (long long)Lp * G) return;
   const int s = (int)(i / G), gq = (int)(i - (long long)s * G);
@@ -604,6 +610,8 @@
 __global__ void poolp_bwd_kernel(ConvGeom gf, int Lpf, ConvGeom gp, int Lpp, int G, int pt, int pl,
                                  const uint4* __restrict__ dy, const uint8_t* __restrict__ idx,
                                  uint4* __restrict__ dx_planes, float* __restrict__ dx_nhwc) {
+  pdl_wait();
+  pdl_trigger();
   const long long i = (long long)blockIdx.x * blockDim.x + threadIdx.x;
   const int H = gf.H, W = gf.W, Ho = gp.H, Wo = gp.W, C = G * 8;
   int gq, s = 0, pix;
@@ -665,10 +673,8 @@
   const ConvGeom g = make_geom(N, Ho, Wo);
   const long long Lp = planes_positions(N, Ho, Wo);
   const long long n = Lp * (C / 8);
-  poolp_fwd_kernel<<<(unsigned)((n + 255) / 256), 256, 0, st>>>(g, (int)Lp, C / 8, H, W, pt, pl, x,
-                                                                reinterpret_cast<uint4*>(out_raw),
-                                                                reinterpret_cast<uint4*>(out_relu), idx);
-  count_launch(PC_POOL, st);
+  launch_kernel(true, PC_POOL, poolp_fwd_kernel, (unsigned)((n + 255) / 256), 256, 0, st, g, (int)Lp, C / 8, H, W,
+                pt, pl, x, reinterpret_cast<uint4*>(out_raw), reinterpret_cast<uint4*>(out_relu), idx);
   SEEDRL_CHECK_LAUNCH();
   return SEEDRL_OK;
 }
@@ -682,15 +688,14 @@
   const long long Lpf = planes_positions(N, H, W), Lpp = planes_positions(N, Ho, Wo);
   if (dx_planes) {
     const long long n = Lpf * (C / 8);
-    poolp_bwd_kernel<true><<<(unsigned)((n + 255) / 256), 256, 0, st>>>(
-        gf, (int)Lpf, gp, (int)Lpp, C / 8, pt, pl, reinterpret_cast<const uint4*>(dy), idx,
-        reinterpret_cast<uint4*>(dx_planes), nullptr);
+    launch_kernel(true, PC_POOL, poolp_bwd_kernel<true>, (unsigned)((n + 255) / 256), 256, 0, st, gf, (int)Lpf, gp,
+                  (int)Lpp, C / 8, pt, pl, reinterpret_cast<const uint4*>(dy), idx,
+                  reinterpret_cast<uint4*>(dx_planes), nullptr);
   } else {
     const long long n = (long long)N * H * W * (C / 8);
-    poolp_bwd_kernel<false><<<(unsigned)((n + 255) / 256), 256, 0, st>>>(
-        gf, (int)Lpf, gp, (int)Lpp, C / 8, pt, pl, reinterpret_cast<const uint4*>(dy), idx, nullptr, dx_nhwc);
-  }
-  count_launch(PC_POOL, st);
+    launch_kernel(true, PC_POOL, poolp_bwd_kernel<false>, (unsigned)((n + 255) / 256), 256, 0, st, gf, (int)Lpf, gp,
+                  (int)Lpp, C / 8, pt, pl, reinterpret_cast<const uint4*>(dy), idx, nullptr, dx_nhwc);
+  }
   SEEDRL_CHECK_LAUNCH();
   return SEEDRL_OK;
 }
diff --git a/seed_rl_b200/csrc/conv_tc_kernels.cu b/seed_rl_b200/csrc/conv_tc_kernels.cu
--- a/seed_rl_b200/csrc/conv_tc_kernels.cu
+++ b/seed_rl_b200/csrc/conv_tc_kernels.cu
@@ -33,6 +33,8 @@
 }
 
 __global__ void pack_w_tc_batch_kernel(const __grid_constant__ PackTable t, int split) {
+  pdl_wait();
+  pdl_trigger();
   const PackJob j = t.jobs[blockIdx.y];
   const int CIN = j.ck, COUT = j.cout;
   const int i = blockIdx.x * blockDim.x + threadIdx.x;
@@ -64,8 +66,7 @@
 
 int conv3x3_tc_pack_weights_batch(const PackTable& t, int split, cudaStream_t st) {
   if (t.n == 0) return SEEDRL_OK;
-  pack_w_tc_batch_kernel<<<dim3(ceil_div(9 * 32 * 32, 256), t.n), 256, 0, st>>>(t, split);
-  count_launch(PC_MISC, st);
+  launch_kernel(true, PC_MISC, pack_w_tc_batch_kernel, dim3(ceil_div(9 * 32 * 32, 256), t.n), 256, 0, st, t, split);
   SEEDRL_CHECK_LAUNCH();
   return SEEDRL_OK;
 }
@@ -554,6 +555,8 @@
 }
 
 __global__ void wgrad_reduce_batch_kernel(const __grid_constant__ ReduceTable t) {
+  pdl_wait();
+  pdl_trigger();
   const ReduceJob j = t.jobs[blockIdx.y];
   const int i = blockIdx.x * blockDim.x + threadIdx.x;
   if (i >= j.nw + j.nb) return;
@@ -580,8 +583,7 @@
     t.jobs[i] = b->jobs[i];
     if (b->jobs[i].nw + b->jobs[i].nb > maxn) maxn = b->jobs[i].nw + b->jobs[i].nb;
   }
-  wgrad_reduce_batch_kernel<<<dim3(ceil_div(maxn, 256), b->n), 256, 0, st>>>(t);
-  count_launch(PC_CONV_WGRAD, st);
+  launch_kernel(true, PC_CONV_WGRAD, wgrad_reduce_batch_kernel, dim3(ceil_div(maxn, 256), b->n), 256, 0, st, t);
   SEEDRL_CHECK_LAUNCH();
   b->n = 0;
   b->used = 0;
diff --git a/seed_rl_b200/csrc/gemm_kernels.cu b/seed_rl_b200/csrc/gemm_kernels.cu
--- a/seed_rl_b200/csrc/gemm_kernels.cu
+++ b/seed_rl_b200/csrc/gemm_kernels.cu
@@ -80,6 +80,8 @@
 __global__ void __launch_bounds__(256) rowdot_kernel(int M, int K, const float* __restrict__ A, int lda,
                                                       const float* __restrict__ b, const float* __restrict__ bias,
                                                       float* __restrict__ C) {
+  pdl_wait();
+  pdl_trigger();
   const int row = blockIdx.x * (blockDim.x >> 5) + (threadIdx.x >> 5), lane = threadIdx.x & 31;
   if (row >= M) return;
   const float* a = A + (size_t)row * lda;
@@ -93,14 +95,12 @@
           float* C, int ldc, const GemmEpi& e, cudaStream_t st) {
   if (M <= 0 || N <= 0) return SEEDRL_OK;
   if (!ta && !tb && N == 1 && ldb == 1 && ldc == 1 && !e.mask && !e.relu && !e.accumulate && !e.a_relu) {
-    rowdot_kernel<<<ceil_div(M, 8), 256, 0, st>>>(M, K, A, lda, B, e.bias, C);
-    count_launch(PC_GEMM, st);
+    launch_kernel(true, PC_GEMM, rowdot_kernel, ceil_div(M, 8), 256, 0, st, M, K, A, lda, B, e.bias, C);
     SEEDRL_CHECK_LAUNCH();
     return SEEDRL_OK;
   }
   if (ta && N == 1 && ldc == 1 && !e.bias && !e.mask && !e.relu && !e.accumulate && !e.a_relu) {
-    colsum_kernel<<<ceil_div(M, 32), 1024, 0, st>>>(K, M, A, lda, B, ldb, C);
-    count_launch(PC_GEMM, st);
+    launch_kernel(true, PC_GEMM, colsum_kernel, ceil_div(M, 32), 1024, 0, st, K, M, A, lda, B, ldb, C);
     SEEDRL_CHECK_LAUNCH();
     return SEEDRL_OK;
   }
@@ -126,6 +126,8 @@
 colsum_kernel(int M, int N, const float* __restrict__ X, int ld, const float* __restrict__ w, int ldw,
               float* __restrict__ out) {
   __shared__ float red[32][33];
+  pdl_wait();
+  pdl_trigger();
   const int lane = threadIdx.x & 31, wid = threadIdx.x >> 5;
   const int n = blockIdx.x * 32 + lane;
   float s0 = 0.f, s1 = 0.f, s2 = 0.f, s3 = 0.f;
@@ -156,6 +158,8 @@
 __global__ void __launch_bounds__(512)
 colsum_slab_kernel(int M, int N, int rps, const float* __restrict__ X, float* __restrict__ part) {
   __shared__ float4 red[512];
+  pdl_wait();
+  pdl_trigger();
   const int t = threadIdx.x;
   const size_t r0 = (size_t)blockIdx.x * rps;
   const size_t r1 = r0 + rps < (size_t)M ? r0 + rps : (size_t)M;
@@ -196,17 +200,14 @@
     if (rps < 8 * sweep) rps = 8 * sweep;
     const int S = ceil_div(M, rps);
     if ((size_t)S * N * sizeof(float) <= ws_bytes && S > 1) {
-      colsum_slab_kernel<<<S, 512, 0, st>>>(M, N, rps, X, ws);
-      count_launch(PC_GEMM, st);
+      launch_kernel(true, PC_GEMM, colsum_slab_kernel, S, 512, 0, st, M, N, rps, X, ws);
       SEEDRL_CHECK_LAUNCH();
-      colsum_kernel<<<ceil_div(N, 32), 1024, 0, st>>>(S, N, ws, N, nullptr, 0, out);
-      count_launch(PC_GEMM, st);
+      launch_kernel(true, PC_GEMM, colsum_kernel, ceil_div(N, 32), 1024, 0, st, S, N, ws, N, nullptr, 0, out);
       SEEDRL_CHECK_LAUNCH();
       return SEEDRL_OK;
     }
   }
-  colsum_kernel<<<ceil_div(N, 32), 1024, 0, st>>>(M, N, X, ld, nullptr, 0, out);
-  count_launch(PC_GEMM, st);
+  launch_kernel(true, PC_GEMM, colsum_kernel, ceil_div(N, 32), 1024, 0, st, M, N, X, ld, nullptr, 0, out);
   SEEDRL_CHECK_LAUNCH();
   return SEEDRL_OK;
 }
diff --git a/seed_rl_b200/csrc/gemm_tc_kernels.cu b/seed_rl_b200/csrc/gemm_tc_kernels.cu
--- a/seed_rl_b200/csrc/gemm_tc_kernels.cu
+++ b/seed_rl_b200/csrc/gemm_tc_kernels.cu
@@ -118,6 +118,8 @@
 #pragma unroll
   for (int i = 0; i < kGtMaxBN / 2; ++i) acc[i] = 0.f;
   wgmma_fence_acc<kGtMaxBN / 2>(acc);
+  pdl_wait();
+  pdl_trigger();
 
   for (int kb = 0; kb < nkb; ++kb) {
     const int st = kb & 1;
@@ -224,6 +226,8 @@
 __global__ void gemm_tc_reduce_kernel(int M, int N, int splits, const float* __restrict__ ws,
                                       float* __restrict__ C, int ldc, GemmEpi e) {
   constexpr int W = VEC ? 4 : 1;
+  pdl_wait();
+  pdl_trigger();
   const int i = (blockIdx.x * blockDim.x + threadIdx.x) * W;
   if (i >= M * N) return;
   const int m = i / N, n = i - m * N;
@@ -255,6 +259,8 @@
 gemm_tc_reduce_wide_kernel(int M, int N, int splits, const float* __restrict__ ws, float* __restrict__ C, int ldc,
                            GemmEpi e) {
   __shared__ float4 part[8][32];
+  pdl_wait();
+  pdl_trigger();
   const int o = threadIdx.x & 31, zl = threadIdx.x >> 5;
   const int i = (blockIdx.x * 32 + o) * 4;
   const bool in = i < M * N;
@@ -355,7 +361,7 @@
 #define SEEDRL_GT_LAUNCH2(TA_, TB_, SP_, G_)                                                    \
   do {                                                                                          \
     SEEDRL_CUDA(allow_smem<gemm_tc_kernel<TA_, TB_, SP_, G_>>(200 * 1024));                     \
-    gemm_tc_kernel<TA_, TB_, SP_, G_><<<grid, kGtThreads, smem, st>>>(p);                       \
+    launch_kernel(true, PC_GEMM, gemm_tc_kernel<TA_, TB_, SP_, G_>, grid, kGtThreads, smem, st, p);    \
   } while (0)
 #define SEEDRL_GT_LAUNCH(TA_, TB_, SP_)                                                         \
   do {                                                                                          \
@@ -375,16 +381,17 @@
   }
 #undef SEEDRL_GT_LAUNCH
 #undef SEEDRL_GT_LAUNCH2
-  count_launch(PC_GEMM, st);
   SEEDRL_CHECK_LAUNCH();
   if (splits > 1) {
     if ((N & 3) == 0 && splits >= 16)
-      gemm_tc_reduce_wide_kernel<<<ceil_div(M * N / 4, 32), 256, 0, st>>>(M, N, splits, ws, C, ldc, e);
+      launch_kernel(true, PC_GEMM, gemm_tc_reduce_wide_kernel, ceil_div(M * N / 4, 32), 256, 0, st, M, N, splits, ws,
+                    C, ldc, e);
     else if ((N & 3) == 0)
-      gemm_tc_reduce_kernel<true><<<ceil_div(M * N / 4, 256), 256, 0, st>>>(M, N, splits, ws, C, ldc, e);
+      launch_kernel(true, PC_GEMM, gemm_tc_reduce_kernel<true>, ceil_div(M * N / 4, 256), 256, 0, st, M, N, splits,
+                    ws, C, ldc, e);
     else
-      gemm_tc_reduce_kernel<false><<<ceil_div(M * N, 256), 256, 0, st>>>(M, N, splits, ws, C, ldc, e);
-    count_launch(PC_GEMM, st);
+      launch_kernel(true, PC_GEMM, gemm_tc_reduce_kernel<false>, ceil_div(M * N, 256), 256, 0, st, M, N, splits, ws,
+                    C, ldc, e);
     SEEDRL_CHECK_LAUNCH();
   }
   return SEEDRL_OK;
diff --git a/seed_rl_b200/csrc/kernels.h b/seed_rl_b200/csrc/kernels.h
--- a/seed_rl_b200/csrc/kernels.h
+++ b/seed_rl_b200/csrc/kernels.h
@@ -90,6 +90,7 @@
   void* out_relu;
   float* out_nhwc;
   int* err;
+  bool pdl = false;
 };
 bool convp_supported(int cin, int cout);
 int convp_forward(int cin, int cout, const PlaneConv& c, cudaStream_t st);
@@ -107,7 +108,7 @@
                        float* dw, float* db, WgradBatch* batch, cudaStream_t st);
 bool conv0pool_supported(int cin, int cout, int H, int W);
 int conv0pool_forward(int N, int H, int W, int C, const uint8_t* frames, const float* w, const float* bias,
-                      void* praw, void* prelu, uint8_t* idx, int* err, cudaStream_t st);
+                      void* praw, void* prelu, uint8_t* idx, int* err, cudaStream_t st, bool pdl = false);
 
 int conv3x3_forward(int cin, int cout, int in_mode, int N, int H, int W, const void* in,
                     const float* w, const float* bias, const float* mask, const float* res,
diff --git a/seed_rl_b200/csrc/lstm.cu b/seed_rl_b200/csrc/lstm.cu
--- a/seed_rl_b200/csrc/lstm.cu
+++ b/seed_rl_b200/csrc/lstm.cu
@@ -49,6 +49,8 @@
 
 __global__ void core_input_tail_kernel(int Nrows, int D, int A, bool clip, const float* __restrict__ reward,
                                        const int64_t* __restrict__ prev_action, float* __restrict__ core_in) {
+  pdl_wait();
+  pdl_trigger();
   const int i = blockIdx.x * blockDim.x + threadIdx.x;
   const int Wd = 1 + A;
   if (i >= Nrows * Wd) return;
@@ -70,9 +72,8 @@
   GemmEpi e = epi_none();
   e.bias = prm + t.offset(k.dense_b); e.relu = 1; e.a_relu = k.flat_relu;
   SEEDRL_TRY(ex.gemm(false, false, N, H, k.flat, flat, k.flat, prm + t.offset(k.dense_w), H, xc, CI, e));
-  core_input_tail_kernel<<<ceil_div(N * (1 + k.A), 256), 256, 0, st>>>(N, H, k.A, k.clip_reward, reward,
-                                                                       prev_actions, xc);
-  count_launch(PC_MISC, st);
+  launch_kernel(true, PC_MISC, core_input_tail_kernel, ceil_div(N * (1 + k.A), 256), 256, 0, st, N, H, k.A,
+                k.clip_reward, reward, prev_actions, xc);
   SEEDRL_CHECK_LAUNCH();
   e = epi_none();
   e.bias = prm + t.offset(k.b);
diff --git a/seed_rl_b200/csrc/net.cu b/seed_rl_b200/csrc/net.cu
--- a/seed_rl_b200/csrc/net.cu
+++ b/seed_rl_b200/csrc/net.cu
@@ -241,7 +241,9 @@
   }
   return conv3x3_tc_pack_weights_batch(c.packed, n->conv_mode == 3 ? 2 : (n->conv_mode >= 2 ? 1 : 0), c.ex.st);
 }
-static int packed_weights(const Call& c, int cin, int cout, const float* w, int flip, int split, const void** wq) {
+static int packed_weights(const Call& c, int cin, int cout, const float* w, int flip, int split, const void** wq,
+                          bool* early = nullptr) {
+  if (early) *early = true;
   for (int i = 0; i < c.packed.n; ++i)
     if (c.packed.jobs[i].w == w && c.packed.jobs[i].flip == flip) {
       *wq = c.packed.jobs[i].wq;
@@ -250,6 +252,7 @@
   void* scratch = W<void>(c.ws, c.pl.wq);
   SEEDRL_TRY(conv3x3_tc_pack_weights(cin, cout, flip, split, w, scratch, c.ex.st));
   *wq = scratch;
+  if (early) *early = false;
   return SEEDRL_OK;
 }
 
@@ -264,11 +267,13 @@
   const float* r = res ? c.at<float>(res->raw) : nullptr;
   const void* wq;
   if (in.planes) {
-    SEEDRL_TRY(packed_weights(c, cin, cout, w, flip, 2, &wq));
+    bool early;
+    SEEDRL_TRY(packed_weights(c, cin, cout, w, flip, 2, &wq, &early));
     PlaneConv pc;
     pc.N = N; pc.H = H; pc.W = Wd; pc.in = x; pc.wq = wq; pc.bias = bias; pc.mask = m; pc.res = r;
     pc.out_raw = out.planes ? c.at(out.raw) : nullptr; pc.out_relu = out.planes ? c.at(out.relu) : nullptr;
     pc.out_nhwc = out.planes ? nullptr : c.at<float>(out.raw); pc.err = c.ex.err;
+    pc.pdl = early;
     return convp_forward(cin, cout, pc, st);
   }
   if (c.n->conv_mode >= 1 && conv3x3_tc_supported(cin, cout, in_mode)) {
@@ -353,7 +358,7 @@
   const void* wq;
   if (c.first == kFirstFused)
     return conv0pool_forward(N, k.hin, k.win, first_c(n), obs, w, bias, c.at(b.p.raw), c.at(b.p.relu),
-                             c.at<uint8_t>(b.idx), c.ex.err, st);
+                             c.at<uint8_t>(b.idx), c.ex.err, st, true);
   if (c.first == kFirstStaged) {
     SEEDRL_TRY(packed_weights(c, k.cin, k.c, w, 0, split, &wq));
     SEEDRL_TRY(conv3x3_tc_forward(k.cin, k.c, IN_U8, split, N, k.hin, k.win, obs, wq, bias, nullptr, nullptr, a0,
diff --git a/seed_rl_b200/csrc/optim_kernels.cu b/seed_rl_b200/csrc/optim_kernels.cu
--- a/seed_rl_b200/csrc/optim_kernels.cu
+++ b/seed_rl_b200/csrc/optim_kernels.cu
@@ -14,6 +14,8 @@
   const float4* g4 = reinterpret_cast<const float4*>(g);
   float4* m4 = reinterpret_cast<float4*>(m);
   float4* v4 = reinterpret_cast<float4*>(v);
+  pdl_wait();
+  pdl_trigger();
   for (size_t i = tid; i < n4; i += stride) {
     float4 pp = p4[i], gg = g4[i], mm = m4[i], vv = v4[i];
 #define SEEDRL_ADAM1(c)                                   \
@@ -38,6 +40,8 @@
 }
 
 __global__ void clamp_one_kernel(float* p, long long idx, float lo, float hi) {
+  pdl_wait();
+  pdl_trigger();
   p[idx] = fminf(fmaxf(p[idx], lo), hi);
 }
 
@@ -59,16 +63,12 @@
   int blocks = (int)ceil_div_sz(n4 > 0 ? n4 : 1, 256);
   const int max_blocks = kNumSMs * 8;
   if (blocks > max_blocks) blocks = max_blocks;
-  adam_kernel<<<blocks, 256, 0, (cudaStream_t)stream>>>(n, params, grads, m, v, lr_t, beta1,
-                                                         beta2, eps, grad_scale,
-                                                         (long long)clamp_index, clamp_lo,
-                                                         clamp_hi);
-  count_launch(PC_ADAM, (cudaStream_t)stream);
+  launch_kernel(true, PC_ADAM, adam_kernel, blocks, 256, 0, (cudaStream_t)stream, n, params, grads, m, v, lr_t,
+                beta1, beta2, eps, grad_scale, (long long)clamp_index, clamp_lo, clamp_hi);
   SEEDRL_CHECK_LAUNCH();
   if (clamp_index >= 0) {
-    clamp_one_kernel<<<1, 1, 0, (cudaStream_t)stream>>>(params, (long long)clamp_index, clamp_lo,
-                                                         clamp_hi);
-    count_launch(PC_ADAM, (cudaStream_t)stream);
+    launch_kernel(true, PC_ADAM, clamp_one_kernel, 1, 1, 0, (cudaStream_t)stream, params, (long long)clamp_index,
+                  clamp_lo, clamp_hi);
     SEEDRL_CHECK_LAUNCH();
   }
   return SEEDRL_OK;
diff --git a/seed_rl_b200/csrc/vtrace_kernels.cu b/seed_rl_b200/csrc/vtrace_kernels.cu
--- a/seed_rl_b200/csrc/vtrace_kernels.cu
+++ b/seed_rl_b200/csrc/vtrace_kernels.cu
@@ -632,8 +632,14 @@
   loss_finalize<POPART>(p, s_red, ec);
 }
 
-__global__ void __launch_bounds__(kLossThreads) vtrace_loss_kernel(const LossParams p) { loss_small_body<false>(p); }
+__global__ void __launch_bounds__(kLossThreads) vtrace_loss_kernel(const LossParams p) {
+  pdl_wait();
+  pdl_trigger();
+  loss_small_body<false>(p);
+}
 __global__ void __launch_bounds__(kLossThreads) vtrace_popart_loss_kernel(const LossParams p) {
+  pdl_wait();
+  pdl_trigger();
   loss_small_body<true>(p);
 }
 
@@ -932,6 +938,8 @@
 vtrace_loss_stream_kernel(const LossParams p, const int ntiles, const int tile_stride_f,
                           const __grid_constant__ CUtensorMap tm_bl, const __grid_constant__ CUtensorMap tm_ll,
                           const __grid_constant__ CUtensorMap tm_dl) {
+  pdl_wait();
+  pdl_trigger();
   loss_stream_body<AS, false>(p, ntiles, tile_stride_f, tm_bl, tm_ll, tm_dl);
 }
 template <int AS>
@@ -939,6 +947,8 @@
 vtrace_popart_loss_stream_kernel(const LossParams p, const int ntiles, const int tile_stride_f,
                                  const __grid_constant__ CUtensorMap tm_bl, const __grid_constant__ CUtensorMap tm_ll,
                                  const __grid_constant__ CUtensorMap tm_dl) {
+  pdl_wait();
+  pdl_trigger();
   loss_stream_body<AS, true>(p, ntiles, tile_stride_f, tm_bl, tm_ll, tm_dl);
 }
 
@@ -964,6 +974,8 @@
 __global__ void __launch_bounds__(kPopThreads)
 vtrace_popart_update_kernel(const PopArtUpdateParams p) {
   __shared__ bool s_last;
+  pdl_wait();
+  pdl_trigger();
   const int tid = threadIdx.x;
   const float mu1 = p.mom[0], mu2 = p.mom[1], sigma = p.comp[0], mu = p.comp[1];
   const float bm1 = (float)((double)p.sums[0] / p.count), bm2 = (float)((double)p.sums[1] / p.count);
@@ -1107,9 +1119,8 @@
   if (per_sm < 1) per_sm = 1;
   int grid = num_sms() * per_sm;
   if (grid > ntiles) grid = ntiles;
-  kernel<<<grid, threads, smem, stream>>>(
-      p, ntiles, stream_tile_stride_f(p.T, p.A, p.BB), tm_bl, tm_ll, tm_dl);
-  return cudaSuccess;
+  return launch_kernel(true, PC_LOSS, kernel, grid, threads, smem, stream, p, ntiles,
+                       stream_tile_stride_f(p.T, p.A, p.BB), tm_bl, tm_ll, tm_dl);
 }
 
 }
@@ -1224,9 +1235,8 @@
   } else {
     p.BB = pick_bb(p.T, B, A, &smem);
     SEEDRL_CHECK_ARG(p.BB > 0, "unroll_length * num_actions too large for shared memory");
-    small_kernel<<<ceil_div(B, p.BB), kLossThreads, smem, st>>>(p);
-  }
-  count_launch(PC_LOSS, st);
+    launch_kernel(true, PC_LOSS, small_kernel, ceil_div(B, p.BB), kLossThreads, smem, st, p);
+  }
   SEEDRL_CHECK_LAUNCH();
   return SEEDRL_OK;
 }
@@ -1309,8 +1319,7 @@
   p.partials = reinterpret_cast<double*>(reinterpret_cast<char*>(scratch) + 256);
   const size_t n = (size_t)p.T * B;
   const int grid = (int)std::min<size_t>(ceil_div_sz(n, (size_t)kPopThreads * 4), (size_t)kNumSMs);
-  vtrace_popart_update_kernel<<<grid, kPopThreads, 0, (cudaStream_t)stream>>>(p);
-  count_launch(PC_LOSS, (cudaStream_t)stream);
+  launch_kernel(true, PC_LOSS, vtrace_popart_update_kernel, grid, kPopThreads, 0, (cudaStream_t)stream, p);
   SEEDRL_CHECK_LAUNCH();
   return SEEDRL_OK;
 }
```
